# scrose/pylc

Measured on AMD Instinct MI355X. Metric: 512x512 tiles/sec fwd+bwd (DeepLabV3+/ResNet101, 9-class), higher is better.
Workload: dtype f32; 1 GPU; DeepLabV3+ ResNet101 OS16, 3-ch 512x512 tiles, 9 classes, CE+Dice+Focal, clip 0.5 + AdamW, bs=32/GPU (BASELINE.json configs[2]); global_batch=32, parallelism=dp1, conv_arithmetic=f16x3 split (fp32-grade), rccl_ranks=0, wgrad_queue=compute stream, sync_bn=True, activation_format=fp16 planes between BatchNorm and conv kernels (4 B/element)

## Files before the change

### include/pylc_hip.h

```cpp
#ifndef PYLC_HIP_H
#define PYLC_HIP_H

#include <stddef.h>
#include <stdint.h>

#ifdef __cplusplus
extern "C" {
#endif

#define PYLC_OK 0
#define PYLC_ERR_ARG 1
#define PYLC_ERR_HIP 2
#define PYLC_ERR_WORKSPACE 3
#define PYLC_ERR_UNSUPPORTED 4

const char* pylc_last_error(void);
int pylc_abi_version(void);
int pylc_experimental_build(void);
int pylc_init(void);

typedef struct PylcConvDesc {
    int B, H, W;
    int Cin, Cout;
    int R, S;
// ... 38 lines not shown
int pylc_to_planes(const float* x, int x_pitch, void* planes, int p_pitch, long long plane_stride, long long M, int C,
                   const unsigned int* amax, int nplanes, void* stream);
int pylc_from_planes(const void* planes, int p_pitch, long long plane_stride, float* x, int x_pitch, long long M, int C,
                     const unsigned int* amax, int nplanes, void* stream);
size_t pylc_planes_colsum_workspace_floats(int C);
int pylc_upsample2_crop_concat_planes(const float* z, int z_pitch, int B, int h, int w, int C1, const float* bridge, int bridge_pitch, int HH, int WW,
                                      int C2, void* planes, long long plane_stride, int nplanes, const unsigned int* bound, void* stream);
int pylc_planes_colsum(const void* planes, int p_pitch, long long plane_stride, int nplanes, const unsigned int* amax, long long M, int C,
                       float* sums, float* workspace, void* stream);

int pylc_conv2d_fwd(const PylcConvDesc* d, const float* x, const float* w_krsc, const float* bias,
                    float* y, void* stream);
int pylc_conv2d_fwd_bnact(const PylcConvDesc* d, const float* x, const float* w_krsc, const float* bias,
                          const float* scale, const float* shift, const float* residual, int relu, float* y,
                          unsigned int* amax_out, void* stream);

typedef struct PylcFwdEp {
    const float* scale;
    const float* shift;
    const unsigned int* scale_amax;
    const unsigned int* shift_amax;
    const void* residual;
    int res_fmt;
    const unsigned int* res_scale_bound;
    const unsigned int* res_amax;
    const unsigned int* x_true_amax;
    int relu;
    unsigned int* amax_out;
} PylcFwdEp;
int pylc_conv2d_fwd_bnact_ex(const PylcConvDesc* d, const void* x, const float* w, const float* bias, const PylcFwdEp* ep, void* y, void* stream);
size_t pylc_conv2d_fwd_stats_floats(const PylcConvDesc* d);
int pylc_conv2d_fwd_stats(const PylcConvDesc* d, const float* x, const float* w_krsc, const float* bias,
                          float* y, float* stats_partial, int* stats_rows, void* stream);
int pylc_conv2d_dgrad(const PylcConvDesc* d, const float* dy, const float* w_crsk, float* dx,
                      int accumulate, void* stream);
int pylc_conv2d_dgrad_add(const PylcConvDesc* d, const float* dy, const float* w_crsk, float* dx, int accumulate,
                          const float* add_src, const void* add_mask, void* stream);
#ifdef PYLC_EXPERIMENTAL
typedef struct PylcBnBack {
    const float* y;
    const float* mean;
    const float* invstd;
    const float* scale;
    const float* shift;
    const void* relu_mask;
    int relu;
    unsigned int* g_amax;
} PylcBnBack;
size_t pylc_conv2d_dgrad_bn_floats(const PylcConvDesc* d);
int pylc_conv2d_dgrad_bn(const PylcConvDesc* d, const float* dy, const float* w_crsk, float* dx, int accumulate,
                         const float* add_src, const void* add_mask, const PylcBnBack* bn, float* sums_partial, int* sums_rows,
                         void* stream);
#endif
int pylc_relu_bwd_bits(const float* dout, const void* mask, float* g_out, long long M, int C, void* stream);
int pylc_conv2d_dgrad_needs_f32_weights(const PylcConvDesc* d);
size_t pylc_conv2d_wgrad_workspace(const PylcConvDesc* d);
int pylc_conv2d_wgrad(const PylcConvDesc* d, const float* x, const float* dy, float* dw_krsc,
                      float* dbias ,
                      void* workspace, size_t workspace_bytes, void* stream);
typedef struct PylcSlabSum {
    const float* slabs;
    float* dw;
    long long n4;
    long long slab_stride;
    int splits;
    int reserved;
// ... 56 lines not shown
int pylc_bn_apply(const float* y, int y_pitch, const float* scale, const float* shift,
                  const float* residual, int res_pitch, float* out, int out_pitch,
                  long long M, int C, int relu, unsigned int* amax_out, void* stream);
int pylc_bn_bwd_reduce(const float* dout, int dout_pitch, const float* out, int out_pitch,
                       const float* y, int y_pitch, const float* mean, const float* invstd,
                       long long M, int C, int relu, float* sums , float* workspace,
                       const float* scale, const float* shift, void* stream);
int pylc_bn_bwd_apply(const float* dout, int dout_pitch, const float* out, int out_pitch,
                      const float* y, int y_pitch, const float* mean, const float* invstd,
                      const float* gamma, const float* sums, double n,
                      long long M, int C, int relu, float* dy, int dy_pitch, float* g_out, int g_pitch,
                      unsigned int* amax_dy, const float* scale, const float* shift, void* stream);
typedef struct PylcBnExtra {
    void* out_planes;        long long out_plane_stride;  const unsigned int* out_bound;
    const void* res_planes;  long long res_plane_stride;  const unsigned int* res_amax;
    void* dy_planes;         long long dy_plane_stride;   const unsigned int* dy_bound;
    int nplanes;
    float drop_p;
    uint64_t drop_seed;
    unsigned int* g_amax;
    void* relu_mask;
    const unsigned int* y_half_bound;
    const unsigned int* dout_half_bound;
} PylcBnExtra;
int pylc_bn_finalize_ex(const float* sums, double n, int C, const float* gamma, const float* beta, float eps, float momentum,
                        int clamp_eps, float* running_mean, float* running_var, float* mean, float* invstd, float* scale,
                        float* shift, const unsigned int* bound_extra, float bound_mul, unsigned int* bound_out,
                        const float* y, int y_pitch, long long M, const float* stat_shift, void* stream);
int pylc_bn_finalize_from_partial_ex(const float* partial, int n_rows, double n, int C, const float* gamma, const float* beta,
                                     float eps, float momentum, int clamp_eps, float* running_mean, float* running_var,
                                     float* mean, float* invstd, float* scale, float* shift, const unsigned int* bound_extra,
                                     float bound_mul, unsigned int* bound_out, const float* y, int y_pitch, long long M,
                                     const float* stat_shift, void* stream);
int pylc_bn_local_moments(const float* sums, double n, int C, const float* y, int y_pitch, long long M, const float* stat_shift,
                          double* moments, void* stream);
int pylc_bn_finalize_moments(const double* moments, double n, int C, const float* gamma, const float* beta, float eps, float momentum,
                             int clamp_eps, float* running_mean, float* running_var, float* mean, float* invstd, float* scale,
                             float* shift, const unsigned int* bound_extra, float bound_mul, unsigned int* bound_out,
                             const float* stat_shift, void* stream);
int pylc_bn_apply_ex(const float* y, int y_pitch, const float* scale, const float* shift, const float* residual, int res_pitch,
                     float* out, int out_pitch, long long M, int C, int relu, unsigned int* amax_out, const PylcBnExtra* ex,
                     void* stream);
int pylc_bn_bwd_reduce_ex(const float* dout, int dout_pitch, const float* out, int out_pitch, const float* y, int y_pitch,
                          const float* mean, const float* invstd, long long M, int C, int relu, float* sums, float* workspace,
                          const float* scale, const float* shift, const float* gamma, double n, const PylcBnExtra* ex,
                          unsigned int* dy_bound_out, void* stream);
int pylc_bn_bwd_bound(const float* sums, const float* gamma, const float* invstd, double n, int C, const unsigned int* g_amax,
                      unsigned int* bound_out, void* stream);
#ifdef PYLC_EXPERIMENTAL
int pylc_bn_bwd_sums_from_partial(const float* partial, int rows, int C, float* sums, const float* gamma, const float* invstd, double n,
                                  const unsigned int* g_amax, unsigned int* dy_bound_out, void* stream);
#endif
int pylc_bn_bwd_apply_ex(const float* dout, int dout_pitch, const float* out, int out_pitch, const float* y, int y_pitch,
                         const float* mean, const float* invstd, const float* gamma, const float* sums, double n, long long M,
                         int C, int relu, float* dy, int dy_pitch, float* g_out, int g_pitch, unsigned int* amax_dy,
                         const float* scale, const float* shift, const PylcBnExtra* ex, void* stream);
typedef struct PylcBnTwin {
    const float* y;          int y_pitch;
    const float* scale;      const float* shift;
    const float* mean;       const float* invstd;         const float* gamma;
    float* sums;             float* workspace;            unsigned int* dy_bound_out;
    float* dy;               int dy_pitch;
    void* dy_planes;         long long dy_plane_stride;   const unsigned int* dy_bound;
    unsigned int* amax_dy;
} PylcBnTwin;
int pylc_bn_affine_amax(const float* y, int y_pitch, const float* scale, const float* shift, long long M, int C, unsigned int* amax_out,
// ... 229 lines not shown
```

### pylc_amd/csrc/bn.hip

```cpp
#include "conv_common.h"
#include "slab.h"

namespace pylc {

struct PlanesRef {
    _Float16* base;
    long long plane_stride;
    int nplanes;
    float scale;
};

__device__ __forceinline__ void planes_store4(const PlanesRef& p, long long elem, f32x4 v) {
    uint2 p0, p1;
    split2(v, p.scale, p0, p1);
    if (p.nplanes == 2) {
        const bool odd = threadIdx.x & 1;
        const uint2 send = odd ? p0 : p1;
        uint2 recv;
        recv.x = (unsigned)__builtin_amdgcn_update_dpp(0, (int)send.x, 0xB1, 0xF, 0xF, true);
        recv.y = (unsigned)__builtin_amdgcn_update_dpp(0, (int)send.y, 0xB1, 0xF, 0xF, true);
        const uint4 val = odd ? make_uint4(recv.x, recv.y, p1.x, p1.y) : make_uint4(p0.x, p0.y, recv.x, recv.y);
        const bool il = planes_il(p.plane_stride);
        _Float16* dst = odd ? p.base + p.plane_stride + planes_phys(elem - 4, il) : p.base + planes_phys(elem, il);
        *reinterpret_cast<uint4*>(dst) = val;
// ... 304 lines not shown
    __shared__ double red[2][32][9];
    const int tx = threadIdx.x & 7, ty = threadIdx.x >> 3;
    const int c = blockIdx.x * 8 + tx;
    const bool mine = ty == 0 && c < C;
    bn_finalize_tail(mine ? (double)sums[c] : 0.0, mine ? (double)sums[C + c] : 0.0, red, tx, ty, c, n, C, gamma, beta, eps, momentum, clamp_eps,
                     running_mean, running_var, mean, invstd, scale, shift, bound_extra, bound_mul, bound_out, src);
}

__global__ __launch_bounds__(256) void bn_local_moments_kernel(const float* __restrict__ sums, double n, int C, RefineSrc src,
                                                               double* __restrict__ moments) {
    __shared__ double red[2][32][9];
    const int tx = threadIdx.x & 7, ty = threadIdx.x >> 3;
    const int c = blockIdx.x * 8 + tx;
    const bool mine = ty == 0 && c < C;
    double S1, S2;
    bn_local_moments(mine ? (double)sums[c] : 0.0, mine ? (double)sums[C + c] : 0.0, red, tx, ty, c, n, C, src, S1, S2);
    if (mine) {
        moments[c] = S1;
        moments[C + c] = S2;
        if (c == 0) moments[2 * C] = n;
    }
}

__global__ void bn_finalize_moments_kernel(const double* __restrict__ moments, double n, int C, const float* __restrict__ gamma,
                                           const float* __restrict__ beta, float eps, float momentum, int clamp_eps, float* running_mean,
                                           float* running_var, float* mean, float* invstd, float* scale, float* shift,
                                           const unsigned* bound_extra, float bound_mul, unsigned* bound_out, const float* stat_shift) {
    const int c = blockIdx.x * blockDim.x + threadIdx.x;
    if (c >= C) return;
    bn_coeffs_from_moments(moments[c], moments[C + c], stat_shift != nullptr ? (double)stat_shift[c] : 0.0, c, n, gamma, beta, eps, momentum,
                           clamp_eps, running_mean, running_var, mean, invstd, scale, shift, bound_extra, bound_mul, bound_out);
}

__global__ __launch_bounds__(256) void bn_finalize_partial_kernel(const float* __restrict__ partial, int nrows, double n, int C,
                                                                  const float* __restrict__ gamma, const float* __restrict__ beta, float eps,
                                                                  float momentum, int clamp_eps, float* running_mean, float* running_var,
                                                                  float* mean, float* invstd, float* scale, float* shift,
                                                                  const unsigned* bound_extra, float bound_mul, unsigned* bound_out,
                                                                  RefineSrc src) {
    __shared__ double red[2][32][9];
    const int tx = threadIdx.x & 7, ty = threadIdx.x >> 3;
    const int c = blockIdx.x * 8 + tx;
    double a0 = 0.0, a1 = 0.0;
    if (c < C) {
        for (int r = ty; r < nrows; r += 8 * 32) {
            float v0[8], v1[8];
#pragma unroll
            for (int u = 0; u < 8; ++u) {
                const int rr = r + u * 32;
                const size_t row = rr < nrows ? (size_t)rr : 0;
                v0[u] = partial[row * 2 * C + c];
                v1[u] = partial[row * 2 * C + C + c];
            }
#pragma unroll
            for (int u = 0; u < 8; ++u) {
                const bool ok = r + u * 32 < nrows;
                a0 += ok ? (double)v0[u] : 0.0;
                a1 += ok ? (double)v1[u] : 0.0;
            }
        }
    }
    red[0][ty][tx] = a0;
    red[1][ty][tx] = a1;
    __syncthreads();
    double s0 = 0.0, s1 = 0.0;
    if (ty == 0) {
#pragma unroll
        for (int k = 0; k < 32; ++k) { s0 += red[0][k][tx]; s1 += red[1][k][tx]; }
    }
    bn_finalize_tail((double)(float)s0, (double)(float)s1, red, tx, ty, c, n, C, gamma, beta, eps, momentum, clamp_eps, running_mean, running_var,
                     mean, invstd, scale, shift, bound_extra, bound_mul, bound_out, src);
}

__global__ void bn_eval_coeffs_kernel(const float* rm, const float* rv, const float* gamma, const float* beta, float eps,
                                      int C, float* scale, float* shift, float* mean, float* invstd) {
    const int c = blockIdx.x * blockDim.x + threadIdx.x;
    if (c >= C) return;
    const float sc = gamma[c] / sqrtf(rv[c] + eps);
    scale[c] = sc;
    shift[c] = beta[c] - rm[c] * sc;
    if (mean != nullptr) {
        mean[c] = rm[c];
        invstd[c] = 1.f / sqrtf(rv[c] + eps);
    }
}

template <bool EX = false, bool DROP = false, bool BITS = false, bool YH = false, bool TWIN = false>
__global__ __launch_bounds__(256) void bn_apply_kernel(const float* __restrict__ y, int y_pitch,
                                                       const float* __restrict__ scale, const float* __restrict__ shift,
                                                       const float* __restrict__ res, int res_pitch, float* __restrict__ out,
                                                       int out_pitch, int relu, Slab g, unsigned* __restrict__ amax_out, BnEx ex, BnTw tw) {
    const int tx = threadIdx.x % g.cols, ty = threadIdx.x / g.cols;
    const long long r_begin = (long long)blockIdx.x * g.rows_per_slab;
    long long r_end = r_begin + g.rows_per_slab;
    if (r_end > g.M) r_end = g.M;
    float amax = 0.f;
    PlanesRef po{}, pr{};
    DropRef dr{};
    float res_inv = 1.f;
    if constexpr (EX) {
        if (ex.out_pl != nullptr) po = PlanesRef{ex.out_pl, ex.out_ps, ex.nplanes, pow2_scale_for(*ex.out_bound)};
        if (ex.res_pl != nullptr) {
            pr = PlanesRef{const_cast<_Float16*>(ex.res_pl), ex.res_ps, ex.nplanes, 1.f};
            res_inv = 1.f / pow2_scale_for(*ex.res_amax);
// ... 419 lines not shown
}

extern "C" int pylc_bn_finalize_ex(const float* sums, double n, int C, const float* gamma, const float* beta, float eps, float momentum,
                                   int clamp_eps, float* running_mean, float* running_var, float* mean, float* invstd, float* scale,
                                   float* shift, const unsigned int* bound_extra, float bound_mul, unsigned int* bound_out,
                                   const float* y, int y_pitch, long long M, const float* stat_shift, void* stream) {
    PYLC_REQUIRE(sums && gamma && beta && mean && invstd && scale && shift && C > 0 && n > 0, "bn_finalize: bad arguments");
    PYLC_REQUIRE((running_mean == nullptr) == (running_var == nullptr), "bn_finalize: running stats must both be set or both NULL");
    PYLC_REQUIRE(y == nullptr || (y_pitch >= C && M > 0 && (double)M == n), "bn_finalize: the refinement source must be the n rows the sums cover");
    hipLaunchKernelGGL(bn_finalize_kernel, dim3(cdiv(C, 8)), dim3(256), 0, as_stream(stream), sums, n, C, gamma, beta, eps, momentum,
                       clamp_eps, running_mean, running_var, mean, invstd, scale, shift, bound_extra, bound_mul, bound_out,
                       RefineSrc{y, y_pitch, M, stat_shift});
    PYLC_LAUNCH_CHECK();
    return PYLC_OK;
}

extern "C" int pylc_bn_finalize(const float* sums, double n, int C, const float* gamma, const float* beta, float eps, float momentum,
                                int clamp_eps, float* running_mean, float* running_var, float* mean, float* invstd, float* scale,
                                float* shift, void* stream) {
    return pylc_bn_finalize_ex(sums, n, C, gamma, beta, eps, momentum, clamp_eps, running_mean, running_var, mean, invstd, scale, shift,
                               nullptr, 1.f, nullptr, nullptr, 0, 0, nullptr, stream);
}

extern "C" int pylc_bn_finalize_from_partial_ex(const float* partial, int n_rows, double n, int C, const float* gamma, const float* beta,
                                                float eps, float momentum, int clamp_eps, float* running_mean, float* running_var,
                                                float* mean, float* invstd, float* scale, float* shift, const unsigned int* bound_extra,
                                                float bound_mul, unsigned int* bound_out, const float* y, int y_pitch, long long M,
                                                const float* stat_shift, void* stream) {
    PYLC_REQUIRE(partial && n_rows > 0 && gamma && beta && mean && invstd && scale && shift && C > 0 && n > 0,
                 "bn_finalize_from_partial: bad arguments");
    PYLC_REQUIRE((running_mean == nullptr) == (running_var == nullptr), "bn_finalize_from_partial: running stats must both be set or both NULL");
    PYLC_REQUIRE(y == nullptr || (y_pitch >= C && M > 0 && (double)M == n),
                 "bn_finalize_from_partial: the refinement source must be the n rows the partials cover");
    hipLaunchKernelGGL(bn_finalize_partial_kernel, dim3(cdiv(C, 8)), dim3(256), 0, as_stream(stream), partial, n_rows, n, C, gamma, beta, eps,
                       momentum, clamp_eps, running_mean, running_var, mean, invstd, scale, shift, bound_extra, bound_mul, bound_out,
                       RefineSrc{y, y_pitch, M, stat_shift});
    PYLC_LAUNCH_CHECK();
    return PYLC_OK;
}

extern "C" int pylc_bn_finalize_from_partial(const float* partial, int n_rows, double n, int C, const float* gamma, const float* beta,
                                             float eps, float momentum, int clamp_eps, float* running_mean, float* running_var,
                                             float* mean, float* invstd, float* scale, float* shift, void* stream) {
    return pylc_bn_finalize_from_partial_ex(partial, n_rows, n, C, gamma, beta, eps, momentum, clamp_eps, running_mean, running_var, mean,
                                            invstd, scale, shift, nullptr, 1.f, nullptr, nullptr, 0, 0, nullptr, stream);
}

extern "C" int pylc_bn_local_moments(const float* sums, double n, int C, const float* y, int y_pitch, long long M, const float* stat_shift,
                                     double* moments, void* stream) {
    PYLC_REQUIRE(sums && moments && C > 0 && n > 0, "bn_local_moments: bad arguments");
    PYLC_REQUIRE(y == nullptr || (y_pitch >= C && M > 0 && (double)M == n), "bn_local_moments: the refinement source must be the n rows the sums cover");
    hipLaunchKernelGGL(bn_local_moments_kernel, dim3(cdiv(C, 8)), dim3(256), 0, as_stream(stream), sums, n, C, RefineSrc{y, y_pitch, M, stat_shift},
                       moments);
    PYLC_LAUNCH_CHECK();
    return PYLC_OK;
}

extern "C" int pylc_bn_finalize_moments(const double* moments, double n, int C, const float* gamma, const float* beta, float eps,
                                        float momentum, int clamp_eps, float* running_mean, float* running_var, float* mean, float* invstd,
                                        float* scale, float* shift, const unsigned int* bound_extra, float bound_mul,
                                        unsigned int* bound_out, const float* stat_shift, void* stream) {
    PYLC_REQUIRE(moments && gamma && beta && mean && invstd && scale && shift && C > 0 && n > 0, "bn_finalize_moments: bad arguments");
    PYLC_REQUIRE((running_mean == nullptr) == (running_var == nullptr), "bn_finalize_moments: running stats must both be set or both NULL");
    hipLaunchKernelGGL(bn_finalize_moments_kernel, dim3(cdiv(C, 256)), dim3(256), 0, as_stream(stream), moments, n, C, gamma, beta, eps, momentum,
                       clamp_eps, running_mean, running_var, mean, invstd, scale, shift, bound_extra, bound_mul, bound_out, stat_shift);
    PYLC_LAUNCH_CHECK();
    return PYLC_OK;
}

// ... 393 lines not shown
```

### pylc_amd/csrc/conv_common.h

```cpp
#pragma once
#include "common.h"
#include <type_traits>

namespace pylc {

typedef float f32x4 __attribute__((ext_vector_type(4)));
typedef float f32x16 __attribute__((ext_vector_type(16)));

typedef __bf16 bf16x8 __attribute__((ext_vector_type(8)));

typedef _Float16 f16x8 __attribute__((ext_vector_type(8)));
typedef _Float16 f16x2 __attribute__((ext_vector_type(2)));
typedef float f32x2 __attribute__((ext_vector_type(2)));

constexpr int LDB = 80;

__device__ __forceinline__ void split3(const float (&x)[4], uint2& p0, uint2& p1, uint2& p2) {
    unsigned u0[4], u1[4], u2[4];
#pragma unroll
    for (int e = 0; e < 4; ++e) {
        u0[e] = __float_as_uint(x[e]);
        const float r1 = x[e] - __uint_as_float(u0[e] & 0xFFFF0000u);
        u1[e] = __float_as_uint(r1);
        const float r2 = r1 - __uint_as_float(u1[e] & 0xFFFF0000u);
// ... 63 lines not shown
    const float* ep_scale;
    const float* ep_shift;
    const float* ep_res;
    unsigned* ep_amax;
    int ep_relu;
    int ep_vec_ok;
    const unsigned* bound_x;
    const unsigned* ep_scale_amax;
    const unsigned* ep_shift_amax;
    const unsigned* ep_res_amax;
    const unsigned* ep_res_scale;
    int ep_res_fmt;
    long long ep_res_plane_stride;
    int out_planes2;
    long long out_plane_stride;
    int tiles_n;
    int n_tiles;
    const unsigned* amax_x;
    const unsigned* amax_w;
    long long x_bytes, w_bytes;
    const void* w_planes;
    long long w_plane_stride;
    int w_il;
    const void* x_planes;
    long long x_plane_stride;
    int nterms;
    int tile_bm;
    int halo_tiles_m;
    int ident;
    int stagger, stagger_blocks;
    int dbg_flags;
    unsigned long long* dbg;
    float* stats;
};

typedef float f32x4v __attribute__((ext_vector_type(4)));

__device__ __forceinline__ float row_sum16(float v) {
#define PYLC_DPP_ADD(ctrl) v += __builtin_bit_cast(float, __builtin_amdgcn_update_dpp(0, __builtin_bit_cast(int, v), ctrl, 0xF, 0xF, true))
    PYLC_DPP_ADD(0xB1);
    PYLC_DPP_ADD(0x4E);
    PYLC_DPP_ADD(0x141);
    PYLC_DPP_ADD(0x140);
#undef PYLC_DPP_ADD
    return v;
}


struct WgradArgs {
    const float* x;
    const float* dy;
    float* out;
    int M, P, Q;
    int IH, IW, Cin, x_pitch, in_sh, in_sw;
    int TR, TS, dh0, dh_step, dw0, dw_step;
    int N, N_ld, dy_pitch;
    int out_row_stride;
    int tiles_n, tiles_c;
    int splits, m_per_split;
    long long slab_stride;
    const unsigned* amax_dy;
    const unsigned* amax_x;
    long long x_bytes, dy_bytes;
    const void* x_planes;
    const void* dy_planes;
    long long x_plane_stride, dy_plane_stride;
// ... 34 lines not shown
```

### pylc_amd/csrc/conv_igemm.hip

```cpp
#include "conv_common.h"

namespace pylc {

template <int BM, int BN, int WM, int WN, bool CIN4, int PREC>
__global__ __launch_bounds__((BM / WM) * (BN / WN) * 64, 2) void gather_gemm_kernel(const GatherGemmArgs a) {
    constexpr int WAVES_N = BN / WN;
    constexpr int MT = WM / 32, NT = WN / 32;
    constexpr int NTHR = (BM / WM) * (BN / WN) * 64;
    constexpr int RPI = NTHR / 8;
    constexpr int A_IT = BM / RPI, B_IT = BN / RPI;
    static_assert(NTHR == 256 || NTHR == 512, "4 or 8 waves per block");
    static_assert(BM % RPI == 0 && BN % RPI == 0, "tile rows must divide evenly over the loader");
    extern __shared__ __attribute__((aligned(16))) float smem[];
    float* sA = smem;
    float* sB = smem + 2 * BM * LDT;

    const int tile = xcd_remap(blockIdx.x, gridDim.x);
    const int m0 = (tile / a.tiles_n) * BM;
    const int n0 = (tile % a.tiles_n) * BN;
    const int tid = threadIdx.x, lane = tid & 63, wave = tid >> 6;
    const int wave_m = wave / WAVES_N, wave_n = wave % WAVES_N;
    const int v = tid & 7, r0 = tid >> 3;

    int rowh[A_IT], roww[A_IT], rowpix[A_IT];
// ... 1506 lines not shown
    const int ow = (d->W + 2 * d->pad - d->dil * (d->S - 1) - 1) / d->stride + 1;
    PYLC_REQUIRE(oh == d->OH && ow == d->OW && oh > 0 && ow > 0, "OH/OW (%d,%d) inconsistent with geometry (%d,%d)", d->OH, d->OW, oh, ow);
    PYLC_REQUIRE((long long)d->B * d->H * d->W * d->x_pitch < (1ll << 31) && (long long)d->B * d->OH * d->OW * d->y_pitch < (1ll << 31),
                 "tensor exceeds 2^31 elements");
    return PYLC_OK;
}

static inline int roundup4(int v) { return (v + 3) & ~3; }

}

using namespace pylc;

extern "C" int pylc_set_conv_precision(int mode) {
    PYLC_REQUIRE(mode >= 0 && mode <= 3, "conv precision mode must be 0 (fp32 MFMA), 1 (bf16x6), 2 (f16x3) or 3 (fp16 operands, fp32 accumulation)");
    g_conv_precision = mode;
    return PYLC_OK;
}

extern "C" int pylc_get_conv_precision(void) { return g_conv_precision; }

extern "C" int pylc_debug_pp_stamps(unsigned long long* buf) { g_pp_stamps = buf; return PYLC_OK; }
extern "C" int pylc_debug_pp_flags(int flags) { g_pp_flags = flags; g_wgrad_fast = !(flags & 8); return PYLC_OK; }

extern "C" int pylc_debug_set_big_tile(int on) { g_big_tile = on; return PYLC_OK; }

namespace {
struct FwdEpilogue {
    const float* scale; const float* shift; const float* res; unsigned* amax; int relu;
    const PylcFwdEp* ex = nullptr;
};
}
static int conv2d_fwd_impl(const PylcConvDesc* d, const float* x, const float* w, const float* bias, float* y, float* stats, int* stats_rows,
                           void* stream, const FwdEpilogue* ep = nullptr);

extern "C" int pylc_conv2d_fwd(const PylcConvDesc* d, const float* x, const float* w, const float* bias, float* y, void* stream) {
    return conv2d_fwd_impl(d, x, w, bias, y, nullptr, nullptr, stream);
}

extern "C" int pylc_conv2d_fwd_bnact(const PylcConvDesc* d, const float* x, const float* w, const float* bias, const float* scale,
                                     const float* shift, const float* residual, int relu, float* y, unsigned int* amax_out, void* stream) {
    PYLC_REQUIRE(scale && shift, "conv2d_fwd_bnact: null scale / shift");
    const FwdEpilogue ep{scale, shift, residual, amax_out, relu};
    return conv2d_fwd_impl(d, x, w, bias, y, nullptr, nullptr, stream, &ep);
}

extern "C" int pylc_conv2d_fwd_bnact_ex(const PylcConvDesc* d, const void* x, const float* w, const float* bias, const PylcFwdEp* ep, void* y,
                                        void* stream) {
    PYLC_REQUIRE(ep != nullptr && ep->scale && ep->shift, "conv2d_fwd_bnact_ex: null epilogue / scale / shift");
    PYLC_REQUIRE(d->x_fmt == 1, "conv2d_fwd_bnact_ex: x must be an fp16-plane tensor (pylc_conv2d_fwd_bnact takes fp32 tensors)");
    PYLC_REQUIRE(ep->res_fmt >= 0 && ep->res_fmt <= 2 && (ep->res_fmt == 0 || (ep->residual && ep->res_scale_bound)),
                 "conv2d_fwd_bnact_ex: res_fmt 1 / 2 needs the residual planes and the bound they were scaled with");
    PYLC_REQUIRE(d->out_fmt == 0 || (d->out_bound && ep->scale_amax && ep->shift_amax && (ep->residual == nullptr || ep->res_amax)),
                 "conv2d_fwd_bnact_ex: a plane output needs out_bound, max|scale|, max|shift| and (with a residual) max|residual|");
    const FwdEpilogue fe{ep->scale, ep->shift, ep->res_fmt == 0 ? static_cast<const float*>(ep->residual) : nullptr, ep->amax_out, ep->relu, ep};
    return conv2d_fwd_impl(d, static_cast<const float*>(x), w, bias, static_cast<float*>(y), nullptr, nullptr, stream, &fe);
}

extern "C" size_t pylc_conv2d_fwd_stats_floats(const PylcConvDesc* d) {
    if (check_desc(d)) return 0;
    const long long M = (long long)d->B * d->OH * d->OW;
    return (size_t)cdiv<long long>(M, 128) * 2 * (size_t)roundup4(d->Cout);
}

extern "C" int pylc_conv2d_fwd_stats(const PylcConvDesc* d, const float* x, const float* w, const float* bias, float* y, float* stats_partial,
                                     int* stats_rows, void* stream) {
    PYLC_REQUIRE(stats_partial && stats_rows, "conv2d_fwd_stats: null statistics buffer");
    return conv2d_fwd_impl(d, x, w, bias, y, stats_partial, stats_rows, stream);
}

static int conv2d_fwd_impl(const PylcConvDesc* d, const float* x, const float* w, const float* bias, float* y, float* stats, int* stats_rows,
                           void* stream, const FwdEpilogue* ep) {
    if (int rc = check_desc(d)) return rc;
    PYLC_REQUIRE(x && y && (w || (d->x_fmt == 1 && d->w_planes)), "null pointer");
    GatherGemmArgs a{};
    if (ep != nullptr) {
        a.ep_scale = ep->scale; a.ep_shift = ep->shift; a.ep_res = ep->res; a.ep_amax = ep->amax; a.ep_relu = ep->relu;
        a.ep_vec_ok = ((reinterpret_cast<uintptr_t>(ep->scale) | reinterpret_cast<uintptr_t>(ep->shift) | reinterpret_cast<uintptr_t>(bias)) & 15) == 0;
    }
    a.stats = stats;
    a.dbg = g_pp_stamps;
    a.dbg_flags = g_pp_flags;
    PYLC_REQUIRE(g_conv_precision < 2 || (d->x_amax && d->w_amax), "f16x3 / fp16 mode: conv2d_fwd needs x_amax and w_amax in the descriptor");
    a.amax_x = d->x_amax; a.amax_w = d->w_amax;
    a.x = x; a.w = w; a.bias = bias; a.y = y;
    a.x_bytes = (((long long)d->B * d->H * d->W - 1) * d->x_pitch + d->Cin) * 4;
    a.w_bytes = (long long)d->Cout * d->R * d->S * d->Cin * 4;
    a.w_planes = d->w_planes; a.w_plane_stride = (long long)d->Cout * d->R * d->S * d->Cin;
    a.w_il = (d->w_planes != nullptr && (d->w_planes_fmt & 1)) ? 1 : 0;
    if (d->x_fmt == 1) {
        a.x_planes = x; a.x = nullptr;
        a.x_plane_stride = planes_stride_rule((long long)d->B * d->H * d->W, d->Cin, d->x_pitch, (g_conv_precision == 3 ? 1 : 2));
        a.x_bytes /= 2;
    }
    a.P = d->OH; a.Q = d->OW; a.M = d->B * d->OH * d->OW;
    a.IH = d->H; a.IW = d->W; a.Cin = d->Cin; a.x_pitch = d->x_pitch;
    a.in_sh = a.in_sw = d->stride;
    a.TR = d->R; a.TS = d->S;
    a.dh0 = -d->pad; a.dh_step = d->dil; a.dw0 = -d->pad; a.dw_step = d->dil;
    a.w_off0 = 0; a.w_step_r = d->S * d->Cin; a.w_step_s = d->Cin; a.w_row_stride = d->R * d->S * d->Cin;
    a.N = d->Cout; a.N_store = roundup4(d->Cout) <= d->y_pitch ? roundup4(d->Cout) : d->Cout;
    a.OH = d->OH; a.OW = d->OW; a.out_sh = a.out_sw = 1; a.oh0 = a.ow0 = 0; a.y_pitch = d->y_pitch;
    a.accumulate = 0;
    if (ep != nullptr && ep->ex != nullptr) {
        const PylcFwdEp* ex = ep->ex;
        a.bound_x = ex->x_true_amax;
        a.ep_scale_amax = ex->scale_amax; a.ep_shift_amax = ex->shift_amax;
        if (ex->residual != nullptr) {
            a.ep_res = static_cast<const float*>(ex->residual);
            a.ep_res_fmt = ex->res_fmt; a.ep_res_scale = ex->res_scale_bound; a.ep_res_amax = ex->res_amax;
            a.ep_res_plane_stride = planes_stride_rule((long long)d->B * d->OH * d->OW, d->Cout, d->Cout, ex->res_fmt == 2 ? 2 : 1);
        }
        if (d->out_fmt != 0) {
            PYLC_REQUIRE((d->out_fmt == 1 || d->out_fmt == 2) && d->y_pitch == d->Cout && d->Cout % 4 == 0,
                         "conv2d_fwd_bnact_ex: a plane output (out_fmt 1 / 2) needs a dense y with Cout %% 4 == 0");
            a.out_half = d->out_fmt == 1; a.out_planes2 = d->out_fmt == 2;
            a.out_plane_stride = planes_stride_rule((long long)d->B * d->OH * d->OW, d->Cout, d->y_pitch, d->out_fmt == 2 ? 2 : 1);
            a.out_bound_k = (float)(d->Cin * d->R * d->S); a.out_bound = d->out_bound;
        }
    } else if (d->out_fmt == 1) {
        PYLC_REQUIRE(d->x_fmt == 1 && d->out_bound && bias == nullptr && ep == nullptr && d->y_pitch == d->Cout && d->Cout % 4 == 0,
                     "conv2d_fwd: a one-plane fp16 output needs fp16-plane input, out_bound, no bias / fused epilogue and a dense y");
        a.out_half = 1; a.out_bound_k = (float)(d->Cin * d->R * d->S); a.out_bound = d->out_bound;
    }
    const bool cin4 = d->Cin == 4 && d->R * d->S > 1;
    if (cin4 && ep == nullptr && takes_stem(a)) {
        if (int rc = launch_stem_fwd(a, as_stream(stream))) return rc;
    } else if (int rc = dispatch_gg(a, cin4, as_stream(stream))) return rc;
    if (stats_rows) *stats_rows = a.halo_tiles_m > 0 ? a.halo_tiles_m : cdiv(a.M, a.x_planes != nullptr ? a.tile_bm : (a.tiles_n > 0 ? g_last_bm : 128));
    return PYLC_OK;
}

extern "C" int pylc_conv2d_dgrad_needs_f32_weights(const PylcConvDesc* d) {
    if (check_desc(d)) return 1;
    if (g_conv_precision < 2 || d->w_planes_t == nullptr) return 1;
    if (d->dy_fmt == 1) return 0;
    if (d->stride != 1) return 1;
    const int Kp = roundup4(d->Cout);
    GatherGemmArgs a{};
    a.Cin = Kp;
    a.x_bytes = (((long long)d->B * d->OH * d->OW - 1) * d->y_pitch + Kp) * 4;
    a.w_bytes = (long long)d->Cin * d->R * d->S * Kp * 4;
    const long long M = (long long)d->B * d->H * d->W;
    const bool big = d->Cin > 64 && g_big_tile && cdiv<long long>(M, 256) * cdiv(d->Cin, 128) >= 192;
    return (big && takes_pp(a)) ? 0 : 1;
}

extern "C" int pylc_conv2d_dgrad_add(const PylcConvDesc* d, const float* dy, const float* w_crsk, float* dx, int accumulate,
                                     const float* add_src, const void* add_mask, void* stream);
extern "C" int pylc_conv2d_dgrad(const PylcConvDesc* d, const float* dy, const float* w_crsk, float* dx, int accumulate, void* stream) {
    return pylc_conv2d_dgrad_add(d, dy, w_crsk, dx, accumulate, nullptr, nullptr, stream);
}

struct BnBackArgs { const float* y; const float* mean; const float* invstd; const float* scale; const float* shift; const void* relu_mask; int relu; unsigned int* g_amax; };
static int conv2d_dgrad_impl(const PylcConvDesc* d, const float* dy, const float* w_crsk, float* dx, int accumulate,
                             const float* add_src, const void* add_mask, const BnBackArgs* bn, float* sums_partial, int* sums_rows, void* stream);

extern "C" int pylc_conv2d_dgrad_add(const PylcConvDesc* d, const float* dy, const float* w_crsk, float* dx, int accumulate,
                                     const float* add_src, const void* add_mask, void* stream) {
    return conv2d_dgrad_impl(d, dy, w_crsk, dx, accumulate, add_src, add_mask, nullptr, nullptr, nullptr, stream);
}
// ... 304 lines not shown
```

### pylc_amd/csrc/conv_pl.hip

```cpp
#include "conv_common.h"

namespace pylc {

typedef __attribute__((address_space(3))) void* lds_vptr;

constexpr int PL_BN = 128;
constexpr int PL_ROW = 64;
template <int NTERMS>
constexpr int pl_row_bytes() { return NTERMS == 1 ? 128 : PL_ROW; }
template <int NTERMS, int BM>
constexpr int pl_stage_bytes() { return (NTERMS == 3 ? 2 : 1) * (BM + PL_BN) * pl_row_bytes<NTERMS>(); }
template <int BM>
constexpr int pl_stages() { return BM == 256 ? 3 : 2; }
template <int NTERMS, int BM>
constexpr int pl_lds_bytes() { return pl_stages<BM>() * pl_stage_bytes<NTERMS, BM>() + BM * 4 + 64; }

#ifndef PYLC_EPI_FULL_LINES
#define PYLC_EPI_FULL_LINES 1
#endif
#ifndef PYLC_EPI_PK
#define PYLC_EPI_PK 0
#endif
__device__ __forceinline__ f32x4v epi_fma(f32x4v a, float b, f32x4v c) {
#if PYLC_EPI_PK
    const f32x4v bb = {b, b, b, b};
    return __builtin_elementwise_fma(a, bb, c);
#else
    return f32x4v{__builtin_fmaf(a[0], b, c[0]), __builtin_fmaf(a[1], b, c[1]), __builtin_fmaf(a[2], b, c[2]), __builtin_fmaf(a[3], b, c[3])};
#endif
}
__device__ __forceinline__ f32x4v epi_mul(f32x4v a, float b) {
#if PYLC_EPI_PK
    return a * b;
#else
    return f32x4v{a[0] * b, a[1] * b, a[2] * b, a[3] * b};
#endif
}
__device__ __forceinline__ f32x4v epi_sq(f32x4v a) {
#if PYLC_EPI_PK
    return a * a;
#else
    return f32x4v{a[0] * a[0], a[1] * a[1], a[2] * a[2], a[3] * a[3]};
#endif
}
__device__ __forceinline__ f32x4v epi_add(f32x4v a, f32x4v b) {
#if PYLC_EPI_PK
    return a + b;
#else
    return f32x4v{a[0] + b[0], a[1] + b[1], a[2] + b[2], a[3] + b[3]};
#endif
}

template <int AM, int NPL, int NTERMS>
__device__ __forceinline__ void pl_step_schedule() {
    constexpr int AT = 4;
    if constexpr (AM >= 3) {
        __builtin_amdgcn_sched_group_barrier(0x100, (AT + 2) * NPL, 0);
        __builtin_amdgcn_sched_group_barrier(0x008, AT * NTERMS, 0);
#pragma unroll
        for (int r = 2; r < AM; ++r) {
            __builtin_amdgcn_sched_group_barrier(0x100, NPL, 0);
            __builtin_amdgcn_sched_group_barrier(0x008, AT * NTERMS, 0);
        }
        __builtin_amdgcn_sched_group_barrier(0x008, AT * NTERMS, 0);
    } else {
        __builtin_amdgcn_sched_group_barrier(0x100, (AT + AM) * NPL, 0);
        __builtin_amdgcn_sched_group_barrier(0x008, AM * AT * NTERMS, 0);
    }
}

template <int AM, int STATS, int PREV, bool HALF>
__device__ __forceinline__ void pl_epilogue_lean(const GatherGemmArgs& a, f32x4v (&acc)[AM][4], const int* rowoff,
                                                 float* sdst, int nb, int wave_m, int lane, float c, float hscale,
                                                 const float* extra, const unsigned char* amask, const float* bias) {
    constexpr int AT = 4, WM = 16 * AM;
    typedef _Float16 f16x4_ __attribute__((ext_vector_type(4)));
    typedef unsigned u32x2_ __attribute__((ext_vector_type(2)));
    unsigned offs[AM];
#pragma unroll
    for (int i = 0; i < AM; ++i) offs[i] = (unsigned)(rowoff[wave_m * WM + i * 16 + (lane & 15)] + nb);
    constexpr bool FULL = !HALF && PYLC_EPI_FULL_LINES != 0;
    unsigned offsP[FULL ? AM : 1];
    if constexpr (FULL) {
#pragma unroll
        for (int i = 0; i < AM; ++i) offsP[i] = (unsigned)(rowoff[wave_m * WM + i * 16 + ((lane & 15) ^ 8)] + nb);
    }
    const bool upper = (lane & 8) != 0;
    uint2 hq[(HALF && PYLC_EPI_FULL_LINES != 0) ? AM : 1][4];
    f32x4v hold[FULL ? AM : 1];
    f32x4v prevn[(FULL && PREV != 0) ? AM : 1];
    const float k = HALF ? c * hscale : c;
    const float post = HALF ? pow2_inv(hscale) : c;
    const bool odd_row = (lane >> 4) & 1;
#pragma unroll
    for (int j = 0; j < AT; ++j) {
        f32x4v prev[PREV ? AM : 1];
        if constexpr (PREV != 0) {
            unsigned mb[AM];
#pragma unroll
            for (int i = 0; i < AM; ++i) {
                if constexpr (!FULL) prev[i] = *reinterpret_cast<const f32x4v*>(extra + (offs[i] + j * 16));
                if constexpr (PREV == 2) mb[i] = amask[(offs[i] + j * 16) >> 3];
            }
            if constexpr (FULL) {
                if ((j & 1) == 0) {
                    const unsigned col = (upper ? j + 1 : j) * 16;
                    f32x4v la[AM], lb[AM];
#pragma unroll
                    for (int i = 0; i < AM; ++i) {
                        la[i] = *reinterpret_cast<const f32x4v*>(extra + ((upper ? offsP[i] : offs[i]) + col));
                        lb[i] = *reinterpret_cast<const f32x4v*>(extra + ((upper ? offs[i] : offsP[i]) + col));
                    }
#pragma unroll
                    for (int i = 0; i < AM; ++i)
#pragma unroll
                        for (int r = 0; r < 4; ++r) {
                            const float send = upper ? la[i][r] : lb[i][r];
                            const float recv = __builtin_bit_cast(float, __builtin_amdgcn_update_dpp(0, __builtin_bit_cast(int, send), 0x128, 0xF, 0xF, true));
                            prev[i][r] = upper ? recv : la[i][r];
                            prevn[i][r] = upper ? lb[i][r] : recv;
                        }
                } else {
#pragma unroll
                    for (int i = 0; i < AM; ++i) prev[i] = prevn[i];
                }
            }
            if constexpr (PREV == 2) {
#pragma unroll
                for (int i = 0; i < AM; ++i) {
                    const int nib = (int)(mb[i] >> ((((offs[i] + j * 16) >> 2) & 1u) * 4u));
#pragma unroll
                    for (int r = 0; r < 4; ++r)
                        prev[i][r] = __uint_as_float(__float_as_uint(prev[i][r]) & (unsigned)__builtin_amdgcn_sbfe(nib, r, 1));
                }
            }
        }
        f32x4v bv = {0.f, 0.f, 0.f, 0.f};
        if (!HALF && bias != nullptr) bv = *reinterpret_cast<const f32x4v*>(bias + nb + j * 16);
        f32x4v cs = {0.f, 0.f, 0.f, 0.f}, css = cs;
#pragma unroll
        for (int i = 0; i < AM; ++i) {
            const f32x4v t = acc[i][j];
            if constexpr (HALF) {
                const f32x4v v = epi_mul(t, k);
                const f16x4_ h = {(_Float16)v[0], (_Float16)v[1], (_Float16)v[2], (_Float16)v[3]};
                if constexpr (STATS != 0) {
#pragma unroll
                    for (int r = 0; r < 4; ++r) {
                        cs[r] = i == 0 ? (float)h[r] : __builtin_fmaf((float)h[r], 1.f, cs[r]);
                        css[r] = i == 0 ? (float)h[r] * (float)h[r] : __builtin_fmaf((float)h[r], (float)h[r], css[r]);
                    }
                }
                if constexpr (PYLC_EPI_FULL_LINES != 0) {
                    hq[i][j] = __builtin_bit_cast(uint2, h);
                } else {
                    const uint2 hu = __builtin_bit_cast(uint2, h);
                    const u32x2_ sx = __builtin_amdgcn_permlane16_swap(hu.x, hu.x, false, false);
                    const u32x2_ sy = __builtin_amdgcn_permlane16_swap(hu.y, hu.y, false, false);
                    if (!odd_row) *reinterpret_cast<uint4*>(reinterpret_cast<_Float16*>(a.y) + (offs[i] + j * 16)) = uint4{hu.x, hu.y, sx.y, sy.y};
                }
            } else {
                if constexpr (STATS != 0) {
                    cs = i == 0 ? t : epi_add(cs, t);
                    css = i == 0 ? epi_sq(t) : epi_add(css, epi_sq(t));
                }
                f32x4v v = epi_fma(t, k, bv);
                if constexpr (PREV != 0) v = epi_add(v, prev[i]);
                if constexpr (!FULL) {
                    *reinterpret_cast<f32x4v*>(a.y + (offs[i] + j * 16)) = v;
                } else if ((j & 1) == 0) {
                    hold[i] = v;
                } else {
                    f32x4v recv;
#pragma unroll
                    for (int r = 0; r < 4; ++r) {
                        const float send = upper ? hold[i][r] : v[r];
                        recv[r] = __builtin_bit_cast(float, __builtin_amdgcn_update_dpp(0, __builtin_bit_cast(int, send), 0x128, 0xF, 0xF, true));
                    }
                    const unsigned col = (upper ? j : j - 1) * 16;
                    f32x4v da, db;
#pragma unroll
                    for (int r = 0; r < 4; ++r) { da[r] = upper ? recv[r] : hold[i][r]; db[r] = upper ? v[r] : recv[r]; }
                    *reinterpret_cast<f32x4v*>(a.y + ((upper ? offsP[i] : offs[i]) + col)) = da;
                    *reinterpret_cast<f32x4v*>(a.y + ((upper ? offs[i] : offsP[i]) + col)) = db;
                }
            }
        }
        if constexpr (STATS != 0) {
#pragma unroll
            for (int r = 0; r < 4; ++r) { cs[r] = row_sum16(cs[r]); css[r] = row_sum16(css[r]); }
            if ((lane & 15) == 0) {
#pragma unroll
                for (int r = 0; r < 4; ++r) { sdst[(j * 16 + r) * 2] = cs[r] * post; sdst[(j * 16 + r) * 2 + 1] = css[r] * post * post; }
            }
        }
    }
    if constexpr (HALF && PYLC_EPI_FULL_LINES != 0) {
        unsigned offsP[AM];
#pragma unroll
        for (int i = 0; i < AM; ++i) offsP[i] = (unsigned)(rowoff[wave_m * WM + i * 16 + ((lane & 15) ^ 8)] + nb - 4 * (lane >> 4));
        const unsigned q4 = (unsigned)(lane >> 4);
        const unsigned colq = odd_row ? 16u + 4u * (q4 - 1u) : 4u * q4;
#pragma unroll
        for (int i = 0; i < AM; ++i) {
            const u32x2_ ax = __builtin_amdgcn_permlane16_swap(hq[i][0].x, hq[i][1].x, false, false);
            const u32x2_ ay = __builtin_amdgcn_permlane16_swap(hq[i][0].y, hq[i][1].y, false, false);
            const u32x2_ bx = __builtin_amdgcn_permlane16_swap(hq[i][2].x, hq[i][3].x, false, false);
            const u32x2_ by = __builtin_amdgcn_permlane16_swap(hq[i][2].y, hq[i][3].y, false, false);
            const unsigned s0 = upper ? ax.x : bx.x, s1 = upper ? ay.x : by.x, s2 = upper ? ax.y : bx.y, s3 = upper ? ay.y : by.y;
            const unsigned r0 = (unsigned)__builtin_amdgcn_update_dpp(0, (int)s0, 0x128, 0xF, 0xF, true);
            const unsigned r1 = (unsigned)__builtin_amdgcn_update_dpp(0, (int)s1, 0x128, 0xF, 0xF, true);
            const unsigned r2 = (unsigned)__builtin_amdgcn_update_dpp(0, (int)s2, 0x128, 0xF, 0xF, true);
            const unsigned r3 = (unsigned)__builtin_amdgcn_update_dpp(0, (int)s3, 0x128, 0xF, 0xF, true);
            const unsigned base_own = offs[i] - 4u * q4, base_par = offsP[i];
            const unsigned col = (upper ? 32u : 0u) + colq;
            const uint4 da = {upper ? r0 : ax.x, upper ? r1 : ay.x, upper ? r2 : ax.y, upper ? r3 : ay.y};
            const uint4 db = {upper ? bx.x : r0, upper ? by.x : r1, upper ? bx.y : r2, upper ? by.y : r3};
            *reinterpret_cast<uint4*>(reinterpret_cast<_Float16*>(a.y) + ((upper ? base_par : base_own) + col)) = da;
            *reinterpret_cast<uint4*>(reinterpret_cast<_Float16*>(a.y) + ((upper ? base_own : base_par) + col)) = db;
        }
    }
}

template <int AM, int PREV, bool EDGE>
__device__ __forceinline__ float pl_epilogue_bn(const GatherGemmArgs& a, f32x4v (&acc)[AM][4], const int* rowoff, float* sdst, int nb, int wave_m,
                                                int lane, float c, const float* extra, const unsigned char* amask) {
// ... 229 lines not shown
                    val[r] = t * esc[j][r] + esh[j][r];
                }
                if constexpr (RES != 0) {
                    const f32x4v rv = __builtin_convertvector(__builtin_bit_cast(f16x4_, rq[j]), f32x4v) * res_unscale;
#pragma unroll
                    for (int r = 0; r < 4; ++r) val[r] += rv[r];
                }
#pragma unroll
                for (int r = 0; r < 4; ++r) {
                    if (relu) val[r] = fmaxf(val[r], 0.f);
                    ep_max = fmaxf(ep_max, fabsf(val[r]));
                }
                const f32x4v v = val * hscale;
                const f16x4_ h = {(_Float16)v[0], (_Float16)v[1], (_Float16)v[2], (_Float16)v[3]};
                hq[j] = __builtin_bit_cast(uint2, h);
            }
            const u32x2_ ax = __builtin_amdgcn_permlane16_swap(hq[0].x, hq[1].x, false, false), ay = __builtin_amdgcn_permlane16_swap(hq[0].y, hq[1].y, false, false);
            const u32x2_ bx = __builtin_amdgcn_permlane16_swap(hq[2].x, hq[3].x, false, false), by = __builtin_amdgcn_permlane16_swap(hq[2].y, hq[3].y, false, false);
            const unsigned s0 = upper ? ax.x : bx.x, s1 = upper ? ay.x : by.x, s2 = upper ? ax.y : bx.y, s3 = upper ? ay.y : by.y;
            const unsigned r0 = (unsigned)__builtin_amdgcn_update_dpp(0, (int)s0, 0x128, 0xF, 0xF, true);
            const unsigned r1 = (unsigned)__builtin_amdgcn_update_dpp(0, (int)s1, 0x128, 0xF, 0xF, true);
            const unsigned r2 = (unsigned)__builtin_amdgcn_update_dpp(0, (int)s2, 0x128, 0xF, 0xF, true);
            const unsigned r3 = (unsigned)__builtin_amdgcn_update_dpp(0, (int)s3, 0x128, 0xF, 0xF, true);
            const uint4 da = {upper ? r0 : ax.x, upper ? r1 : ay.x, upper ? r2 : ax.y, upper ? r3 : ay.y};
            const uint4 db = {upper ? bx.x : r0, upper ? by.x : r1, upper ? bx.y : r2, upper ? by.y : r3};
            *reinterpret_cast<uint4*>(yp + ((upper ? baseP[i] : base[i]) + col)) = da;
            *reinterpret_cast<uint4*>(yp + ((upper ? base[i] : baseP[i]) + col)) = db;
        }
        __builtin_amdgcn_sched_barrier(0);
    }
    return ep_max;
}

template <int NTERMS, int BM, bool BNB = false, int AM = 4, bool EP = false, bool LEAN_RES = true>
__device__ __forceinline__ int pl_epilogue(const GatherGemmArgs& a, f32x4v (&acc)[AM][4], f32x4v (&acc_lo)[NTERMS == 3 ? AM : 1][NTERMS == 3 ? 4 : 1],
                                            const int* rowoff, float* smem, int tile_m, int n0, int wave_m, int wave_n, int lane, int tid, bool rows_full,
                                            const unsigned* ranges = nullptr, int stat_cols = PL_BN) {
    constexpr int BN = PL_BN, WM = 16 * AM, WN = 64, AT = 4;
    typedef f32x4v f32x4v_;
    float* sred = smem;
    const bool do_stats = a.stats != nullptr;
    const unsigned ax_bits = ranges != nullptr ? ranges[0] : (a.amax_x ? *a.amax_x : 0u);
    const unsigned aw_bits = ranges != nullptr ? ranges[1] : (a.amax_w ? *a.amax_w : 0u);
    const float scale_a = a.amax_x ? pow2_scale_for(ax_bits) : 1.f;
    const float scale_b = a.amax_w ? pow2_scale_for(aw_bits) : 1.f;
    const float unscale_a = pow2_inv(scale_a), unscale_b = pow2_inv(scale_b);
    float hscale = 1.f;
    if (a.out_half || (EP && a.out_planes2)) {
        float b;
        if constexpr (EP) {
            b = a.out_bound_k * __uint_as_float(*(a.bound_x != nullptr ? a.bound_x : a.amax_x)) * __uint_as_float(*a.amax_w);
            if (a.ep_scale_amax != nullptr) b = b * __uint_as_float(*a.ep_scale_amax) + __uint_as_float(*a.ep_shift_amax);
            if (a.ep_res_amax != nullptr) b += __uint_as_float(*a.ep_res_amax);
        } else {
            b = a.out_bound_k * __uint_as_float(ax_bits) * __uint_as_float(aw_bits);
        }
        hscale = pow2_scale_for(__float_as_uint(b));
        if (blockIdx.x == 0 && tid == 0) *a.out_bound = __float_as_uint(b);
    }
    const float* extra = a.add_src != nullptr ? a.add_src : (a.accumulate ? a.y : ((EP && a.ep_res_fmt == 0) ? a.ep_res : nullptr));
    const bool res_planes = EP && a.ep_res != nullptr && a.ep_res_fmt != 0;
    const float res_unscale = res_planes ? pow2_inv(pow2_scale_for(*a.ep_res_scale)) : 1.f;
    const unsigned char* amask = a.add_mask;
    if constexpr (NTERMS == 3) {
#pragma unroll
        for (int i = 0; i < AM; ++i)
#pragma unroll
            for (int j = 0; j < AT; ++j) acc[i][j] = epi_fma(acc_lo[i][j], 1.f / 2048.f, acc[i][j]);
    }
    bool done = false;
    int tail_stores = 0;
    if constexpr (!EP && !BNB) {
        const bool cols_full = n0 + wave_n * WN + WN <= (a.bias != nullptr ? a.N : a.N_store);
        if ((a.bias == nullptr || ((reinterpret_cast<uintptr_t>(a.bias) & 15) == 0 && !a.out_half)) && rows_full && cols_full && !(do_stats && extra != nullptr) && (NTERMS == 1 || !a.out_half) &&
            !(a.out_half && extra != nullptr) && !(a.dbg_flags & 8)) {
            done = true;
            tail_stores = (PYLC_EPI_FULL_LINES != 0) ? (a.out_half ? 2 * AM : 4 * AM) : 0;
            float* const sd = smem + ((wave_m * BN) + wave_n * WN + 4 * (lane >> 4)) * 2;
            const int nb = n0 + wave_n * WN + 4 * (lane >> 4);
            const float c = unscale_a * unscale_b;
#define PYLC_LEAN(ST, PV, HF) pl_epilogue_lean<AM, ST, PV, HF>(a, acc, rowoff, sd, nb, wave_m, lane, c, hscale, extra, amask, a.bias)
            if constexpr (NTERMS == 1) {
                if (a.out_half) {
                    if (do_stats) PYLC_LEAN(1, 0, true); else PYLC_LEAN(0, 0, true);
                } else if (extra != nullptr) {
                    if (amask != nullptr) PYLC_LEAN(0, 2, false); else PYLC_LEAN(0, 1, false);
                } else if (do_stats) PYLC_LEAN(1, 0, false);
                else PYLC_LEAN(0, 0, false);
            } else {
                if (extra != nullptr) {
                    if (amask != nullptr) PYLC_LEAN(0, 2, false); else PYLC_LEAN(0, 1, false);
                } else if (do_stats) PYLC_LEAN(1, 0, false);
                else PYLC_LEAN(0, 0, false);
            }
#undef PYLC_LEAN
        }
    }
    if constexpr (EP) {
        const int nchunk = n0 + wave_n * WN;
        const bool res_ok = a.ep_res == nullptr || (LEAN_RES && a.ep_res_fmt == 2 && planes_il(a.ep_res_plane_stride));
        if (rows_full && nchunk + WN <= a.N && a.out_planes2 && !a.out_half && planes_il(a.out_plane_stride) && a.y_pitch == a.N_store && (a.bias == nullptr || a.ep_res == nullptr) &&
            a.ep_scale != nullptr && a.ep_vec_ok && extra == nullptr && res_ok &&
            !do_stats && !(a.dbg_flags & 8)) {
            done = true;
            const float c = unscale_a * unscale_b;
            float m;
            if (LEAN_RES && a.ep_res != nullptr) m = pl_epilogue_lean_ep<AM, LEAN_RES ? 2 : 0, false>(a, acc, rowoff, nchunk, wave_m, lane, c, hscale, res_unscale);
            else if (a.bias != nullptr) m = pl_epilogue_lean_ep<AM, 0, true>(a, acc, rowoff, nchunk, wave_m, lane, c, hscale, res_unscale);
            else m = pl_epilogue_lean_ep<AM, 0, false>(a, acc, rowoff, nchunk, wave_m, lane, c, hscale, res_unscale);
            if (a.ep_amax != nullptr) amax_commit(m, a.ep_amax);
        }
        if constexpr (NTERMS == 1) {
            const bool res1_ok = a.ep_res == nullptr || (LEAN_RES && a.ep_res_fmt == 1);
            if (!done && rows_full && nchunk + WN <= a.N && a.out_half && a.y_pitch == a.N_store && (a.N_store & 7) == 0 && a.ep_scale != nullptr &&
                a.ep_vec_ok && extra == nullptr && res1_ok && !do_stats && !(a.dbg_flags & 8)) {
                done = true;
                const float c = unscale_a * unscale_b;
                float m;
                if (LEAN_RES && a.ep_res != nullptr) {
                    m = a.bias != nullptr ? pl_epilogue_lean_ep_half<AM, LEAN_RES ? 1 : 0, true>(a, acc, rowoff, nchunk, wave_m, lane, c, hscale, res_unscale)
                                          : pl_epilogue_lean_ep_half<AM, LEAN_RES ? 1 : 0, false>(a, acc, rowoff, nchunk, wave_m, lane, c, hscale, res_unscale);
                } else {
                    m = a.bias != nullptr ? pl_epilogue_lean_ep_half<AM, 0, true>(a, acc, rowoff, nchunk, wave_m, lane, c, hscale, res_unscale)
                                          : pl_epilogue_lean_ep_half<AM, 0, false>(a, acc, rowoff, nchunk, wave_m, lane, c, hscale, res_unscale);
                }
// ... 38 lines not shown
            for (int i = 0; i < AM; ++i) eoff[i][j] = (nok && offs[i] >= 0) ? offs[i] + n4 : -1;
#pragma unroll
            for (int r = 0; r < 4; ++r) bv[j][r] = (a.bias != nullptr && n4 + r < a.N) ? a.bias[n4 + r] : 0.f;
            if constexpr (EP) {
#pragma unroll
                for (int r = 0; r < 4; ++r) {
                    esc[j][r] = (a.ep_scale != nullptr && n4 + r < a.N) ? a.ep_scale[n4 + r] : 1.f;
                    esh[j][r] = (a.ep_scale != nullptr && n4 + r < a.N) ? a.ep_shift[n4 + r] : 0.f;
                }
            }
        }
    }
    constexpr int PJ = 2;
    __builtin_amdgcn_sched_barrier(0);
#pragma unroll
    for (int i = 0; i < AM; ++i)
#pragma unroll
        for (int j = 0; j < AT; ++j)
#pragma unroll
            for (int r = 0; r < 4; ++r) {
                acc[i][j][r] = acc[i][j][r] * unscale_a * unscale_b;
            }
    if (!EP && a.out_half) {
        const float inv_h = pow2_inv(hscale);
#pragma unroll
        for (int i = 0; i < AM; ++i)
#pragma unroll
            for (int j = 0; j < AT; ++j)
#pragma unroll
                for (int r = 0; r < 4; ++r) acc[i][j][r] = (float)(_Float16)(acc[i][j][r] * hscale) * inv_h;
    }
    __builtin_amdgcn_sched_barrier(0);
    float* sdst = sred + ((wave_m * BN) + wave_n * WN + 4 * (lane >> 4)) * 2;
    auto finish = [&](auto has_prev, auto j0c, const f32x4v_ (&prev)[AM][PJ]) {
        constexpr int j0 = decltype(j0c)::value;
        constexpr bool phased = decltype(has_prev)::value;
        constexpr int NJ = phased ? PJ : AT;
#pragma unroll
        for (int jj = 0; jj < NJ; ++jj) {
            const int j = j0 + jj;
            float cs[4] = {0.f, 0.f, 0.f, 0.f}, css[4] = {0.f, 0.f, 0.f, 0.f};
#pragma unroll
            for (int i = 0; i < AM; ++i) {
                const bool stored = eoff[i][j] >= 0;
#pragma unroll
                for (int r = 0; r < 4; ++r) {
                    float val = acc[i][j][r] + bv[j][r];
                    if constexpr (EP) val = val * esc[j][r] + esh[j][r];
                    if constexpr (decltype(has_prev)::value) val += prev[i][jj][r];
                    if constexpr (EP) {
                        if (a.ep_relu) val = fmaxf(val, 0.f);
                        ep_max = fmaxf(ep_max, stored ? fabsf(val) : 0.f);
                    }
                    acc[i][j][r] = val;
                    const float cv = stored ? val - bv[j][r] : 0.f;
                    cs[r] += cv;
                    css[r] += cv * cv;
                }
            }
            if (do_stats) {
#pragma unroll
                for (int r = 0; r < 4; ++r) { cs[r] = row_sum16(cs[r]); css[r] = row_sum16(css[r]); }
                if ((lane & 15) == 0) {
#pragma unroll
                    for (int r = 0; r < 4; ++r) { sdst[(j * 16 + r) * 2] = cs[r]; sdst[(j * 16 + r) * 2 + 1] = css[r]; }
                }
            }
        }
        __builtin_amdgcn_sched_barrier(0);
        if (a.out_half || (EP && a.out_planes2)) {
            typedef _Float16 f16x4_ __attribute__((ext_vector_type(4)));
            typedef unsigned u32x2_ __attribute__((ext_vector_type(2)));
            const bool odd_row = (lane >> 4) & 1;
#pragma unroll
            for (int jj = 0; jj < NJ; ++jj)
#pragma unroll
                for (int i = 0; i < AM; ++i) {
                    const int e = eoff[i][j0 + jj];
                    uint4 q;
                    const bool ilo = !a.out_half && planes_il(a.out_plane_stride);
                    _Float16* dst = reinterpret_cast<_Float16*>(a.y) + planes_phys(odd_row ? e - 4 : e, ilo);
                    if (a.out_half) {
                        const f32x4v_ v = acc[i][j0 + jj] * hscale;
                        const f16x4_ h = {(_Float16)v[0], (_Float16)v[1], (_Float16)v[2], (_Float16)v[3]};
                        const uint2 hu = __builtin_bit_cast(uint2, h);
                        const u32x2_ sx = __builtin_amdgcn_permlane16_swap(hu.x, hu.x, false, false);
                        const u32x2_ sy = __builtin_amdgcn_permlane16_swap(hu.y, hu.y, false, false);
                        q = uint4{hu.x, hu.y, sx.y, sy.y};
                        if (e >= 0 && !odd_row) *reinterpret_cast<uint4*>(dst) = q;
                    } else {
// ... 74 lines not shown
        fetch_res(0);
        __builtin_amdgcn_sched_barrier(0);
        finish(std::true_type{}, std::integral_constant<int, 0>{}, prev);
        __builtin_amdgcn_sched_barrier(0);
        fetch_res(2);
        __builtin_amdgcn_sched_barrier(0);
        finish(std::true_type{}, std::integral_constant<int, 2>{}, prev);
    } else if (extra == nullptr) {
        finish(std::false_type{}, std::integral_constant<int, 0>{}, none);
    } else {
        fetch(0);
        __builtin_amdgcn_sched_barrier(0);
        finish(std::true_type{}, std::integral_constant<int, 0>{}, prev);
        __builtin_amdgcn_sched_barrier(0);
        fetch(2);
        __builtin_amdgcn_sched_barrier(0);
        finish(std::true_type{}, std::integral_constant<int, 2>{}, prev);
    }
    if (EP && a.ep_amax != nullptr) amax_commit(ep_max, a.ep_amax);
    }
    }
    if (bn && a.bn_gmax != nullptr) amax_commit(gmax, a.bn_gmax);
    if (do_stats) {
        asm volatile("s_waitcnt lgkmcnt(0)\n\ts_barrier" ::: "memory");
        if (tid < stat_cols) {
            const int n = n0 + tid;
            if (n < a.N_store) {
                float sm = 0.f, sq = 0.f;
#pragma unroll
                for (int wm = 0; wm < BM / WM; ++wm) { sm += sred[(wm * BN + tid) * 2]; sq += sred[(wm * BN + tid) * 2 + 1]; }
                float* dst = a.stats + (size_t)tile_m * 2 * a.N_store;
                dst[n] = sm;
                dst[a.N_store + n] = sq;
            }
        }
    }
    return tail_stores;
}

template <int NTERMS, int BM, bool STAMPS = false, bool BNB = false, bool NARROW = false, bool EP = false>
__global__ __launch_bounds__(BM * 2, 2) void gg_pl_kernel(const GatherGemmArgs a) {
    constexpr int BN = PL_BN, AM = NARROW ? 2 : 4, WM = 16 * AM, WN = 64, AT = 4, ROW = pl_row_bytes<NTERMS>();
    constexpr int KS = ROW / 2;
    constexpr int RPI = 1024 / ROW;
    constexpr int NW = BM / 32;
    constexpr int NST = pl_stages<BM>();
    constexpr int AI = 32 / RPI;
    constexpr int BI = BN / (RPI * NW);
    constexpr int NPL = NTERMS == 3 ? 2 : 1;
    constexpr int NDMA = (AI + BI) * NPL;
    constexpr int STAGE = pl_stage_bytes<NTERMS, BM>();
    constexpr int OFF_B = NPL * BM * ROW;
    constexpr unsigned OOB = 0x80000000u;
    extern __shared__ __attribute__((aligned(16))) float smem[];
    char* lds = reinterpret_cast<char*>(smem);
    int* rowoff = reinterpret_cast<int*>(lds + NST * STAGE);
    unsigned long long* s_wave_taps = reinterpret_cast<unsigned long long*>(lds + NST * STAGE + BM * 4);
    unsigned long long* stamp_base = reinterpret_cast<unsigned long long*>(lds + NST * STAGE + BM * 4 + 64);
    int n_stamp = 0;
#define PL_STAMP()                                                                                                    \
    if constexpr (STAMPS) {                                                                                           \
        if (stamper && n_stamp < 250) stamp_base[(wave != 0) * 256 + n_stamp++] = __builtin_amdgcn_s_memtime();       \
    }

    const int tile = xcd_remap(blockIdx.x, gridDim.x);
    const int m0 = (tile / a.tiles_n) * BM;
    const int n0 = (tile % a.tiles_n) * BN;
    const int tid = threadIdx.x, lane = tid & 63;
    const int wave = __builtin_amdgcn_readfirstlane(tid >> 6);
    const int wave_m = NARROW ? wave : wave >> 1, wave_n = NARROW ? 0 : wave & 1;
    if constexpr (BM == 128) {
        if (a.stagger > 0 && (int)blockIdx.x < a.stagger_blocks) {
            if (a.dbg_flags & 32768) {
// ... 198 lines not shown
    } else {
        if (S > 0) {
            PL_STAMP();
            issue(0);
            if (S > 1) issue(1);
            int sc = 0, sn = 2;
            const bool late = wave >= NW / 2 && !(a.dbg_flags & 32768);
            for (int s = 0; s < S; ++s) {
                PL_STAMP();
                if (s + 1 < S) {
                    static_assert(NDMA == 6, "256-row tiles: 6 DMA instructions per wave and K-step (f16x3: (2 + 1) x 2 planes; one plane, 128-byte rows: 4 + 2)");
                    asm volatile("s_waitcnt vmcnt(6)" ::: "memory");
                } else {
                    asm volatile("s_waitcnt vmcnt(0)" ::: "memory");
                }
                __builtin_amdgcn_s_barrier();
                __builtin_amdgcn_sched_barrier(0);
                PL_STAMP();
                if (!late && s + 2 < S && !(STAMPS && (a.dbg_flags & 64))) issue(sn);
                __builtin_amdgcn_sched_barrier(0);
                PL_STAMP();
                if (!(STAMPS && (a.dbg_flags & 128))) compute(sc);
                __builtin_amdgcn_sched_barrier(0);
                if (late && s + 2 < S && !(STAMPS && (a.dbg_flags & 64))) issue(sn);
                __builtin_amdgcn_sched_barrier(0);
                sc = sc == 2 ? 0 : sc + 1;
                sn = sn == 2 ? 0 : sn + 1;
            }
        }
    }
    PL_STAMP();
    __syncthreads();

    pl_epilogue<NTERMS, BM, BNB, AM, EP>(a, acc, acc_lo, rowoff, reinterpret_cast<float*>(smem), tile / a.tiles_n, n0, wave_m, wave_n, lane, tid, m0 + BM <= a.M);
    if constexpr (STAMPS) {
        __builtin_amdgcn_sched_barrier(0);
        PL_STAMP();
        if (stamper && a.dbg != nullptr)
            for (int k = 0; k < 256; ++k) a.dbg[(wave != 0) * 256 + k] = k < n_stamp ? stamp_base[(wave != 0) * 256 + k] : 0ull;
    }
#undef PL_STAMP
}

template <int PREV, typename Between, typename Stamp>
__device__ __forceinline__ void plp_epilogue_lean(const GatherGemmArgs& a, f32x4v (&acc)[4][4], const int* rowoff, int n0, int wave_m, int wave_n, int lane, float c,
                                                  const float* extra, const unsigned char* amask, Between&& between, Stamp&& stamp) {
    constexpr int AM = 4, AT = 4, WM = 64, WN = 64;
    const int nb = n0 + wave_n * WN + 4 * (lane >> 4);
    unsigned offs[AM], offsP[AM];
#pragma unroll
    for (int i = 0; i < AM; ++i) {
        offs[i] = (unsigned)(rowoff[wave_m * WM + i * 16 + (lane & 15)] + nb);
        offsP[i] = (unsigned)(rowoff[wave_m * WM + i * 16 + ((lane & 15) ^ 8)] + nb);
    }
    const bool upper = (lane & 8) != 0;
    f32x4v la[PREV ? 2 : 1][PREV ? AM : 1], lb[PREV ? 2 : 1][PREV ? AM : 1];
    uint2 mw[PREV == 2 ? AM : 1];
    if constexpr (PREV != 0) {
#pragma unroll
        for (int jp = 0; jp < 2; ++jp) {
            const unsigned col = (upper ? 2 * jp + 1 : 2 * jp) * 16;
#pragma unroll
            for (int i = 0; i < AM; ++i) {
                la[jp][i] = *reinterpret_cast<const f32x4v*>(extra + ((upper ? offsP[i] : offs[i]) + col));
                lb[jp][i] = *reinterpret_cast<const f32x4v*>(extra + ((upper ? offs[i] : offsP[i]) + col));
            }
        }
// ... 23 lines not shown
                        prev[r] = upper ? recv : la[j >> 1][i][r];
                        la[j >> 1][i][r] = upper ? lb[j >> 1][i][r] : recv;
                    }
                } else {
                    prev = la[j >> 1][i];
                }
                if constexpr (PREV == 2) {
                    const int nib = (int)(((j < 2) ? mw[i].x : mw[i].y) >> (16u * (unsigned)(j & 1) + 4u * (unsigned)(lane >> 4)));
#pragma unroll
                    for (int r = 0; r < 4; ++r) prev[r] = __uint_as_float(__float_as_uint(prev[r]) & (unsigned)__builtin_amdgcn_sbfe(nib, r, 1));
                }
                v = epi_add(v, prev);
            }
            if ((j & 1) == 0) {
                hold[i] = v;
            } else {
                f32x4v recv;
#pragma unroll
                for (int r = 0; r < 4; ++r) {
                    const float send = upper ? hold[i][r] : v[r];
                    recv[r] = __builtin_bit_cast(float, __builtin_amdgcn_update_dpp(0, __builtin_bit_cast(int, send), 0x128, 0xF, 0xF, true));
                }
                const unsigned col = (upper ? j : j - 1) * 16;
                f32x4v da, db;
#pragma unroll
                for (int r = 0; r < 4; ++r) { da[r] = upper ? recv[r] : hold[i][r]; db[r] = upper ? v[r] : recv[r]; }
                *reinterpret_cast<f32x4v*>(a.y + ((upper ? offsP[i] : offs[i]) + col)) = da;
                *reinterpret_cast<f32x4v*>(a.y + ((upper ? offs[i] : offsP[i]) + col)) = db;
            }
        }
    }
}

template <typename Between, typename Stamp>
__device__ __forceinline__ void plp_epilogue_stats(const GatherGemmArgs& a, f32x4v (&acc)[4][4], const int* rowoff, float* sred, int tile_m, int n0,
                                                   int wave_m, int wave_n, int lane, int tid, float c, Between&& between, Stamp&& stamp) {
    constexpr int AM = 4, AT = 4, WM = 64, WN = 64, BN = PL_BN, BM = 128;
    const int nb = n0 + wave_n * WN + 4 * (lane >> 4);
    unsigned offs[AM], offsP[AM];
#pragma unroll
    for (int i = 0; i < AM; ++i) {
        offs[i] = (unsigned)(rowoff[wave_m * WM + i * 16 + (lane & 15)] + nb);
        offsP[i] = (unsigned)(rowoff[wave_m * WM + i * 16 + ((lane & 15) ^ 8)] + nb);
    }
    const bool upper = (lane & 8) != 0;
    const unsigned sdst_at = (unsigned)(uintptr_t)(lds_vptr)(sred + ((wave_m * BN) + wave_n * WN + 4 * (lane >> 4)) * 2);
    const unsigned comb_at = (unsigned)(uintptr_t)(lds_vptr)(sred + (tid & (BN - 1)) * 2);
    __builtin_amdgcn_sched_barrier(0);
    stamp();
    between();
    __builtin_amdgcn_sched_barrier(0);
    stamp();
    f32x4v hold[AM];
#pragma unroll
    for (int j = 0; j < AT; ++j) {
        f32x4v cs = {0.f, 0.f, 0.f, 0.f}, css = cs;
#pragma unroll
        for (int i = 0; i < AM; ++i) {
            const f32x4v t = acc[i][j];
            cs = i == 0 ? t : epi_add(cs, t);
            css = i == 0 ? epi_sq(t) : epi_add(css, epi_sq(t));
            const f32x4v v = epi_mul(t, c);
            if ((j & 1) == 0) {
                hold[i] = v;
            } else {
                f32x4v recv;
#pragma unroll
                for (int r = 0; r < 4; ++r) {
                    const float send = upper ? hold[i][r] : v[r];
                    recv[r] = __builtin_bit_cast(float, __builtin_amdgcn_update_dpp(0, __builtin_bit_cast(int, send), 0x128, 0xF, 0xF, true));
                }
                const unsigned col = (upper ? j : j - 1) * 16;
                f32x4v da, db;
#pragma unroll
                for (int r = 0; r < 4; ++r) { da[r] = upper ? recv[r] : hold[i][r]; db[r] = upper ? v[r] : recv[r]; }
                *reinterpret_cast<f32x4v*>(a.y + ((upper ? offsP[i] : offs[i]) + col)) = da;
                *reinterpret_cast<f32x4v*>(a.y + ((upper ? offs[i] : offsP[i]) + col)) = db;
            }
        }
#pragma unroll
        for (int r = 0; r < 4; ++r) { cs[r] = row_sum16(cs[r]); css[r] = row_sum16(css[r]); }
        if ((lane & 15) == 0) {
#pragma unroll
            for (int r = 0; r < 4; ++r) {
                const float s0 = cs[r] * c, s1 = css[r] * c * c;
                asm volatile("ds_write_b32 %0, %1" :: "v"(sdst_at + (unsigned)((j * 16 + r) * 8)), "v"(s0) : "memory");
                asm volatile("ds_write_b32 %0, %1" :: "v"(sdst_at + (unsigned)((j * 16 + r) * 8 + 4)), "v"(s1) : "memory");
            }
        }
    }
    asm volatile("s_waitcnt lgkmcnt(0)\n\ts_barrier" ::: "memory");
    if (tid < BN) {
        const int n = n0 + tid;
        if (n < a.N_store) {
            float p00, p01, p10, p11;
            asm volatile("ds_read_b32 %0, %1" : "=v"(p00) : "v"(comb_at) : "memory");
            asm volatile("ds_read_b32 %0, %1" : "=v"(p01) : "v"(comb_at + 4u) : "memory");
            asm volatile("ds_read_b32 %0, %1" : "=v"(p10) : "v"(comb_at + (unsigned)(BN * 8)) : "memory");
            asm volatile("ds_read_b32 %0, %1" : "=v"(p11) : "v"(comb_at + (unsigned)(BN * 8 + 4)) : "memory");
            asm volatile("s_waitcnt lgkmcnt(0)" ::: "memory");
            asm volatile("" : "+v"(p00), "+v"(p01), "+v"(p10), "+v"(p11));
            float sm = 0.f, sq = 0.f;
            sm += p00; sq += p01;
            sm += p10; sq += p11;
            float* dst = a.stats + (size_t)tile_m * 2 * a.N_store;
            dst[n] = sm;
            dst[a.N_store + n] = sq;
        }
    }
    static_assert(BM / WM == 2, "two row halves per statistics column");
}

template <int NTERMS>
constexpr int plp_lds_bytes() { return 2 * pl_stage_bytes<NTERMS, 128>() + 4 * 128 * 4 + 2 * PL_BN * 2 * 4 + 64; }

#define PLP_VMCNT(n) __builtin_amdgcn_s_waitcnt(((n) & 15) | (((n) >> 4) << 14) | (7 << 4) | (15 << 8))
__device__ __forceinline__ void plp_wait_vm(int n) {
    if (n >= 16) PLP_VMCNT(16);
    else if (n >= 8) PLP_VMCNT(8);
    else PLP_VMCNT(0);
}

template <int NTERMS, int EPK, bool STAMPS = false>
__global__ __launch_bounds__(256, 2) void gg_plp_kernel(const GatherGemmArgs a) {
    constexpr int BM = 128, BN = PL_BN, AM = 4, WM = 64, WN = 64, AT = 4, ROW = pl_row_bytes<NTERMS>();
    constexpr int KS = ROW / 2, RPI = 1024 / ROW, NW = 4, AI = 32 / RPI, BI = BN / (RPI * NW), NPL = NTERMS == 3 ? 2 : 1;
    constexpr int STAGE = pl_stage_bytes<NTERMS, BM>();
    constexpr int OFF_B = NPL * BM * ROW;
    constexpr unsigned OOB = 0x80000000u;
    extern __shared__ __attribute__((aligned(16))) float smem[];
    char* lds = reinterpret_cast<char*>(smem);
    int* const rowoff4 = reinterpret_cast<int*>(lds + 2 * STAGE);
    float* const sred = reinterpret_cast<float*>(lds + 2 * STAGE + 4 * BM * 4);

    const int tid = threadIdx.x, lane = tid & 63;
    const int wave = __builtin_amdgcn_readfirstlane(tid >> 6);
    const int wave_m = wave >> 1, wave_n = wave & 1;
    const bool stamper = STAMPS && (int)blockIdx.x == (a.dbg_flags >> 16) && lane == 0 && (wave == 0 || wave == 3);
    unsigned stamp_at = (unsigned)(uintptr_t)(lds_vptr)(lds + plp_lds_bytes<NTERMS>() + (wave != 0) * 2048);
    int n_stamp = 0;
    auto stamp = [&]() {
        if constexpr (STAMPS) {
            if (stamper && n_stamp < 250) {
                const unsigned long long t = __builtin_amdgcn_s_memtime();
                asm volatile("ds_write_b64 %0, %1" :: "v"(stamp_at), "v"(t) : "memory");
                stamp_at += 8;
                ++n_stamp;
// ... 128 lines not shown
    zero_acc();
#pragma clang loop unroll(disable)
    for (int g = 0; g < total; ++g) {
        stamp();
        if (soft_waits > 0) { plp_wait_vm(stores_in_flight); --soft_waits; }
        else PLP_VMCNT(0);
        if constexpr (STAMPS) { __builtin_amdgcn_sched_barrier(0); stamp(); }
        __builtin_amdgcn_s_barrier();
        __builtin_amdgcn_sched_barrier(0);
        stamp();
        if (skip_issue > 0) --skip_issue;
        else issue((g + 1) & 1);
        __builtin_amdgcn_sched_barrier(0);
        stamp();
        compute(g & 1);
        __builtin_amdgcn_sched_barrier(0);
        if (++s == S) {
            s = 0;
            stamp();
            asm volatile("s_waitcnt lgkmcnt(0)" ::: "memory");
            __builtin_amdgcn_s_barrier();
            __builtin_amdgcn_sched_barrier(0);
            stamp();
            const int tile = xcd_remap(v, n_tiles);
            const int n0 = (tile % a.tiles_n) * BN;
            bool pre2 = false;
            if constexpr (NTERMS == 3) {
#pragma unroll
                for (int i = 0; i < AM; ++i)
#pragma unroll
                    for (int j = 0; j < AT; ++j) acc[i][j] = epi_fma(acc_lo[i][j], 1.f / 2048.f, acc[i][j]);
            }
            auto between = [&]() { pre2 = issue(g & 1); };
            if constexpr (EPK == 1)
                plp_epilogue_stats(a, acc, rowoff4 + (k & 3) * BM, sred, tile / a.tiles_n, n0, wave_m, wave_n, lane, tid, c_unscale, between, stamp);
            else
                plp_epilogue_lean<EPK >= 2 ? EPK - 1 : 0>(a, acc, rowoff4 + (k & 3) * BM, n0, wave_m, wave_n, lane, c_unscale, a.add_src != nullptr ? a.add_src : a.y,
                                                          a.add_mask, between, stamp);
            stamp();
            PLP_VMCNT(16);
            stores_in_flight = 16;
            __builtin_amdgcn_sched_barrier(0);
            zero_acc();
            v += G;
            ++k;
            soft_waits = (pre2 && !(a.dbg_flags & 2097152)) ? 2 : 0;
            skip_issue = pre2 ? 1 : 0;
        }
    }
    if constexpr (STAMPS) {
        stamp();
        PLP_VMCNT(0);
        asm volatile("s_waitcnt lgkmcnt(0)" ::: "memory");
        if (stamper && a.dbg != nullptr) {
            const unsigned long long* sb = reinterpret_cast<const unsigned long long*>(lds + plp_lds_bytes<NTERMS>() + (wave != 0) * 2048);
            for (int q = 0; q < 256; ++q) a.dbg[(wave != 0) * 256 + q] = q < n_stamp ? sb[q] : 0ull;
        }
    }
}

template __global__ void gg_plp_kernel<3, 0>(const GatherGemmArgs);
template __global__ void gg_plp_kernel<3, 0, true>(const GatherGemmArgs);
template __global__ void gg_plp_kernel<3, 1, true>(const GatherGemmArgs);
template __global__ void gg_plp_kernel<3, 1>(const GatherGemmArgs);
template __global__ void gg_plp_kernel<3, 2>(const GatherGemmArgs);
template __global__ void gg_plp_kernel<3, 3>(const GatherGemmArgs);
template __global__ void gg_plp_kernel<1, 0>(const GatherGemmArgs);
template __global__ void gg_plp_kernel<1, 1>(const GatherGemmArgs);
template __global__ void gg_plp_kernel<1, 2>(const GatherGemmArgs);
template __global__ void gg_plp_kernel<1, 3>(const GatherGemmArgs);

constexpr int PLH_HW = 18;
constexpr int PLH_PIECES = 24;
constexpr int PLH_HROWS = PLH_PIECES * 16;
template <int NTERMS>
constexpr int plh_halo_bytes() { return (NTERMS == 3 ? 2 : 1) * PLH_HROWS * PL_ROW; }
template <int NTERMS>
constexpr int plh_bstage_bytes() { return (NTERMS == 3 ? 2 : 1) * PL_BN * PL_ROW; }
template <int NTERMS>
constexpr int plh_lds_bytes() { return 2 * plh_halo_bytes<NTERMS>() + 3 * plh_bstage_bytes<NTERMS>() + 256 * 4 + 64; }

template <int NTERMS, bool BNB = false, bool EP = false>
__global__ __launch_bounds__(512, 2) void gg_plh_kernel(const GatherGemmArgs a) {
    constexpr int BM = 256, BN = PL_BN, WN = 64, AT = 4, ROW = PL_ROW;
    constexpr int NPL = NTERMS == 3 ? 2 : 1;
    constexpr int HALO = plh_halo_bytes<NTERMS>(), HPL = PLH_HROWS * ROW;
    constexpr int BST = plh_bstage_bytes<NTERMS>();
    constexpr int NB = NPL, NH = 3 * NPL;
    constexpr unsigned OOB = 0x80000000u;
    extern __shared__ __attribute__((aligned(16))) float smem[];
    char* lds = reinterpret_cast<char*>(smem);
    char* const ldsB = lds + 2 * HALO;
    int* rowoff = reinterpret_cast<int*>(lds + 2 * HALO + 3 * BST);

    const int tile = xcd_remap(blockIdx.x, gridDim.x);
    const int tm = tile / a.tiles_n;
    const int n0 = (tile % a.tiles_n) * BN;
    const int tid = threadIdx.x, lane = tid & 63;
    const int wave = __builtin_amdgcn_readfirstlane(tid >> 6);
// ... 112 lines not shown
    for (int s = 0; s < S; ++s) {
        const bool more = c + 1 < nchunks;
        const int young = (s + 1 < S ? NB : 0) + ((more && (t == 1 || t == 2)) ? NH : 0);
        if (young == NB + NH) {
            if constexpr (NPL == 2) asm volatile("s_waitcnt vmcnt(8)" ::: "memory"); else asm volatile("s_waitcnt vmcnt(4)" ::: "memory");
        } else if (young == NB) {
            if constexpr (NPL == 2) asm volatile("s_waitcnt vmcnt(2)" ::: "memory"); else asm volatile("s_waitcnt vmcnt(1)" ::: "memory");
        } else {
            asm volatile("s_waitcnt vmcnt(0)" ::: "memory");
        }
        __builtin_amdgcn_s_barrier();
        __builtin_amdgcn_sched_barrier(0);
        if (s + 2 < S) issue_b(s + 2, nslot);
        if (t == 0 && more) issue_halo(c + 1);
        __builtin_amdgcn_sched_barrier(0);
        compute(c, t, slot);
        __builtin_amdgcn_sched_barrier(0);
        slot = slot == 2 ? 0 : slot + 1;
        nslot = nslot == 2 ? 0 : nslot + 1;
        if (++t == 9) { t = 0; ++c; }
    }
    asm volatile("s_waitcnt vmcnt(0)" ::: "memory");
    __syncthreads();
    pl_epilogue<NTERMS, BM, BNB, 4, EP, false>(a, acc, acc_lo, rowoff, reinterpret_cast<float*>(smem), tm, n0, wave_m, wave_n, lane, tid, y0 + 16 <= a.P && x0 + 16 <= a.Q);
}

template __global__ void gg_plh_kernel<3>(const GatherGemmArgs);
template __global__ void gg_plh_kernel<1>(const GatherGemmArgs);

template __global__ void gg_pl_kernel<3, 128>(const GatherGemmArgs);
template __global__ void gg_pl_kernel<3, 256>(const GatherGemmArgs);
template __global__ void gg_pl_kernel<1, 128>(const GatherGemmArgs);
template __global__ void gg_pl_kernel<1, 256>(const GatherGemmArgs);
template __global__ void gg_pl_kernel<3, 128, true>(const GatherGemmArgs);
template __global__ void gg_pl_kernel<3, 256, true>(const GatherGemmArgs);
#ifdef PYLC_EXPERIMENTAL
template __global__ void gg_pl_kernel<3, 128, false, true>(const GatherGemmArgs);
template __global__ void gg_pl_kernel<3, 256, false, true>(const GatherGemmArgs);
template __global__ void gg_pl_kernel<1, 128, false, true>(const GatherGemmArgs);
template __global__ void gg_pl_kernel<1, 256, false, true>(const GatherGemmArgs);
#endif
template __global__ void gg_pl_kernel<3, 128, false, false, true>(const GatherGemmArgs);
template __global__ void gg_pl_kernel<3, 256, false, false, true>(const GatherGemmArgs);
template __global__ void gg_pl_kernel<1, 128, false, false, true>(const GatherGemmArgs);
template __global__ void gg_pl_kernel<1, 256, false, false, true>(const GatherGemmArgs);
#ifdef PYLC_EXPERIMENTAL
template __global__ void gg_plh_kernel<3, true>(const GatherGemmArgs);
template __global__ void gg_plh_kernel<1, true>(const GatherGemmArgs);
#endif
template __global__ void gg_pl_kernel<3, 128, false, false, false, true>(const GatherGemmArgs);
template __global__ void gg_pl_kernel<3, 256, false, false, false, true>(const GatherGemmArgs);
template __global__ void gg_pl_kernel<1, 128, false, false, false, true>(const GatherGemmArgs);
template __global__ void gg_pl_kernel<1, 256, false, false, false, true>(const GatherGemmArgs);
template __global__ void gg_pl_kernel<3, 128, false, false, true, true>(const GatherGemmArgs);
template __global__ void gg_pl_kernel<3, 256, false, false, true, true>(const GatherGemmArgs);
template __global__ void gg_pl_kernel<1, 128, false, false, true, true>(const GatherGemmArgs);
template __global__ void gg_pl_kernel<1, 256, false, false, true, true>(const GatherGemmArgs);
template __global__ void gg_plh_kernel<3, false, true>(const GatherGemmArgs);
template __global__ void gg_plh_kernel<1, false, true>(const GatherGemmArgs);


template <int NTERMS>
constexpr int plhn_bstage_bytes() { return (NTERMS == 3 ? 2 : 1) * 64 * PL_ROW; }
template <int NTERMS>
constexpr int plhn_lds_bytes() { return plh_halo_bytes<NTERMS>() + 3 * plhn_bstage_bytes<NTERMS>() + 256 * 4 + 64; }

// ... 154 lines not shown
            if (s + 2 < S) issue_b(s + 2, nslot);
        }
        __builtin_amdgcn_sched_barrier(0);
        compute(t, slot);
        __builtin_amdgcn_sched_barrier(0);
        slot = slot == 2 ? 0 : slot + 1;
        nslot = nslot == 2 ? 0 : nslot + 1;
        if (++t == 9) { t = 0; ++c; }
    }
    static_assert(NB == NPL, "counted waits above: one filter DMA instruction per plane, wave and step");
    asm volatile("s_waitcnt vmcnt(0)" ::: "memory");
    __syncthreads();
    pl_epilogue<NTERMS, BM, false, 4, EP, false>(a, acc, acc_lo, rowoff, reinterpret_cast<float*>(smem), tm, n0, wave, 0, lane, tid, y0 + 16 <= a.P && x0 + 16 <= a.Q, nullptr, BNN);
}

template __global__ void gg_plhn_kernel<3>(const GatherGemmArgs);
template __global__ void gg_plhn_kernel<1>(const GatherGemmArgs);
template __global__ void gg_plhn_kernel<3, true>(const GatherGemmArgs);
template __global__ void gg_plhn_kernel<1, true>(const GatherGemmArgs);


int g_stagger = -1;
extern "C" int pylc_debug_stagger(int units) { g_stagger = units; return PYLC_OK; }

bool takes_pl(const GatherGemmArgs& a) {
    const bool aligned = a.y_pitch % 4 == 0 && a.N_store % 4 == 0 && (reinterpret_cast<uintptr_t>(a.y) & 15) == 0 &&
                         (reinterpret_cast<uintptr_t>(a.x_planes) & 15) == 0 && (a.x_plane_stride % 8) == 0 && a.x_pitch % 8 == 0;
    const bool ila = a.nterms == 3 && planes_il(a.x_plane_stride);
    if (ila && (a.Cin % 32 != 0 || a.x_pitch != a.Cin || a.x_bytes >= (1ll << 30))) return false;
    return a.x_planes != nullptr && a.w_planes != nullptr && aligned && a.Cin % 8 == 0 && a.x_bytes > 0 && a.x_bytes < (1ll << 31) &&
           a.w_plane_stride * 4 < (1ll << 31);
}

template <int NTERMS, int BM>
static void launch_pl(const GatherGemmArgs& a, unsigned grid, hipStream_t st) {
    constexpr int lds_bytes = pl_lds_bytes<NTERMS, BM>();
    if (NTERMS == 3 && (a.dbg != nullptr || (a.dbg_flags & (64 | 128)))) {
        hipLaunchKernelGGL((gg_pl_kernel<3, BM, true>), dim3(grid), dim3(BM * 2), lds_bytes + 4096, st, a);
        return;
    }
    const bool ep = a.ep_scale != nullptr || a.ep_amax != nullptr || a.out_planes2 || a.ep_res != nullptr;
    if (ep && a.N_store <= 64 && !(g_pp_flags & 65536)) hipLaunchKernelGGL((gg_pl_kernel<NTERMS, BM, false, false, true, true>), dim3(grid), dim3(BM * 2), lds_bytes, st, a);
    else if (ep) hipLaunchKernelGGL((gg_pl_kernel<NTERMS, BM, false, false, false, true>), dim3(grid), dim3(BM * 2), lds_bytes, st, a);
#ifdef PYLC_EXPERIMENTAL
    else if (a.bn_y != nullptr) hipLaunchKernelGGL((gg_pl_kernel<NTERMS, BM, false, true>), dim3(grid), dim3(BM * 2), lds_bytes, st, a);
#endif
    else if (a.N_store <= 64 && !(g_pp_flags & 65536)) hipLaunchKernelGGL((gg_pl_kernel<NTERMS, BM, false, false, true>), dim3(grid), dim3(BM * 2), lds_bytes, st, a);
    else hipLaunchKernelGGL((gg_pl_kernel<NTERMS, BM>), dim3(grid), dim3(BM * 2), lds_bytes, st, a);
}

int launch_gg_pl(GatherGemmArgs& a, hipStream_t st) {
    PYLC_REQUIRE(takes_pl(a), "conv (fp16-plane operands): needs prepared filter planes, Cin %% 8 == 0, pitches %% 8 == 0, 16-byte aligned "
                              "buffers below 2 GiB per plane");
    if (a.dh_step > 2 || a.dh_step < -2 || a.dw_step > 2 || a.dw_step < -2) a.dbg_flags |= 4096;
    a.ident = a.TR == 1 && a.TS == 1 && a.in_sh == 1 && a.in_sw == 1 && a.dh0 == 0 && a.dw0 == 0 && a.IH == a.P && a.IW == a.Q &&
              a.out_sh == 1 && a.out_sw == 1 && a.oh0 == 0 && a.ow0 == 0 && a.OH == a.P && a.OW == a.Q;
    PYLC_REQUIRE(!(a.out_half || a.out_planes2) ||
                     (a.out_bound != nullptr && a.amax_x && a.amax_w && !a.accumulate && a.add_src == nullptr && a.bn_y == nullptr &&
                      (a.bias == nullptr || a.ep_scale != nullptr) && a.y_pitch == a.N_store && a.N_store % 8 == 0),
                 "conv with an fp16-plane output: needs out_bound, the operand ranges and a dense y of a multiple of 8 channels; no accumulation, residual-gradient source or BatchNorm sums "
                 "(a bias only with the fused inference epilogue)");
    PYLC_REQUIRE(a.ep_res == nullptr || a.ep_res_fmt == 0 || (a.ep_res_scale != nullptr && a.y_pitch == a.N_store && a.N_store % 8 == 0),
                 "conv with a fused fp16-plane residual: needs the residual's scale bound and a dense y of a multiple of 8 channels");
    PYLC_REQUIRE(!(a.ep_scale != nullptr || a.out_planes2 || a.ep_res != nullptr) || (a.stats == nullptr && !a.accumulate && a.add_src == nullptr && a.bn_y == nullptr),
                 "conv with the fused inference epilogue: no statistics, accumulation or backward fusions");
    PYLC_REQUIRE(a.add_src == nullptr || (a.y_pitch == a.N_store && a.N_store % 8 == 0 && !a.accumulate),
                 "conv dgrad with a masked residual source needs a dense output (pitch == channels, channels %% 8 == 0) and no accumulation");
    PYLC_REQUIRE(a.bn_y == nullptr || (a.y_pitch == a.N_store && a.stats != nullptr && a.bn_mean && a.bn_invstd && (!a.bn_relu || a.bn_mask || (a.bn_scale && a.bn_shift))),
                 "conv dgrad with BatchNorm-backward sums needs a dense output, a partials buffer, mean / invstd and a mask source");
// ... 40 lines not shown
        } else if (a.nterms == 1) hipLaunchKernelGGL((gg_plh_kernel<1>), dim3((unsigned)n_tiles), dim3(512), plh_lds_bytes<1>(), st, a);
        else hipLaunchKernelGGL((gg_plh_kernel<3>), dim3((unsigned)n_tiles), dim3(512), plh_lds_bytes<3>(), st, a);
        PYLC_LAUNCH_CHECK();
        return PYLC_OK;
    }
    const long long ksteps = (long long)a.TR * a.TS * cdiv(a.Cin, BK);
    const long long tiles256 = (long long)cdiv(a.M, 256) * cdiv(a.N_store, PL_BN);
    bool big = ksteps >= 24 && tiles256 >= kNumCU;
    if (g_pp_flags & 2048) big = false;
    if (a.TR * a.TS > 1 && !(g_pp_flags & 8388608)) big = false;
    if (g_pp_flags & 8192) big = true;
    const int bm = big ? 256 : 128;
    a.tile_bm = bm;
    a.tiles_n = cdiv(a.N_store, PL_BN);
    const long long n_tiles = (long long)cdiv(a.M, bm) * a.tiles_n;
    PYLC_REQUIRE(n_tiles > 0 && n_tiles < (1ll << 31), "conv grid out of range");
    a.n_tiles = (int)n_tiles;
    a.stagger = 0;
    a.stagger_blocks = 2 * kNumCU;
    if (!big && n_tiles >= 3 * kNumCU) {
        const long long cycles = (ksteps * 1200 + 8000) / 2;
        a.stagger = (int)(cycles / 2048);
        if (g_stagger >= 0) a.stagger = g_stagger;
    }
    const bool ep_any = a.ep_scale != nullptr || a.ep_amax != nullptr || a.out_planes2 || a.ep_res != nullptr;
    const int ks_tile = a.nterms == 1 ? 64 : 32;
    const float* extra_src = a.add_src != nullptr ? a.add_src : (a.accumulate ? a.y : nullptr);
    if (!big && !(g_pp_flags & 524288) && a.ident && n_tiles > 2 * kNumCU && !ep_any && a.bn_y == nullptr && (a.dbg == nullptr || a.nterms == 3) &&
        !(a.dbg_flags & (8 | 64 | 128)) && cdiv(a.Cin, ks_tile) >= 2 &&
        a.M % 128 == 0 && a.N_store % PL_BN == 0 && a.bias == nullptr && !a.out_half && !(a.stats != nullptr && extra_src != nullptr) && PYLC_EPI_FULL_LINES != 0 &&
        (long long)a.M * a.y_pitch < (1ll << 31) && (a.add_mask == nullptr || (a.y_pitch == a.N_store && (reinterpret_cast<uintptr_t>(a.add_mask) & 7) == 0))) {
        const unsigned grid = (g_pp_flags & 1048576) ? (unsigned)n_tiles : ((g_pp_flags & 4194304) ? 3 * kNumCU : 2 * kNumCU);
        const int epk = extra_src != nullptr ? (a.add_mask != nullptr ? 3 : 2) : (a.stats != nullptr ? 1 : 0);
#define PYLC_PLP(NT, E) hipLaunchKernelGGL((gg_plp_kernel<NT, E>), dim3(grid), dim3(256), plp_lds_bytes<NT>(), st, a)
        if (a.dbg != nullptr && epk <= 1) {
            if (epk == 0) hipLaunchKernelGGL((gg_plp_kernel<3, 0, true>), dim3(grid), dim3(256), plp_lds_bytes<3>() + 4096, st, a);
            else hipLaunchKernelGGL((gg_plp_kernel<3, 1, true>), dim3(grid), dim3(256), plp_lds_bytes<3>() + 4096, st, a);
            PYLC_LAUNCH_CHECK();
            return PYLC_OK;
        }
        if (a.nterms == 1) { if (epk == 0) PYLC_PLP(1, 0); else if (epk == 1) PYLC_PLP(1, 1); else if (epk == 2) PYLC_PLP(1, 2); else PYLC_PLP(1, 3); }
        else { if (epk == 0) PYLC_PLP(3, 0); else if (epk == 1) PYLC_PLP(3, 1); else if (epk == 2) PYLC_PLP(3, 2); else PYLC_PLP(3, 3); }
#undef PYLC_PLP
        PYLC_LAUNCH_CHECK();
        return PYLC_OK;
    }
    if (a.nterms == 1) {
        if (big) launch_pl<1, 256>(a, (unsigned)n_tiles, st); else launch_pl<1, 128>(a, (unsigned)n_tiles, st);
    } else {
        if (big) launch_pl<3, 256>(a, (unsigned)n_tiles, st); else launch_pl<3, 128>(a, (unsigned)n_tiles, st);
    }
    PYLC_LAUNCH_CHECK();
    return PYLC_OK;
}

template <typename K>
static hipError_t opt_in(K kernel, int bytes) {
    return hipFuncSetAttribute(reinterpret_cast<const void*>(kernel), hipFuncAttributeMaxDynamicSharedMemorySize, bytes);
}

int conv_pl_init() {
    PYLC_HIP(opt_in(gg_pl_kernel<3, 128>, pl_lds_bytes<3, 128>()));
    PYLC_HIP(opt_in(gg_pl_kernel<3, 256>, pl_lds_bytes<3, 256>()));
    PYLC_HIP(opt_in(gg_pl_kernel<1, 128>, pl_lds_bytes<1, 128>()));
    PYLC_HIP(opt_in(gg_pl_kernel<1, 256>, pl_lds_bytes<1, 256>()));
    PYLC_HIP(opt_in(gg_plh_kernel<3>, plh_lds_bytes<3>()));
    PYLC_HIP(opt_in(gg_plh_kernel<1>, plh_lds_bytes<1>()));
    PYLC_HIP(opt_in(gg_plhn_kernel<3>, plhn_lds_bytes<3>()));
    PYLC_HIP(opt_in(gg_plhn_kernel<1>, plhn_lds_bytes<1>()));
    PYLC_HIP(opt_in((gg_plhn_kernel<3, true>), plhn_lds_bytes<3>()));
    PYLC_HIP(opt_in((gg_plhn_kernel<1, true>), plhn_lds_bytes<1>()));
    PYLC_HIP(opt_in((gg_plp_kernel<3, 0>), plp_lds_bytes<3>()));
    PYLC_HIP(opt_in((gg_plp_kernel<3, 0, true>), plp_lds_bytes<3>() + 4096));
    PYLC_HIP(opt_in((gg_plp_kernel<3, 1, true>), plp_lds_bytes<3>() + 4096));
    PYLC_HIP(opt_in((gg_plp_kernel<3, 1>), plp_lds_bytes<3>()));
    PYLC_HIP(opt_in((gg_plp_kernel<3, 2>), plp_lds_bytes<3>()));
    PYLC_HIP(opt_in((gg_plp_kernel<3, 3>), plp_lds_bytes<3>()));
    PYLC_HIP(opt_in((gg_plp_kernel<1, 0>), plp_lds_bytes<1>()));
    PYLC_HIP(opt_in((gg_plp_kernel<1, 1>), plp_lds_bytes<1>()));
    PYLC_HIP(opt_in((gg_plp_kernel<1, 2>), plp_lds_bytes<1>()));
    PYLC_HIP(opt_in((gg_plp_kernel<1, 3>), plp_lds_bytes<1>()));
#ifdef PYLC_EXPERIMENTAL
    PYLC_HIP(opt_in((gg_pl_kernel<3, 128, false, true>), pl_lds_bytes<3, 128>()));
    PYLC_HIP(opt_in((gg_pl_kernel<3, 256, false, true>), pl_lds_bytes<3, 256>()));
    PYLC_HIP(opt_in((gg_pl_kernel<1, 128, false, true>), pl_lds_bytes<1, 128>()));
    PYLC_HIP(opt_in((gg_pl_kernel<1, 256, false, true>), pl_lds_bytes<1, 256>()));
#endif
    PYLC_HIP(opt_in((gg_pl_kernel<3, 128, false, false, true>), pl_lds_bytes<3, 128>()));
    PYLC_HIP(opt_in((gg_pl_kernel<3, 256, false, false, true>), pl_lds_bytes<3, 256>()));
    PYLC_HIP(opt_in((gg_pl_kernel<1, 128, false, false, true>), pl_lds_bytes<1, 128>()));
    PYLC_HIP(opt_in((gg_pl_kernel<1, 256, false, false, true>), pl_lds_bytes<1, 256>()));
#ifdef PYLC_EXPERIMENTAL
    PYLC_HIP(opt_in((gg_plh_kernel<3, true>), plh_lds_bytes<3>()));
    PYLC_HIP(opt_in((gg_plh_kernel<1, true>), plh_lds_bytes<1>()));
#endif
    PYLC_HIP(opt_in((gg_pl_kernel<3, 128, false, false, false, true>), pl_lds_bytes<3, 128>()));
    PYLC_HIP(opt_in((gg_pl_kernel<3, 256, false, false, false, true>), pl_lds_bytes<3, 256>()));
    PYLC_HIP(opt_in((gg_pl_kernel<1, 128, false, false, false, true>), pl_lds_bytes<1, 128>()));
    PYLC_HIP(opt_in((gg_pl_kernel<1, 256, false, false, false, true>), pl_lds_bytes<1, 256>()));
    PYLC_HIP(opt_in((gg_pl_kernel<3, 128, false, false, true, true>), pl_lds_bytes<3, 128>()));
    PYLC_HIP(opt_in((gg_pl_kernel<3, 256, false, false, true, true>), pl_lds_bytes<3, 256>()));
    PYLC_HIP(opt_in((gg_pl_kernel<1, 128, false, false, true, true>), pl_lds_bytes<1, 128>()));
    PYLC_HIP(opt_in((gg_pl_kernel<1, 256, false, false, true, true>), pl_lds_bytes<1, 256>()));
    PYLC_HIP(opt_in((gg_plh_kernel<3, false, true>), plh_lds_bytes<3>()));
    PYLC_HIP(opt_in((gg_plh_kernel<1, false, true>), plh_lds_bytes<1>()));
    PYLC_HIP(opt_in(gg_pl_kernel<3, 128, true>, pl_lds_bytes<3, 128>() + 4096));
    PYLC_HIP(opt_in(gg_pl_kernel<3, 256, true>, pl_lds_bytes<3, 256>() + 4096));

    return PYLC_OK;
}

}
```

### pylc_amd/layers.py

```python
import math

import torch
from torch import nn

from . import ops
from .runtime import runtime


class Conv2d(nn.Module):

    def __init__(self, cin, cout, k, stride=1, padding=0, dilation=1, bias=False, init='resnet', bn=False):
        super().__init__()
        self.cin, self.cout, self.k = cin, cout, k
        self.feeds_bn = bn and cout % 4 == 0
        self.bn_frozen = False
        self.stride, self.padding, self.dilation = stride, padding, dilation
        w = torch.empty(cout, k, k, cin)
        fan_in = cin * k * k
        if init == 'resnet':
            w.normal_(0, math.sqrt(2.0 / (k * k * cout)))
        elif init == 'kaiming':
            w.normal_(0, math.sqrt(2.0 / fan_in))
        else:
            w.uniform_(-1.0 / math.sqrt(fan_in), 1.0 / math.sqrt(fan_in))
        self.weight = nn.Parameter(w.permute(0, 3, 1, 2))
        if bias:
            self.bias = nn.Parameter(torch.empty(cout).uniform_(-1.0 / math.sqrt(fan_in), 1.0 / math.sqrt(fan_in)))
        else:
            self.register_parameter('bias', None)

    def forward(self, x, res_link=None, out=None):
        return ops.conv2d(x, self.weight, self.bias, self.stride, self.padding, self.dilation, self.feeds_bn and self.training and not self.bn_frozen, res_link, out)

    def takes_planes(self):
        return self.cout % 4 == 0 and self.cin % 8 == 0

    def extra_repr(self):
        return '%d, %d, k=%d, s=%d, p=%d, d=%d%s' % (self.cin, self.cout, self.k, self.stride, self.padding, self.dilation,
                                                      '' if self.bias is None else ', bias')


class DepthwiseConv3x3(nn.Module):

    def __init__(self, c, stride=1, dilation=1):
        super().__init__()
        self.c, self.stride, self.dilation = c, stride, dilation
        self.bn_frozen = False
        self.weight = nn.Parameter(torch.empty(c, 1, 3, 3).normal_(0, math.sqrt(2.0 / (9 * c))))

    def forward(self, x, res_link=None):
        return ops.dwconv3x3(x, self.weight, self.stride, self.dilation, res_link, want_stats=self.training and not self.bn_frozen)


class BatchNorm2d(nn.Module):

    frozen = False

    def __init__(self, c, eps=1e-5, momentum=0.1):
        super().__init__()
        self.num_features, self.eps, self.momentum = c, eps, momentum
        self.weight = nn.Parameter(torch.ones(c))
        self.bias = nn.Parameter(torch.zeros(c))
        self.register_buffer('running_mean', torch.zeros(c))
        self.register_buffer('running_var', torch.ones(c))
        self.register_buffer('num_batches_tracked', torch.zeros((), dtype=torch.long))
# ... 114 lines not shown
```

### pylc_amd/lib.py

```python
import ctypes as C
import os

import torch

_HERE = os.path.dirname(os.path.abspath(__file__))
LIB_PATH = os.environ.get('PYLC_LIB') or os.path.join(_HERE, 'libpylc_hip.so')

ABI_VERSION = 15


class PylcError(RuntimeError):
    pass


class ConvDesc(C.Structure):
    _fields_ = [(n, C.c_int) for n in ('B', 'H', 'W', 'Cin', 'Cout', 'R', 'S', 'stride', 'pad', 'dil',
                                       'OH', 'OW', 'x_pitch', 'y_pitch')] + \
               [(n, C.c_void_p) for n in ('x_amax', 'w_amax', 'dy_amax',
                                          'w_planes', 'w_planes_t')] + \
               [(n, C.c_int) for n in ('x_fmt', 'dy_fmt', 'out_fmt')] + [('out_bound', C.c_void_p)] + \
               [('w_planes_fmt', C.c_int)]


class WPrepEntry(C.Structure):
# ... 53 lines not shown
    'pylc_debug_pp_flags': (_I, [_I]),
    'pylc_debug_stagger': (_I, [_I]),
    'pylc_debug_wgrad_flags': (_I, [_I]),
    'pylc_debug_wgrad_max_steps': (_I, [_I]),
    'pylc_comm_available': (_I, []),
    'pylc_comm_unique_id': (_I, [_P]),
    'pylc_comm_init': (_I, [_P, _I, _I, C.POINTER(C.c_void_p)]),
    'pylc_comm_allreduce': (_I, [_P, _P, _LL, _I, _P]),
    'pylc_comm_syncbn_reduce': (_I, [_P, _P, _I, _P]),
    'pylc_comm_destroy': (_I, [_P]),
    'pylc_debug_dw_tiles': (_I, [_I]),
    'pylc_range_product': (_I, [_P, _P, _F, _P, _P, _P]),
    'pylc_maxpool_fwd_planes': (_I, [_P, _P, _LL, _I, _P, _P, _I, _I, _I, _I, _I, _I, _I, _I, _I, _P]),
    'pylc_upsample2_crop_concat_planes': (_I, [_P, _I, _I, _I, _I, _I, _P, _I, _I, _I, _I, _P, _LL, _I, _P, _P]),
    'pylc_conv1x1_fold_input_affine': (_I, [_P, _P, _P, _P, _I, _I, _P, _P, _P, _P]),
    'pylc_debug_wgrad_acc1': (_I, [_I]),
    'pylc_debug_wgrad_sets': (_I, [_I]),
    'pylc_debug_wgrad_m16': (_I, [_I]),
    'pylc_debug_wgrad_dma': (_I, [_I]),
    'pylc_debug_pp_stamps': (_I, [_P]),
    'pylc_amax': (_I, [_P, _LL, _I, _I, _P, _P]),
    'pylc_amax_segments': (_I, [_P, _P, _I, _P, _P]),
    'pylc_to_planes': (_I, [_P, _I, _P, _I, _LL, _LL, _I, _P, _I, _P]),
    'pylc_from_planes': (_I, [_P, _I, _LL, _P, _I, _LL, _I, _P, _I, _P]),
    'pylc_planes_colsum_workspace_floats': (C.c_size_t, [_I]),
    'pylc_planes_colsum': (_I, [_P, _I, _LL, _I, _P, _LL, _I, _P, _P, _P]),
    'pylc_weight_prepare': (_I, [_P, _P, _I, _LL, _P, _P, _I, _P]),
    'pylc_conv2d_dgrad_needs_f32_weights': (_I, [C.POINTER(ConvDesc)]),
    'pylc_conv2d_fwd': (_I, [C.POINTER(ConvDesc), _P, _P, _P, _P, _P]),
    'pylc_conv2d_fwd_bnact': (_I, [C.POINTER(ConvDesc), _P, _P, _P, _P, _P, _P, _I, _P, _P, _P]),
    'pylc_conv2d_fwd_bnact_ex': (_I, [C.POINTER(ConvDesc), _P, _P, _P, C.POINTER(FwdEp), _P, _P]),
    'pylc_conv2d_fwd_stats_floats': (_SZ, [C.POINTER(ConvDesc)]),
    'pylc_conv2d_fwd_stats': (_I, [C.POINTER(ConvDesc), _P, _P, _P, _P, _P, C.POINTER(_I), _P]),
    'pylc_conv2d_dgrad': (_I, [C.POINTER(ConvDesc), _P, _P, _P, _I, _P]),
    'pylc_conv2d_dgrad_add': (_I, [C.POINTER(ConvDesc), _P, _P, _P, _I, _P, _P, _P]),
    'pylc_relu_bwd_bits': (_I, [_P, _P, _P, _LL, _I, _P]),
    'pylc_conv2d_dgrad_bn_floats': (_SZ, [C.POINTER(ConvDesc)]),
    'pylc_conv2d_dgrad_bn': (_I, [C.POINTER(ConvDesc), _P, _P, _P, _I, _P, _P, C.POINTER(BnBack), _P, C.POINTER(_I), _P]),
    'pylc_bn_bwd_sums_from_partial': (_I, [_P, _I, _I, _P, _P, _P, _D, _P, _P, _P]),
    'pylc_conv2d_wgrad_workspace': (_SZ, [C.POINTER(ConvDesc)]),
    'pylc_conv2d_wgrad': (_I, [C.POINTER(ConvDesc), _P, _P, _P, _P, _P, _SZ, _P]),
    'pylc_conv2d_wgrad_slabs': (_I, [C.POINTER(ConvDesc), _P, _P, _P, _P, _SZ, C.POINTER(SlabSum), _P]),
    'pylc_splitk_reduce_batch': (_I, [_P, _P, _I, C.c_longlong, _P]),
    'pylc_weight_transpose': (_I, [_P, _P, _I, _I, _I, _P]),
    'pylc_dwconv3x3_fwd': (_I, [C.POINTER(DwDesc), _P, _P, _P, _P]),
    'pylc_dwconv3x3_fwd_stats_rows': (_I, [C.POINTER(DwDesc)]),
    'pylc_dwconv3x3_fwd_stats': (_I, [C.POINTER(DwDesc), _P, _P, _P, _P, _P]),
    'pylc_dwconv3x3_dgrad': (_I, [C.POINTER(DwDesc), _P, _P, _P, _P]),
    'pylc_dwconv3x3_dgrad_acc': (_I, [C.POINTER(DwDesc), _P, _P, _P, _I, _P]),
    'pylc_dwconv3x3_wgrad_workspace': (_SZ, [C.POINTER(DwDesc)]),
    'pylc_dwconv3x3_wgrad': (_I, [C.POINTER(DwDesc), _P, _P, _P, _P, _SZ, _P]),
    'pylc_dwconv3x3_half_ok': (_I, [C.POINTER(DwDesc)]),
    'pylc_dwconv3x3_fwd_h_stats_rows': (_I, [C.POINTER(DwDesc)]),
    'pylc_dwconv3x3_bn_ok': (_I, [C.POINTER(DwDesc)]),
    'pylc_dwconv3x3_fwd_h_bn': (_I, [C.POINTER(DwDesc), _P, _P, _P, _P, _I, _P, _P, _P, _P, _P, _P, _P]),
    'pylc_dwconv3x3_wgrad_h_bn': (_I, [C.POINTER(DwDesc), _P, _P, _P, _P, _I, _P, _P, _P, _P, _P, _SZ, _P]),
    'pylc_dwconv3x3_dgrad_h_add_ok': (_I, [C.POINTER(DwDesc)]),
    'pylc_dwconv3x3_dgrad_h_add': (_I, [C.POINTER(DwDesc), _P, _P, _P, _P, _P, _P, _P, _P]),
    'pylc_dwconv3x3_fwd_h': (_I, [C.POINTER(DwDesc), _P, _P, _P, _P, _P, _P, _P, _P]),
    'pylc_dwconv3x3_fwd_h_eval': (_I, [C.POINTER(DwDesc), _P, _P, _P, _P, _P, _P, _P, _P]),
    'pylc_dwconv3x3_dgrad_h': (_I, [C.POINTER(DwDesc), _P, _P, _P, _P, _P, _P, _I, _P, _P]),
    'pylc_dwconv3x3_wgrad_h': (_I, [C.POINTER(DwDesc), _P, _P, _P, _P, _P, _P, _SZ, _P]),
    'pylc_bn_workspace_floats': (_SZ, [_LL, _I]),
    'pylc_bn_stats': (_I, [_P, _LL, _I, _I, _P, _P, _P]),
    'pylc_bn_stats_from_partial': (_I, [_P, _I, _I, _P, _P]),
    'pylc_bn_finalize': (_I, [_P, _D, _I, _P, _P, _F, _F, _I, _P, _P, _P, _P, _P, _P, _P]),
    'pylc_bn_eval_coeffs': (_I, [_P, _P, _P, _P, _F, _I, _P, _P, _P]),
    'pylc_bn_eval_coeffs_full': (_I, [_P, _P, _P, _P, _F, _I, _P, _P, _P, _P, _P]),
    'pylc_bn_finalize_from_partial': (_I, [_P, _I, _D, _I, _P, _P, _F, _F, _I, _P, _P, _P, _P, _P, _P, _P]),
    'pylc_bn_finalize_ex': (_I, [_P, _D, _I, _P, _P, _F, _F, _I, _P, _P, _P, _P, _P, _P, _P, _F, _P, _P, _I, _LL, _P, _P]),
    'pylc_bn_local_moments': (_I, [_P, _D, _I, _P, _I, _LL, _P, _P, _P]),
    'pylc_bn_finalize_moments': (_I, [_P, _D, _I, _P, _P, _F, _F, _I, _P, _P, _P, _P, _P, _P, _P, _F, _P, _P, _P]),
    'pylc_bn_finalize_from_partial_ex': (_I, [_P, _I, _D, _I, _P, _P, _F, _F, _I, _P, _P, _P, _P, _P, _P, _P, _F, _P, _P, _I, _LL, _P, _P]),
    'pylc_bn_apply_ex': (_I, [_P, _I, _P, _P, _P, _I, _P, _I, _LL, _I, _I, _P, C.POINTER(BnExtra), _P]),
    'pylc_bn_bwd_reduce_ex': (_I, [_P, _I, _P, _I, _P, _I, _P, _P, _LL, _I, _I, _P, _P, _P, _P, _P, _D, C.POINTER(BnExtra), _P, _P]),
    'pylc_bn_bwd_bound': (_I, [_P, _P, _P, _D, _I, _P, _P, _P]),
    'pylc_bn_bwd_apply_ex': (_I, [_P, _I, _P, _I, _P, _I, _P, _P, _P, _P, _D, _LL, _I, _I, _P, _I, _P, _I, _P, _P, _P,
                                  C.POINTER(BnExtra), _P]),
    'pylc_bn_affine_amax': (_I, [_P, _I, _P, _P, _LL, _I, _P, _P]),
    'pylc_bn_apply_pair': (_I, [_P, _I, _P, _P, _P, _I, _LL, _I, _P, C.POINTER(BnExtra), C.POINTER(BnTwin), _P]),
    'pylc_bn_bwd_reduce_pair': (_I, [_P, _I, _P, _I, _P, _P, _LL, _I, _P, _P, _P, _D, C.POINTER(BnExtra), _P, C.POINTER(BnTwin), _P]),
    'pylc_bn_bwd_apply_pair': (_I, [_P, _I, _P, _I, _P, _P, _P, _P, _D, _LL, _I, _P, _I, _P, C.POINTER(BnExtra), C.POINTER(BnTwin), _P]),
    'pylc_bn_apply': (_I, [_P, _I, _P, _P, _P, _I, _P, _I, _LL, _I, _I, _P, _P]),
    'pylc_bn_bwd_reduce': (_I, [_P, _I, _P, _I, _P, _I, _P, _P, _LL, _I, _I, _P, _P, _P, _P, _P]),
    'pylc_bn_bwd_apply': (_I, [_P, _I, _P, _I, _P, _I, _P, _P, _P, _P, _D, _LL, _I, _I, _P, _I, _P, _I, _P, _P, _P, _P]),
    'pylc_bn_frozen_bwd': (_I, [_P, _I, _P, _I, _P, _I, _P, _P, _P, _LL, _I, _I, _P, _I, _P, _I, _P, _P, _P, _P, _P, C.POINTER(BnExtra), _P]),
    'pylc_relu_fwd': (_I, [_P, _I, _P, _I, _LL, _I, _P]),
    'pylc_relu_bwd': (_I, [_P, _I, _P, _I, _P, _I, _LL, _I, _P]),
    'pylc_maxpool_fwd': (_I, [_P, _P, _P, _I, _I, _I, _I, _I, _I, _I, _I, _I, _P]),
    'pylc_maxpool_bwd': (_I, [_P, _P, _P, _I, _I, _I, _I, _I, _I, _I, _I, _I, _P]),
    'pylc_maxpool_bwd_add': (_I, [_P, _P, _P, _I, _I, _I, _I, _I, _I, _I, _I, _I, _P, _I, _I, _I, _I, _I, _P]),
    'pylc_crop_copy': (_I, [_P, _I, _I, _I, _I, _I, _P, _I, _I, _I, _I, _I, _P]),
    'pylc_bilinear_fwd': (_I, [_P, _I, _P, _I, _I, _I, _I, _I, _I, _I, _P]),
    'pylc_bilinear_bwd': (_I, [_P, _I, _P, _I, _I, _I, _I, _I, _I, _I, _P]),
    'pylc_bilinear_bwd_workspace': (C.c_size_t, [_I, _I, _I, _I]),
    'pylc_bilinear_bwd_separable': (_I, [_P, _I, _P, _I, _I, _I, _I, _I, _I, _I, _P, _P, _P]),
    'pylc_gap_fwd': (_I, [_P, _P, _I, _I, _I, _P]),
    'pylc_gap_fwd_planes': (_I, [_P, _LL, _I, _P, _P, _I, _I, _I, _P]),
    'pylc_gap_bwd': (_I, [_P, _P, _I, _I, _I, _P]),
    'pylc_gap_bwd_acc': (_I, [_P, _P, _I, _I, _I, _I, _P]),
    'pylc_image_pack': (_I, [_P, _I, _I, _I, _I, C.POINTER(_F), C.POINTER(_F), _P, _P]),
    'pylc_image_pack_tiles': (_I, [_P, _I, _I, _I, _I, _I, _I, _I, C.POINTER(_F), C.POINTER(_F), _P, _P]),
    'pylc_stitch_argmax': (_I, [_P, _I, _I, _I, _I, _I, _I, _P, _P]),
    'pylc_colourize_resize': (_I, [_P, _I, _I, _P, _P, _I, _I, _P]),
    'pylc_image_pack_tiles_reflect': (_I, [_P, _I, _I, _I, _I, _I, _I, _I, _I, _I, C.POINTER(_F), C.POINTER(_F), _P, _P]),
    'pylc_stitch_overlap_argmax': (_I, [_P, _I, _I, _I, _I, _I, _I, _I, _P, _P, _P]),
# ... 137 lines not shown
```

### pylc_amd/nets/encoder_resnet.py

```python
import torch
from torch import nn

from .. import ops
from ..layers import Conv2d, BatchNorm2d, Named, conv_bn
from ..runtime import runtime


class Bottleneck(nn.Module):
    def __init__(self, inplanes, planes, stride, dilation, project):
        super().__init__()
        self.conv1 = Conv2d(inplanes, planes, 1, bn=True)
        self.bn1 = BatchNorm2d(planes)
        self.conv2 = Conv2d(planes, planes, 3, stride, dilation, dilation, bn=True)
        self.bn2 = BatchNorm2d(planes)
        self.conv3 = Conv2d(planes, planes * 4, 1, bn=True)
        self.bn3 = BatchNorm2d(planes * 4)
        if project:
            self.downsample = Named(_0=Conv2d(inplanes, planes * 4, 1, stride, bn=True), _1=BatchNorm2d(planes * 4))
        else:
            self.downsample = None
        self.pl1, self.pl2 = self.conv2.takes_planes(), self.conv3.takes_planes()
        self.out_planes = False

    def forward(self, x):
        link = ops.grad_link(x)
        out = conv_bn(self.conv1, self.bn1, x, relu=True, conv_link=link, out_planes=self.pl1, sole=True)
        out = conv_bn(self.conv2, self.bn2, out, relu=True, out_planes=self.pl2, sole=True)
        if self.downsample is not None:
            if self.pair_eligible(torch.is_grad_enabled() and (x.requires_grad or self.bn3.weight.requires_grad)):
                return self._tail_pair(out, x, link)
            res = conv_bn(self.downsample.child(0), self.downsample.child(1), x, conv_link=link)
            return self._tail(out, res, None)
        return self._tail(out, x, link)

    def pair_eligible(self, needs_grad=True):
        bn3, dbn = self.bn3, self.downsample.child(1)
        return ops.proj_pair_eligible(runtime.fuse_proj_bn, bn3.training and dbn.training, bn3.frozen or dbn.frozen,
                                      runtime.sync_group if runtime.sync_bn else None, runtime.bn_clamp_eps, None, bn3.num_features,
                                      not ops.half_acts(), not runtime.no_relu_bits, needs_grad)

    def _tail_pair(self, out, x, link):
        dconv, dbn, bn3 = self.downsample.child(0), self.downsample.child(1), self.bn3
        y_ds = dconv(x, res_link=link)
        y3 = self.conv3(out)
        bn3._nbt_pending += 1
        dbn._nbt_pending += 1
        return ops.bn_act_pair(y3, bn3.weight, bn3.bias, bn3.running_mean, bn3.running_var, bn3.eps, bn3.momentum,
                               y_ds, dbn.weight, dbn.bias, dbn.running_mean, dbn.running_var, dbn.eps, dbn.momentum,
                               out_planes=self.out_planes)

    def _tail(self, out, res, link):
        if link is None:
            return conv_bn(self.conv3, self.bn3, out, residual=res, relu=True, out_planes=self.out_planes)
        return self.bn3(self.conv3(out), residual=res, relu=True, res_link=link, out_planes=self.out_planes)


class ResNet101(nn.Module):
    LAYERS = ((64, 3), (128, 4), (256, 23))
    MULTI_GRID = (1, 2, 4)

    def __init__(self, output_stride=16):
        super().__init__()
        if output_stride == 16:
            strides, dils = (1, 2, 2, 1), (1, 1, 1, 2)
        elif output_stride == 8:
            strides, dils = (1, 2, 1, 1), (1, 1, 2, 4)
        else:
            raise NotImplementedError(output_stride)
        self.conv1 = Conv2d(3, 64, 7, 2, 3, bn=True)
        self.bn1 = BatchNorm2d(64)
        inpl = 64
        for li, (planes, n) in enumerate(self.LAYERS):
            blocks = []
            for b in range(n):
                s = strides[li] if b == 0 else 1
                blocks.append(Bottleneck(inpl, planes, s, dils[li], b == 0 and (s != 1 or inpl != planes * 4)))
# ... 24 lines not shown
```

### pylc_amd/ops/bn.py

```python
from . import _core
from ._core import *


def _bn_extra(**kw):
    ex = L.BnExtra()
    ex.nplanes = nplanes()
    for k, v in kw.items():
        setattr(ex, k, v)
    return ex


class BnState:
    __slots__ = ('cfg', 'g_param', 'b_param', 'y_shape', 'clamp', 'bn_emit_ok', 'sole', 'pre_sums', 'want_amax', 'out_pl', 'drop', 'dy_pl', 'res_link')

    def __init__(self, cfg, g_param, b_param, y_shape=None, clamp=(False, 1e-5), bn_emit_ok=False, sole=False, want_amax=False, out_pl=False,
                 drop=(0.0, 0), dy_pl=False, res_link=None):
        self.cfg, self.g_param, self.b_param, self.y_shape = cfg, g_param, b_param, y_shape
        self.clamp, self.want_amax, self.out_pl, self.drop, self.dy_pl, self.res_link = clamp, want_amax, out_pl, drop, dy_pl, res_link
        self.bn_emit_ok, self.sole, self.pre_sums = bn_emit_ok, sole, None


def bn_node_of(x):
    src = x.grad_fn if (torch.is_grad_enabled() and x.requires_grad) else None
    return src if isinstance(getattr(src, 'st', None), BnState) else None
# ... 353 lines not shown
        tm.__exit__()
        if amax_dy is not None:
            tag_amax(dy, amax_dy)
        dgamma = dbeta = None
        if direct:
            _deliver_grad(gamma, tg)
            _deliver_grad(beta, tb)
        else:
            if ctx.needs_input_grad[1]:
                if tg is not None:
                    tg.copy_(sums[:c])
                    dgamma = _deliver_grad(gamma, tg)
                else:
                    dgamma = sums[:c].clone()
            if ctx.needs_input_grad[2]:
                if tb is not None:
                    tb.copy_(sums[c:])
                    dbeta = _deliver_grad(beta, tb)
                else:
                    dbeta = sums[c:].clone()
        if res_is_dout:
            g_out = dout
        if g_out is not None and armed and lk.buf is None and lk.masked is None:
            lk.buf = g_out
            g_out = None
        return (dy if ctx.needs_input_grad[0] else None, dgamma, dbeta, None, None, g_out) + (None,) * 6


def proj_pair_eligible(fuse, training, frozen, group, clamp_eps, drop, channels, fp32_y, relu_bits, needs_grad=True):
    return bool(fuse and training and not frozen and group is None and not clamp_eps and drop is None and channels % 8 == 0 and fp32_y
                and relu_bits and needs_grad)


def _pair_finalize(y, yp, pre_sums, gamma, beta, running_mean, running_var, eps, momentum, coef, res_amax, bound, m, c, st):
    mean, invstd, scale, shift = coef[:c], coef[c:2 * c], coef[2 * c:3 * c], coef[3 * c:]
    refine_y = y if _runtime.bn_refine else None
    partial = pre_sums if (pre_sums is not None and pre_sums.dim() == 2 and pre_sums.shape[1] == 2 * c) else None
    kshift = getattr(partial, '_pylc_shift', None) if partial is not None else None
    if partial is not None:
        check(lib.pylc_bn_finalize_from_partial_ex(ptr(partial), partial.shape[0], float(m), c, ptr(gamma), ptr(beta), eps, momentum, 0,
                                                   ptr(running_mean), ptr(running_var), ptr(mean), ptr(invstd), ptr(scale), ptr(shift),
                                                   ptr(res_amax), 1.0, ptr(bound), ptr(refine_y), yp, m, ptr(kshift), st))
    else:
        sums = torch.empty(2 * c, device=y.device)
        ws = torch.empty(lib.pylc_bn_workspace_floats(m, c), device=y.device)
        check(lib.pylc_bn_stats(ptr(y), m, c, yp, ptr(sums), ptr(ws), st))
        check(lib.pylc_bn_finalize_ex(ptr(sums), float(m), c, ptr(gamma), ptr(beta), eps, momentum, 0, ptr(running_mean), ptr(running_var),
                                      ptr(mean), ptr(invstd), ptr(scale), ptr(shift), ptr(res_amax), 1.0, ptr(bound), ptr(refine_y), yp, m,
                                      None, st))


def _pair_param_grads(ctx, gi, bi, gamma, beta, tg, tb, direct, sums, c):
    dgamma = dbeta = None
    if direct:
        _deliver_grad(gamma, tg)
        _deliver_grad(beta, tb)
        return None, None
    if ctx.needs_input_grad[gi]:
        if tg is not None:
            tg.copy_(sums[:c])
            dgamma = _deliver_grad(gamma, tg)
        else:
            dgamma = sums[:c].clone()
    if ctx.needs_input_grad[bi]:
        if tb is not None:
            tb.copy_(sums[c:])
            dbeta = _deliver_grad(beta, tb)
        else:
            dbeta = sums[c:].clone()
    return dgamma, dbeta


class BnPairFn(torch.autograd.Function):

    @staticmethod
    def forward(ctx, y, y2, gamma, beta, running_mean, running_var, gamma2, beta2, running_mean2, running_var2, eps, momentum, eps2, momentum2,
                pre_sums, pre_sums2, want_amax, out_planes, dy_planes, dy_planes2):
        L.init()
        ctx.set_materialize_grads(False)
        y, y2 = as_nhwc(y), as_nhwc(y2)
        b, c, h, w = y.shape
        if tuple(y2.shape) != (b, c, h, w) or c % 8:
            raise L.PylcError('bn_act_pair: shapes %s / %s (need equal shapes, C %% 8 == 0)' % (tuple(y.shape), tuple(y2.shape)))
        m = b * h * w
        dev = y.device
        st = stream()
        yp, yp2 = pitch_of(y), pitch_of(y2)
        if m == 1:
            raise ValueError('Expected more than 1 value per channel when training, got input size %s' % (tuple(y.shape),))
        out_planes = bool(out_planes and planes_ok(c, m) and m >= _core.PLANES_MIN_PIXELS)
        coef, coef2 = torch.empty(4 * c, device=dev), torch.empty(4 * c, device=dev)
        bound = amax_slot(dev) if out_planes else None
        _pair_finalize(y2, yp2, pre_sums2, gamma2, beta2, running_mean2, running_var2, eps2, momentum2, coef2, None, None, m, c, st)
        res_amax = None
        if out_planes:
            res_amax = amax_slot(dev)
            tm = _bn_time('apply_range+proj', m, c, m * c * 4)
            tm.__enter__()
            check(lib.pylc_bn_affine_amax(ptr(y2), yp2, ptr(coef2[2 * c:3 * c]), ptr(coef2[3 * c:]), m, c, ptr(res_amax), st))
            tm.__exit__()
        _pair_finalize(y, yp, pre_sums, gamma, beta, running_mean, running_var, eps, momentum, coef, res_amax, bound, m, c, st)
        out = empty_nhwc(b, c, h, w, dev)
        amax = amax_slot(dev) if (want_amax and not out_planes) else None
        mask = torch.empty(m * c // 8, dtype=torch.uint8, device=dev)
        tm = _bn_time('apply+res+bits+proj', m, c, m * c * (4 + (2 * nplanes() if out_planes else 4) + 4 + 0.125))
        tm.__enter__()
        ex = _bn_extra()
        ex.relu_mask = ptr(mask)
        if out_planes:
            ex.out_planes, ex.out_plane_stride, ex.out_bound = ptr(out), pstride(m, c), ptr(bound)
        tw = L.BnTwin()
        tw.y, tw.y_pitch, tw.scale, tw.shift = ptr(y2), yp2, ptr(coef2[2 * c:3 * c]), ptr(coef2[3 * c:])
        check(lib.pylc_bn_apply_pair(ptr(y), yp, ptr(coef[2 * c:3 * c]), ptr(coef[3 * c:]), None if out_planes else ptr(out), c, m, c, ptr(amax),
                                     C.byref(ex), C.byref(tw), st))
        tm.__exit__()
        ctx.save_for_backward(y, y2, coef, coef2, mask)
        ctx.params = (gamma, beta, gamma2, beta2)
        ctx.want_amax = want_amax
        ctx.dy_pl = bool(dy_planes and planes_ok(c, m) and yp == c)
        ctx.dy_pl2 = bool(dy_planes2 and planes_ok(c, m) and yp2 == c)
        if out_planes:
            ctx.mark_non_differentiable(bound)
            return out, bound
        if want_amax:
            ctx.mark_non_differentiable(amax)
            return out, amax
        return out

    @staticmethod
    def backward(ctx, dout, *_unused):
        if dout is None:
            return (None,) * 20
        y, y2, coef, coef2, mask = ctx.saved_tensors
        gamma, beta, gamma2, beta2 = ctx.params
        dout = as_nhwc(dout)
        b, c, h, w = y.shape
        m = b * h * w
        dev = y.device
        st = stream()
        yp, yp2 = pitch_of(y), pitch_of(y2)
        n = float(m)
        tg, tb, tg2, tb2 = _grad_target(gamma), _grad_target(beta), _grad_target(gamma2), _grad_target(beta2)
        direct = (tg is not None and tb is not None and tb.data_ptr() == tg.data_ptr() + 4 * c
                  and ctx.needs_input_grad[2] and ctx.needs_input_grad[3])
        direct2 = (tg2 is not None and tb2 is not None and tb2.data_ptr() == tg2.data_ptr() + 4 * c
                   and ctx.needs_input_grad[6] and ctx.needs_input_grad[7])
        sums = torch.as_strided(tg, (2 * c,), (1,)) if direct else torch.empty(2 * c, device=dev)
        sums2 = torch.as_strided(tg2, (2 * c,), (1,)) if direct2 else torch.empty(2 * c, device=dev)
        ws = torch.empty(lib.pylc_bn_workspace_floats(m, c), device=dev)
        ws2 = torch.empty(lib.pylc_bn_workspace_floats(m, c), device=dev)
        dy_pl, dy_pl2 = ctx.dy_pl, ctx.dy_pl2
        g_amax = amax_slot(dev) if (dy_pl or dy_pl2) else None
        dy_bound = amax_slot(dev) if dy_pl else None
        dy_bound2 = amax_slot(dev) if dy_pl2 else None
        ex = _bn_extra()
        ex.relu_mask, ex.g_amax = ptr(mask), ptr(g_amax)
        tw = L.BnTwin()
        tw.y, tw.y_pitch, tw.mean, tw.invstd, tw.gamma = ptr(y2), yp2, ptr(coef2[:c]), ptr(coef2[c:2 * c]), ptr(gamma2)
        tw.sums, tw.workspace, tw.dy_bound_out = ptr(sums2), ptr(ws2), ptr(dy_bound2)
        tm = _bn_time('bwd_reduce(+sums)+proj', m, c, m * c * (12 + 0.125))
        tm.__enter__()
        check(lib.pylc_bn_bwd_reduce_pair(ptr(dout), pitch_of(dout), ptr(y), yp, ptr(coef[:c]), ptr(coef[c:2 * c]), m, c, ptr(sums), ptr(ws),
                                          ptr(gamma), n, C.byref(ex), ptr(dy_bound), C.byref(tw), st))
        tm.__exit__()
        dy, dy2 = empty_nhwc(b, c, h, w, dev), empty_nhwc(b, c, h, w, dev)
        amax_dy = amax_slot(dev) if (ctx.want_amax and not dy_pl) else None
        amax_dy2 = amax_slot(dev) if (ctx.want_amax and not dy_pl2) else None
        tm = _bn_time('bwd_apply+proj', m, c, m * c * (12 + 0.125 + (2 * nplanes() if dy_pl else 4) + (2 * nplanes() if dy_pl2 else 4)))
        tm.__enter__()
        if dy_pl:
            ex.dy_planes, ex.dy_plane_stride, ex.dy_bound = ptr(dy), pstride(m, c), ptr(dy_bound)
        if dy_pl2:
            tw.dy_planes, tw.dy_plane_stride, tw.dy_bound = ptr(dy2), pstride(m, c), ptr(dy_bound2)
        else:
            tw.dy = ptr(dy2)
        tw.dy_pitch, tw.amax_dy = c, ptr(amax_dy2)
        check(lib.pylc_bn_bwd_apply_pair(ptr(dout), pitch_of(dout), ptr(y), yp, ptr(coef[:c]), ptr(coef[c:2 * c]), ptr(gamma), ptr(sums), n, m, c,
                                         None if dy_pl else ptr(dy), c, ptr(amax_dy), C.byref(ex), C.byref(tw), st))
        tm.__exit__()
        for t, pl, bnd, amx in ((dy, dy_pl, dy_bound, amax_dy), (dy2, dy_pl2, dy_bound2, amax_dy2)):
            if pl:
                mark_planes(t, bnd)
            elif amx is not None:
                tag_amax(t, amx)
            t._pylc_zero_colsum = True
        dgamma, dbeta = _pair_param_grads(ctx, 2, 3, gamma, beta, tg, tb, direct, sums, c)
        dgamma2, dbeta2 = _pair_param_grads(ctx, 6, 7, gamma2, beta2, tg2, tb2, direct2, sums2, c)
        return (dy, dy2, dgamma, dbeta, None, None, dgamma2, dbeta2) + (None,) * 12


def bn_act_pair(y, gamma, beta, running_mean, running_var, eps, momentum, y2, gamma2, beta2, running_mean2, running_var2, eps2, momentum2,
                out_planes=False):
    pre, pre2 = getattr(y, '_pylc_sums', None), getattr(y2, '_pylc_sums', None)
    dy_ok = not _runtime.no_planes and _runtime.planes_dy
    dy_pl, dy_pl2 = bool(getattr(y, '_pylc_dy_pl', False)) and dy_ok, bool(getattr(y2, '_pylc_dy_pl', False)) and dy_ok
    ranged = ranges_needed()
    out_planes = bool(out_planes) and ranged and not _runtime.no_planes
    args = (y, y2, gamma, beta, running_mean, running_var, gamma2, beta2, running_mean2, running_var2, eps, momentum, eps2, momentum2, pre, pre2)
    if not ranged:
        return BnPairFn.apply(*args, False, False, False, False)
    out, tagv = BnPairFn.apply(*args, True, out_planes, dy_pl, dy_pl2)
    if is_planes_candidate(out_planes, True, y):
        mark_planes(out, tagv)
    else:
        tag_amax(out, tagv)
    return out


def _drive_collectives(gens, group):
    results = [None] * len(gens)
    live = list(range(len(gens)))
    while live:
        msgs = []
        for i in list(live):
            try:
                msgs.append(next(gens[i]))
            except StopIteration as e:
                results[i] = e.value
                live.remove(i)
        if len(msgs) == 1:
            _runtime.sync_all_reduce(msgs[0], group)
        elif msgs:
            flat = torch.cat([t.reshape(-1) for t in msgs])
            _runtime.sync_all_reduce(flat, group)
            o = 0
            for t in msgs:
                t.copy_(flat[o:o + t.numel()].view_as(t))
                o += t.numel()
    return results


class GroupBnActFn(torch.autograd.Function):

    @staticmethod
# ... 105 lines not shown
```

### pylc_amd/ops/conv.py

```python
from . import _core
from ._core import *
from .bn import bn_node_of


def pad_stem_filter(w, cin):
    cout, cin_w, r, s = w.shape
    w_k = torch.zeros((cout, r, s, cin), device=w.device, dtype=torch.float32)
    w_k[..., :cin_w] = w.detach().permute(0, 2, 3, 1)
    return w_k


def _padded_stem_filter(w, cin):
    arena = getattr(w, '_pylc_arena', None)
    arena = arena() if arena is not None else None
    key = (w._version, arena.generation if arena is not None else -1, cin)
    cache = getattr(w, '_pylc_w4', None)
    if cache is not None and cache[0] == key:
        return cache[1]
    w_k = pad_stem_filter(w, cin)
    w._pylc_w4 = (key, w_k)
    return w_k


class ConvState:
    __slots__ = ('geom', 'w_param', 'b_param', 'ranges', 'x_pl', 'dy_pl_ok', 'res_link', 'bn_src')

    def __init__(self, geom, w_param, b_param, ranges=(None, None), x_pl=False, dy_pl_ok=False, res_link=None, bn_src=None):
        self.geom, self.w_param, self.b_param, self.ranges = geom, w_param, b_param, ranges
        self.x_pl, self.dy_pl_ok = x_pl, dy_pl_ok
        self.res_link, self.bn_src = res_link, bn_src


def conv2d_forward(needs, x, w, bias, stride, pad, dil, want_stats=False, x_amax=None, w_amax=None, res_link=None, out=None, convert=False,
                   bn_src=None):
    L.init()
    res_link = res_link.arm() if (res_link is not None and needs[0]) else None
    bn_src = bn_src if needs[0] else None
    cout, cin_w, r, s = w.shape
    b_, _, h_, w_ = x.shape
    takes = conv_takes_planes(w, b_ * h_ * w_, 0) and w_amax is not None and out is None
    if takes and not is_planes(x) and convert:
        cache = getattr(x, '_pylc_plcache', None)
        if cache is not None and cache[1] == x._version:
            x = cache[0]
        else:
            src = x
            x = to_planes(x, x_amax)
            src._pylc_plcache = (x, src._version)
    x_pl = takes and is_planes(x)
    if not x_pl:
        x = as_nhwc(x)
        if _runtime.debug_planes:
            print('[pylc] conv fwd on fp32 operands: x %s w %s takes=%s grad=%s' % (tuple(x.shape), tuple(w.shape), takes, torch.is_grad_enabled()), flush=True)
    cin = x.shape[1]
    xp = pitch_of(x)
    w_k = w
    if cin_w % 4 != 0:
        if cin != _r4(cin_w):
            raise L.PylcError('conv expects the %d-channel packed input for a %d-channel filter' % (_r4(cin_w), cin_w))
        w_k = _padded_stem_filter(w, cin)
    elif cin != cin_w:
        raise L.PylcError('conv: input has %d channels, filter expects %d' % (cin, cin_w))
    elif not (w.permute(0, 2, 3, 1).is_contiguous()):
        raise L.PylcError('conv weight must have KRSC (channels_last) memory')
    b, _, h, wd = x.shape
    oh, ow = conv_out_size(h, r, stride, pad, dil), conv_out_size(wd, s, stride, pad, dil)
    if out is not None:
        buf = out[0]
        yp = pitch_of(buf)
        if tuple(buf.shape[2:]) != (oh, ow) or buf.shape[0] != b or buf.shape[1] < cout or cout % 4:
            raise L.PylcError('conv out= buffer %s does not fit a [%d,%d,%d,%d] result' % (tuple(buf.shape), b, cout, oh, ow))
        y = buf[:, :cout]
    else:
        yp = _r4(cout)
        y = empty_nhwc(b, cout, oh, ow, x.device, yp)
    d = _conv_desc(x, cin, cout, r, s, stride, pad, dil, xp, yp)
    if x_pl:
        d.x_fmt = 1
        x_amax = planes_amax(x)
    d.x_amax, d.w_amax = ptr(x_amax), ptr(w_amax)
    y_bound = None
    if want_stats and x_pl and convert and half_acts() and bias is None and out is None and cout % 8 == 0 and yp == cout and planes_ok(cout, b * oh * ow):
        y_bound = amax_slot(x.device)
        d.out_fmt, d.out_bound = 1, ptr(y_bound)
    planes = getattr(w, '_pylc_planes', None) if (w_amax is not None and w_k is w) else None
    if planes is not None:
        d.w_planes, d.w_planes_fmt = ptr(planes[0]), filter_planes_fmt(planes)
    ev = None
    if _core._timer is not None and (x_pl if _core._timer.planes else _is_dominant_tile(b * oh * ow, yp, cin, r * s)):
        ev = _core._timer.bracket(2.0 * b * oh * ow * cout * r * s * cin, 1, 'fwd%dx%d' % (r, s),
                            4.0 * (b * h * wd * cin + cout * r * s * cin + b * oh * ow * cout))
        ev[0].record()
    sums = None
    if want_stats:
        if cout % 4:
            raise L.PylcError('fused BatchNorm statistics need Cout % 4 == 0')
        part = torch.empty(lib.pylc_conv2d_fwd_stats_floats(C.byref(d)), device=x.device)
        rows = C.c_int(0)
        check(lib.pylc_conv2d_fwd_stats(C.byref(d), ptr(x), ptr(w_k), ptr(bias), ptr(y), ptr(part), C.byref(rows), stream()))
        sums = part[:rows.value * 2 * cout].view(rows.value, 2 * cout)
    else:
        check(lib.pylc_conv2d_fwd(C.byref(d), ptr(x), ptr(w_k), ptr(bias), ptr(y), stream()))
    if ev is not None:
        ev[1].record()
    st = ConvState((stride, pad, dil, cin_w, bias is not None), w, bias, (x_amax, w_amax), x_pl,
                   x_pl and cout % 8 == 0 and ow >= 16 and planes_ok(cout, b * oh * ow) and yp == cout, res_link, bn_src)
    aux = tuple(t for t in (sums, y_bound) if t is not None)
    return ((y,) + aux if aux else y), (x, w_k), st, aux


def conv2d_backward(state, saved, needs, dy):
    x, w_k = saved
    flush_deferred_wgrad(x.device)
    stride, pad, dil, cin_w, has_bias = state.geom
    w, bias = state.w_param, state.b_param
    x_pl = state.x_pl
    if x_pl:
        mark_planes(x, state.ranges[0])
    dy_pl = is_planes(dy)
    if x_pl and _runtime.planes_fwd_only:
        x, x_pl = from_planes(x), False
    if dy_pl and not x_pl:
        dy, dy_pl = from_planes(dy), False
    elif x_pl and not dy_pl:
        dy = as_nhwc(dy)
        if dy.shape[1] % 8 == 0 and pitch_of(dy) == dy.shape[1] and planes_ok(dy.shape[1], dy.shape[0] * dy.shape[2] * dy.shape[3]) \
                and dy.shape[3] >= 16:
            dy, dy_pl = to_planes(dy), True
        else:
            x, x_pl = from_planes(x), False
    if not dy_pl:
        dy = as_nhwc(dy)
        if _runtime.debug_planes:
            print('[pylc] conv bwd on fp32 operands: x %s w %s x_pl=%s dy_pl_ok=%s' % (tuple(x.shape), tuple(w.shape), state.x_pl, state.dy_pl_ok), flush=True)
    cout, _, r, s = w.shape
    cin = x.shape[1]
    yp = pitch_of(dy)
    if yp < _r4(cout):
        t = zeros_nhwc(dy.shape[0], cout, dy.shape[2], dy.shape[3], dy.device, _r4(cout))
        t.copy_(dy)
# ... 114 lines not shown
        hold = getattr(w, '_pylc_wgrad_hold', 0) if _runtime.wgrad_hold else 0
        if hold and side is not None and tgt is not None:
            _defer_wgrad(x.device, launch_wgrad, hold)
            dw = None
        elif _runtime.defer_wgrad_1x1 and r * s == 1 and side is not None and tgt is not None:
            _defer_wgrad(x.device, launch_wgrad)
            dw = None
        else:
            dw = launch_wgrad()
    if has_bias and needs[2] and getattr(dy, '_pylc_zero_colsum', False) and _runtime.skip_zero_bias_grad:
        tgt = _grad_target(bias)
        if tgt is not None:
            tgt.zero_()
            db = _deliver_grad(bias, tgt)
        else:
            db = torch.zeros_like(bias)
    elif has_bias and needs[2]:
        db = bias_grad(bias, dy, cout, dy_pl)
    return dx, dw, db


class Conv2dFn(torch.autograd.Function):

    @staticmethod
    def forward(ctx, *args):
        ctx.set_materialize_grads(False)
        return _adapt(ctx, conv2d_forward(ctx.needs_input_grad, *args))

    @staticmethod
    def backward(ctx, dy, *_unused):
        return _adapt_back(ctx, conv2d_backward, dy)


def conv2d(x, w, bias=None, stride=1, pad=0, dil=1, want_stats=False, res_link=None, out=None):
    xa = wa = None
    if ranges_needed():
        L.init()
        xa, wa = amax_of(x), weight_amax(w)
    bn_src = bn_node_of(x)
    if want_stats:
        res = Conv2dFn.apply(x, w, bias, stride, pad, dil, True, xa, wa, res_link, out, torch.is_grad_enabled(), bn_src)
        y, sums = res[0], res[1]
        if len(res) == 3:
            mark_planes(y, res[2])
        y._pylc_sums = sums
        if bias is not None:
            sums._pylc_shift = bias.detach()
    else:
        y = Conv2dFn.apply(x, w, bias, stride, pad, dil, False, xa, wa, res_link, out, torch.is_grad_enabled(), bn_src)
    fn = y.grad_fn
    if fn is not None and fn.st.dy_pl_ok:
        y._pylc_dy_pl = True
    return y


class ConvTranspose2x2Fn(torch.autograd.Function):

    @staticmethod
    def forward(ctx, x, w, bias):
        L.init()
        x = as_nhwc(x)
        b, cin, h, wd = x.shape
        if tuple(w.shape[:1] + w.shape[2:]) != (cin, 2, 2) or not w.permute(0, 2, 3, 1).is_contiguous() or cin % 4 or w.shape[1] % 4:
            raise L.PylcError('conv_transpose2x2: weight must be [Cin, Cout, 2, 2] with KRSC memory, channels multiples of 4')
        cout = w.shape[1]
        y = empty_nhwc(b, cout, 2 * h, 2 * wd, x.device)
        d = _conv_desc(y, cout, cin, 2, 2, 2, 0, 1, cout, pitch_of(x))
        xa = wa = None
        if ranges_needed():
            xa, wa = amax_of(x), weight_amax(w)
            d.dy_amax, d.w_amax = ptr(xa), ptr(wa)
        wt = torch.empty((cout, 4, cin), device=x.device, dtype=torch.float32)
        st = stream()
        check(lib.pylc_weight_transpose(ptr(w), ptr(wt), cin, 4, cout, st))
        check(lib.pylc_conv2d_dgrad(C.byref(d), ptr(x), ptr(wt), ptr(y), 0, st))
        if bias is not None:
# ... 166 lines not shown
```

### pylc_amd/runtime.py

```python
import itertools
import os


class _Runtime:
    def side_stream_on(self):
        if self.wgrad_side_stream is None:
            from .lib import lib
            return lib.pylc_get_conv_precision() == 3
        return bool(self.wgrad_side_stream)

    def __init__(self):
        self.sync_group = None
        self.sync_bn = os.environ.get('PYLC_SYNC_BN', '1') != '0'
        self.coalesce_sync_bn = True
        self.bn_refine = True
        self.defer_wgrad_1x1 = False
        self.wgrad_hold = True
        self.grad_group = None
        self.grad_ready = None
        self.wgrad_side_stream = False if os.environ.get('PYLC_NO_SIDE_STREAM') else (True if os.environ.get('PYLC_SIDE_STREAM') else None)
        self.wgrad_cus = 0
        self.no_relu_bits = False
        self.fuse_res_grad = True
        self.fuse_proj_bn = True
        self.skip_zero_bias_grad = True
        self.defer_bn_apply = True
        self.upcat_planes = True
        self.fused_grad_ranges = True
        self.gap_planes = True
        self.batch_slab_sums = True
        self.fuse_bn_sums = False
        self.half_acts = True
        self.half_dw = True
        self.eval_planes = True
        self.fuse_eval_bn = True
        self.bn_clamp_eps = False
        self.dropout_enabled = True
        self.no_planes = False
        self.planes_dy = True
        self.pool_planes = True
        self.fold_planes = True
        self.dw_wgrad_side = True
        self.adamw_ranges = True
        self.grad_overlap = True
        self.decoder_hold = (0, 0)
        self.debug_planes = False
        self.debug_streams = False
        self.planes_only = ''
        self.planes_fwd_only = False
        self.comm = None
        self.grad_comm = None
        self.shard_check = None
        self.collectives = 0
        self.seed = 0x5EED
        self._counter = itertools.count(1)
        self._apply_overrides(os.environ.get('PYLC_RUNTIME', ''))

# ... 50 lines not shown
```

Before: 445.4 tiles/s.

## Derive projection BN output range from conv epilogue column min/max

The projection-shortcut conv's fused stats epilogue now also records per-column min and max partials using DPP row reductions. The BN finalize kernel reduces them and computes the post-affine amax directly. This replaces the separate apply_range pass over the projection activation that was needed to bound the fp16 planes. It adds epilogue work and a second partial buffer, and the new path is only taken for plain f16x3 fp32-output launches.

```diff
diff --git a/include/pylc_hip.h b/include/pylc_hip.h
--- a/include/pylc_hip.h
+++ b/include/pylc_hip.h
@@ -94,6 +94,8 @@
 size_t pylc_conv2d_fwd_stats_floats(const PylcConvDesc* d);
 int pylc_conv2d_fwd_stats(const PylcConvDesc* d, const float* x, const float* w_krsc, const float* bias,
                           float* y, float* stats_partial, int* stats_rows, void* stream);
+int pylc_conv2d_fwd_stats_mm(const PylcConvDesc* d, const float* x, const float* w_krsc, const float* bias, float* y, float* stats_partial,
+                             int* stats_rows, float* minmax_partial, int* minmax_done, void* stream);
 int pylc_conv2d_dgrad(const PylcConvDesc* d, const float* dy, const float* w_crsk, float* dx,
                       int accumulate, void* stream);
 int pylc_conv2d_dgrad_add(const PylcConvDesc* d, const float* dy, const float* w_crsk, float* dx, int accumulate,
@@ -216,6 +218,10 @@
                                      float* mean, float* invstd, float* scale, float* shift, const unsigned int* bound_extra,
                                      float bound_mul, unsigned int* bound_out, const float* y, int y_pitch, long long M,
                                      const float* stat_shift, void* stream);
+int pylc_bn_finalize_from_partial_mm(const float* partial, const float* minmax_partial, int n_rows, double n, int C, const float* gamma,
+                                     const float* beta, float eps, float momentum, float* running_mean, float* running_var, float* mean,
+                                     float* invstd, float* scale, float* shift, unsigned int* affine_amax_out, const float* y, int y_pitch,
+                                     long long M, const float* stat_shift, void* stream);
 int pylc_bn_local_moments(const float* sums, double n, int C, const float* y, int y_pitch, long long M, const float* stat_shift,
                           double* moments, void* stream);
 int pylc_bn_finalize_moments(const double* moments, double n, int C, const float* gamma, const float* beta, float eps, float momentum,
diff --git a/pylc_amd/csrc/bn.hip b/pylc_amd/csrc/bn.hip
--- a/pylc_amd/csrc/bn.hip
+++ b/pylc_amd/csrc/bn.hip
@@ -360,44 +360,80 @@
                            clamp_eps, running_mean, running_var, mean, invstd, scale, shift, bound_extra, bound_mul, bound_out);
 }
 
+struct BnMm { const float* partial; unsigned* amax_out; };
+__device__ __forceinline__ float (*bn_mm_red())[32][9] {
+    __shared__ float r[2][32][9];
+    return r;
+}
+template <bool MM = false>
 __global__ __launch_bounds__(256) void bn_finalize_partial_kernel(const float* __restrict__ partial, int nrows, double n, int C,
                                                                   const float* __restrict__ gamma, const float* __restrict__ beta, float eps,
                                                                   float momentum, int clamp_eps, float* running_mean, float* running_var,
                                                                   float* mean, float* invstd, float* scale, float* shift,
                                                                   const unsigned* bound_extra, float bound_mul, unsigned* bound_out,
-                                                                  RefineSrc src) {
+                                                                  RefineSrc src, BnMm mm) {
     __shared__ double red[2][32][9];
     const int tx = threadIdx.x & 7, ty = threadIdx.x >> 3;
     const int c = blockIdx.x * 8 + tx;
+    [[maybe_unused]] float mn = INFINITY, mx = -INFINITY;
     double a0 = 0.0, a1 = 0.0;
     if (c < C) {
         for (int r = ty; r < nrows; r += 8 * 32) {
             float v0[8], v1[8];
+            [[maybe_unused]] float w0[MM ? 8 : 1], w1[MM ? 8 : 1];
 #pragma unroll
             for (int u = 0; u < 8; ++u) {
                 const int rr = r + u * 32;
                 const size_t row = rr < nrows ? (size_t)rr : 0;
                 v0[u] = partial[row * 2 * C + c];
                 v1[u] = partial[row * 2 * C + C + c];
+                if constexpr (MM) {
+                    w0[u] = mm.partial[row * 2 * C + c];
+                    w1[u] = mm.partial[row * 2 * C + C + c];
+                }
             }
 #pragma unroll
             for (int u = 0; u < 8; ++u) {
                 const bool ok = r + u * 32 < nrows;
                 a0 += ok ? (double)v0[u] : 0.0;
                 a1 += ok ? (double)v1[u] : 0.0;
+                if constexpr (MM) { mn = fminf(mn, w0[u]); mx = fmaxf(mx, w1[u]); }
             }
         }
     }
     red[0][ty][tx] = a0;
     red[1][ty][tx] = a1;
+    if constexpr (MM) {
+        float (*redm)[32][9] = bn_mm_red();
+        redm[0][ty][tx] = mn;
+        redm[1][ty][tx] = mx;
+    }
     __syncthreads();
     double s0 = 0.0, s1 = 0.0;
     if (ty == 0) {
 #pragma unroll
         for (int k = 0; k < 32; ++k) { s0 += red[0][k][tx]; s1 += red[1][k][tx]; }
+        if constexpr (MM) {
+            float (*redm)[32][9] = bn_mm_red();
+#pragma unroll
+            for (int k = 1; k < 32; ++k) { mn = fminf(mn, redm[0][k][tx]); mx = fmaxf(mx, redm[1][k][tx]); }
+        }
     }
     bn_finalize_tail((double)(float)s0, (double)(float)s1, red, tx, ty, c, n, C, gamma, beta, eps, momentum, clamp_eps, running_mean, running_var,
                      mean, invstd, scale, shift, bound_extra, bound_mul, bound_out, src);
+    if constexpr (MM) {
+        if (threadIdx.x < 64) {
+            float m = 0.f;
+            if (ty == 0 && c < C) {
+                const float sc = scale[c], sh = shift[c];
+                const float k = src.shift != nullptr ? src.shift[c] : 0.f;
+                const float lo = src.shift != nullptr ? mn + k : mn, hi = src.shift != nullptr ? mx + k : mx;
+                const float v0 = lo * sc + sh, v1 = hi * sc + sh;
+                m = fmaxf(fmaxf(m, fabsf(v0)), fabsf(v1));
+            }
+            amax_commit(m, mm.amax_out);
+        }
+    }
 }
 
 __global__ void bn_eval_coeffs_kernel(const float* rm, const float* rv, const float* gamma, const float* beta, float eps,
@@ -883,9 +919,25 @@
     PYLC_REQUIRE((running_mean == nullptr) == (running_var == nullptr), "bn_finalize_from_partial: running stats must both be set or both NULL");
     PYLC_REQUIRE(y == nullptr || (y_pitch >= C && M > 0 && (double)M == n),
                  "bn_finalize_from_partial: the refinement source must be the n rows the partials cover");
-    hipLaunchKernelGGL(bn_finalize_partial_kernel, dim3(cdiv(C, 8)), dim3(256), 0, as_stream(stream), partial, n_rows, n, C, gamma, beta, eps,
+    hipLaunchKernelGGL(bn_finalize_partial_kernel<false>, dim3(cdiv(C, 8)), dim3(256), 0, as_stream(stream), partial, n_rows, n, C, gamma, beta, eps,
                        momentum, clamp_eps, running_mean, running_var, mean, invstd, scale, shift, bound_extra, bound_mul, bound_out,
-                       RefineSrc{y, y_pitch, M, stat_shift});
+                       RefineSrc{y, y_pitch, M, stat_shift}, BnMm{nullptr, nullptr});
+    PYLC_LAUNCH_CHECK();
+    return PYLC_OK;
+}
+
+extern "C" int pylc_bn_finalize_from_partial_mm(const float* partial, const float* minmax_partial, int n_rows, double n, int C, const float* gamma,
+                                                const float* beta, float eps, float momentum, float* running_mean, float* running_var, float* mean,
+                                                float* invstd, float* scale, float* shift, unsigned int* affine_amax_out, const float* y, int y_pitch,
+                                                long long M, const float* stat_shift, void* stream) {
+    PYLC_REQUIRE(partial && minmax_partial && affine_amax_out && n_rows > 0 && gamma && beta && mean && invstd && scale && shift && C > 0 && n > 0,
+                 "bn_finalize_from_partial_mm: bad arguments");
+    PYLC_REQUIRE((running_mean == nullptr) == (running_var == nullptr), "bn_finalize_from_partial_mm: running stats must both be set or both NULL");
+    PYLC_REQUIRE(y == nullptr || (y_pitch >= C && M > 0 && (double)M == n),
+                 "bn_finalize_from_partial_mm: the refinement source must be the n rows the partials cover");
+    hipLaunchKernelGGL(bn_finalize_partial_kernel<true>, dim3(cdiv(C, 8)), dim3(256), 0, as_stream(stream), partial, n_rows, n, C, gamma, beta, eps,
+                       momentum, 0, running_mean, running_var, mean, invstd, scale, shift, nullptr, 1.f, nullptr,
+                       RefineSrc{y, y_pitch, M, stat_shift}, BnMm{minmax_partial, affine_amax_out});
     PYLC_LAUNCH_CHECK();
     return PYLC_OK;
 }
diff --git a/pylc_amd/csrc/conv_common.h b/pylc_amd/csrc/conv_common.h
--- a/pylc_amd/csrc/conv_common.h
+++ b/pylc_amd/csrc/conv_common.h
@@ -119,6 +119,8 @@
     int dbg_flags;
     unsigned long long* dbg;
     float* stats;
+    float* stats_mm;
+    int mm_done;
 };
 
 typedef float f32x4v __attribute__((ext_vector_type(4)));
diff --git a/pylc_amd/csrc/conv_igemm.hip b/pylc_amd/csrc/conv_igemm.hip
--- a/pylc_amd/csrc/conv_igemm.hip
+++ b/pylc_amd/csrc/conv_igemm.hip
@@ -1562,7 +1562,7 @@
 };
 }
 static int conv2d_fwd_impl(const PylcConvDesc* d, const float* x, const float* w, const float* bias, float* y, float* stats, int* stats_rows,
-                           void* stream, const FwdEpilogue* ep = nullptr);
+                           void* stream, const FwdEpilogue* ep = nullptr, float* stats_mm = nullptr, int* mm_done = nullptr);
 
 extern "C" int pylc_conv2d_fwd(const PylcConvDesc* d, const float* x, const float* w, const float* bias, float* y, void* stream) {
     return conv2d_fwd_impl(d, x, w, bias, y, nullptr, nullptr, stream);
@@ -1599,8 +1599,14 @@
     return conv2d_fwd_impl(d, x, w, bias, y, stats_partial, stats_rows, stream);
 }
 
+extern "C" int pylc_conv2d_fwd_stats_mm(const PylcConvDesc* d, const float* x, const float* w, const float* bias, float* y, float* stats_partial,
+                                        int* stats_rows, float* minmax_partial, int* minmax_done, void* stream) {
+    PYLC_REQUIRE(stats_partial && stats_rows && minmax_partial && minmax_done, "conv2d_fwd_stats_mm: null statistics buffer");
+    return conv2d_fwd_impl(d, x, w, bias, y, stats_partial, stats_rows, stream, nullptr, minmax_partial, minmax_done);
+}
+
 static int conv2d_fwd_impl(const PylcConvDesc* d, const float* x, const float* w, const float* bias, float* y, float* stats, int* stats_rows,
-                           void* stream, const FwdEpilogue* ep) {
+                           void* stream, const FwdEpilogue* ep, float* stats_mm, int* mm_done) {
     if (int rc = check_desc(d)) return rc;
     PYLC_REQUIRE(x && y && (w || (d->x_fmt == 1 && d->w_planes)), "null pointer");
     GatherGemmArgs a{};
@@ -1609,6 +1615,7 @@
         a.ep_vec_ok = ((reinterpret_cast<uintptr_t>(ep->scale) | reinterpret_cast<uintptr_t>(ep->shift) | reinterpret_cast<uintptr_t>(bias)) & 15) == 0;
     }
     a.stats = stats;
+    a.stats_mm = stats_mm;
     a.dbg = g_pp_stamps;
     a.dbg_flags = g_pp_flags;
     PYLC_REQUIRE(g_conv_precision < 2 || (d->x_amax && d->w_amax), "f16x3 / fp16 mode: conv2d_fwd needs x_amax and w_amax in the descriptor");
@@ -1657,6 +1664,7 @@
     if (cin4 && ep == nullptr && takes_stem(a)) {
         if (int rc = launch_stem_fwd(a, as_stream(stream))) return rc;
     } else if (int rc = dispatch_gg(a, cin4, as_stream(stream))) return rc;
+    if (mm_done) *mm_done = a.mm_done;
     if (stats_rows) *stats_rows = a.halo_tiles_m > 0 ? a.halo_tiles_m : cdiv(a.M, a.x_planes != nullptr ? a.tile_bm : (a.tiles_n > 0 ? g_last_bm : 128));
     return PYLC_OK;
 }
diff --git a/pylc_amd/csrc/conv_pl.hip b/pylc_amd/csrc/conv_pl.hip
--- a/pylc_amd/csrc/conv_pl.hip
+++ b/pylc_amd/csrc/conv_pl.hip
@@ -51,6 +51,23 @@
 #endif
 }
 
+__device__ __forceinline__ f32x4v epi_min(f32x4v a, f32x4v b) { return f32x4v{fminf(a[0], b[0]), fminf(a[1], b[1]), fminf(a[2], b[2]), fminf(a[3], b[3])}; }
+__device__ __forceinline__ f32x4v epi_max(f32x4v a, f32x4v b) { return f32x4v{fmaxf(a[0], b[0]), fmaxf(a[1], b[1]), fmaxf(a[2], b[2]), fmaxf(a[3], b[3])}; }
+template <bool MAX>
+__device__ __forceinline__ float row_minmax16(float v) {
+#define PYLC_DPP_MM(ctrl)                                                                                                                  \
+    {                                                                                                                                      \
+        const float o = __builtin_bit_cast(float, __builtin_amdgcn_update_dpp(0, __builtin_bit_cast(int, v), ctrl, 0xF, 0xF, true));       \
+        v = MAX ? fmaxf(v, o) : fminf(v, o);                                                                                               \
+    }
+    PYLC_DPP_MM(0xB1);
+    PYLC_DPP_MM(0x4E);
+    PYLC_DPP_MM(0x141);
+    PYLC_DPP_MM(0x140);
+#undef PYLC_DPP_MM
+    return v;
+}
+
 template <int AM, int NPL, int NTERMS>
 __device__ __forceinline__ void pl_step_schedule() {
     constexpr int AT = 4;
@@ -72,8 +89,9 @@
 template <int AM, int STATS, int PREV, bool HALF>
 __device__ __forceinline__ void pl_epilogue_lean(const GatherGemmArgs& a, f32x4v (&acc)[AM][4], const int* rowoff,
                                                  float* sdst, int nb, int wave_m, int lane, float c, float hscale,
-                                                 const float* extra, const unsigned char* amask, const float* bias) {
+                                                 const float* extra, const unsigned char* amask, const float* bias, float* sdst_mm = nullptr) {
     constexpr int AT = 4, WM = 16 * AM;
+    static_assert(STATS != 2 || !HALF, "column min / max: fp32 outputs only");
     typedef _Float16 f16x4_ __attribute__((ext_vector_type(4)));
     typedef unsigned u32x2_ __attribute__((ext_vector_type(2)));
     unsigned offs[AM];
@@ -138,9 +156,14 @@
         f32x4v bv = {0.f, 0.f, 0.f, 0.f};
         if (!HALF && bias != nullptr) bv = *reinterpret_cast<const f32x4v*>(bias + nb + j * 16);
         f32x4v cs = {0.f, 0.f, 0.f, 0.f}, css = cs;
+        [[maybe_unused]] f32x4v cmn = cs, cmx = cs;
 #pragma unroll
         for (int i = 0; i < AM; ++i) {
             const f32x4v t = acc[i][j];
+            if constexpr (STATS == 2) {
+                cmn = i == 0 ? t : epi_min(cmn, t);
+                cmx = i == 0 ? t : epi_max(cmx, t);
+            }
             if constexpr (HALF) {
                 const f32x4v v = epi_mul(t, k);
                 const f16x4_ h = {(_Float16)v[0], (_Float16)v[1], (_Float16)v[2], (_Float16)v[3]};
@@ -192,6 +215,14 @@
             if ((lane & 15) == 0) {
 #pragma unroll
                 for (int r = 0; r < 4; ++r) { sdst[(j * 16 + r) * 2] = cs[r] * post; sdst[(j * 16 + r) * 2 + 1] = css[r] * post * post; }
+            }
+        }
+        if constexpr (STATS == 2) {
+#pragma unroll
+            for (int r = 0; r < 4; ++r) { cmn[r] = row_minmax16<false>(cmn[r]); cmx[r] = row_minmax16<true>(cmx[r]); }
+            if ((lane & 15) == 0) {
+#pragma unroll
+                for (int r = 0; r < 4; ++r) { sdst_mm[(j * 16 + r) * 2] = cmn[r] * post; sdst_mm[(j * 16 + r) * 2 + 1] = cmx[r] * post; }
             }
         }
     }
@@ -487,13 +518,15 @@
     return ep_max;
 }
 
-template <int NTERMS, int BM, bool BNB = false, int AM = 4, bool EP = false, bool LEAN_RES = true>
+template <int NTERMS, int BM, bool BNB = false, int AM = 4, bool EP = false, bool LEAN_RES = true, bool MM = false>
 __device__ __forceinline__ int pl_epilogue(const GatherGemmArgs& a, f32x4v (&acc)[AM][4], f32x4v (&acc_lo)[NTERMS == 3 ? AM : 1][NTERMS == 3 ? 4 : 1],
                                             const int* rowoff, float* smem, int tile_m, int n0, int wave_m, int wave_n, int lane, int tid, bool rows_full,
                                             const unsigned* ranges = nullptr, int stat_cols = PL_BN) {
     constexpr int BN = PL_BN, WM = 16 * AM, WN = 64, AT = 4;
     typedef f32x4v f32x4v_;
+    static_assert(!MM || (NTERMS == 3 && !BNB && !EP && AM == 4), "column min / max: the plain f16x3 launches");
     float* sred = smem;
+    [[maybe_unused]] float* const sred_mm = smem + (BM / WM) * BN * 2;
     const bool do_stats = a.stats != nullptr;
     const unsigned ax_bits = ranges != nullptr ? ranges[0] : (a.amax_x ? *a.amax_x : 0u);
     const unsigned aw_bits = ranges != nullptr ? ranges[1] : (a.amax_w ? *a.amax_w : 0u);
@@ -534,7 +567,8 @@
             float* const sd = smem + ((wave_m * BN) + wave_n * WN + 4 * (lane >> 4)) * 2;
             const int nb = n0 + wave_n * WN + 4 * (lane >> 4);
             const float c = unscale_a * unscale_b;
-#define PYLC_LEAN(ST, PV, HF) pl_epilogue_lean<AM, ST, PV, HF>(a, acc, rowoff, sd, nb, wave_m, lane, c, hscale, extra, amask, a.bias)
+            [[maybe_unused]] float* const sd_mm = sd + (BM / WM) * BN * 2;
+#define PYLC_LEAN(ST, PV, HF) pl_epilogue_lean<AM, ST, PV, HF>(a, acc, rowoff, sd, nb, wave_m, lane, c, hscale, extra, amask, a.bias, sd_mm)
             if constexpr (NTERMS == 1) {
                 if (a.out_half) {
                     if (do_stats) PYLC_LEAN(1, 0, true); else PYLC_LEAN(0, 0, true);
@@ -545,7 +579,7 @@
             } else {
                 if (extra != nullptr) {
                     if (amask != nullptr) PYLC_LEAN(0, 2, false); else PYLC_LEAN(0, 1, false);
-                } else if (do_stats) PYLC_LEAN(1, 0, false);
+                } else if (do_stats) PYLC_LEAN(MM ? 2 : 1, 0, false);
                 else PYLC_LEAN(0, 0, false);
             }
 #undef PYLC_LEAN
@@ -650,6 +684,7 @@
     }
     __builtin_amdgcn_sched_barrier(0);
     float* sdst = sred + ((wave_m * BN) + wave_n * WN + 4 * (lane >> 4)) * 2;
+    [[maybe_unused]] float* const sdst_mm = sdst + (BM / WM) * BN * 2;
     auto finish = [&](auto has_prev, auto j0c, const f32x4v_ (&prev)[AM][PJ]) {
         constexpr int j0 = decltype(j0c)::value;
         constexpr bool phased = decltype(has_prev)::value;
@@ -658,6 +693,7 @@
         for (int jj = 0; jj < NJ; ++jj) {
             const int j = j0 + jj;
             float cs[4] = {0.f, 0.f, 0.f, 0.f}, css[4] = {0.f, 0.f, 0.f, 0.f};
+            [[maybe_unused]] float cmn[4] = {INFINITY, INFINITY, INFINITY, INFINITY}, cmx[4] = {-INFINITY, -INFINITY, -INFINITY, -INFINITY};
 #pragma unroll
             for (int i = 0; i < AM; ++i) {
                 const bool stored = eoff[i][j] >= 0;
@@ -674,6 +710,18 @@
                     const float cv = stored ? val - bv[j][r] : 0.f;
                     cs[r] += cv;
                     css[r] += cv * cv;
+                    if constexpr (MM) {
+                        cmn[r] = fminf(cmn[r], stored ? val - bv[j][r] : INFINITY);
+                        cmx[r] = fmaxf(cmx[r], stored ? val - bv[j][r] : -INFINITY);
+                    }
+                }
+            }
+            if constexpr (MM) {
+#pragma unroll
+                for (int r = 0; r < 4; ++r) { cmn[r] = row_minmax16<false>(cmn[r]); cmx[r] = row_minmax16<true>(cmx[r]); }
+                if ((lane & 15) == 0) {
+#pragma unroll
+                    for (int r = 0; r < 4; ++r) { sdst_mm[(j * 16 + r) * 2] = cmn[r]; sdst_mm[(j * 16 + r) * 2 + 1] = cmx[r]; }
                 }
             }
             if (do_stats) {
@@ -814,13 +862,21 @@
                 float* dst = a.stats + (size_t)tile_m * 2 * a.N_store;
                 dst[n] = sm;
                 dst[a.N_store + n] = sq;
+                if constexpr (MM) {
+                    float mn = INFINITY, mx = -INFINITY;
+#pragma unroll
+                    for (int wm = 0; wm < BM / WM; ++wm) { mn = fminf(mn, sred_mm[(wm * BN + tid) * 2]); mx = fmaxf(mx, sred_mm[(wm * BN + tid) * 2 + 1]); }
+                    float* dmm = a.stats_mm + (size_t)tile_m * 2 * a.N_store;
+                    dmm[n] = mn;
+                    dmm[a.N_store + n] = mx;
+                }
             }
         }
     }
     return tail_stores;
 }
 
-template <int NTERMS, int BM, bool STAMPS = false, bool BNB = false, bool NARROW = false, bool EP = false>
+template <int NTERMS, int BM, bool STAMPS = false, bool BNB = false, bool NARROW = false, bool EP = false, bool MM = false>
 __global__ __launch_bounds__(BM * 2, 2) void gg_pl_kernel(const GatherGemmArgs a) {
     constexpr int BN = PL_BN, AM = NARROW ? 2 : 4, WM = 16 * AM, WN = 64, AT = 4, ROW = pl_row_bytes<NTERMS>();
     constexpr int KS = ROW / 2;
@@ -1085,7 +1141,7 @@
     PL_STAMP();
     __syncthreads();
 
-    pl_epilogue<NTERMS, BM, BNB, AM, EP>(a, acc, acc_lo, rowoff, reinterpret_cast<float*>(smem), tile / a.tiles_n, n0, wave_m, wave_n, lane, tid, m0 + BM <= a.M);
+    pl_epilogue<NTERMS, BM, BNB, AM, EP, true, MM>(a, acc, acc_lo, rowoff, reinterpret_cast<float*>(smem), tile / a.tiles_n, n0, wave_m, wave_n, lane, tid, m0 + BM <= a.M);
     if constexpr (STAMPS) {
         __builtin_amdgcn_sched_barrier(0);
         PL_STAMP();
@@ -1175,7 +1231,7 @@
     }
 }
 
-template <typename Between, typename Stamp>
+template <bool MM, typename Between, typename Stamp>
 __device__ __forceinline__ void plp_epilogue_stats(const GatherGemmArgs& a, f32x4v (&acc)[4][4], const int* rowoff, float* sred, int tile_m, int n0,
                                                    int wave_m, int wave_n, int lane, int tid, float c, Between&& between, Stamp&& stamp) {
     constexpr int AM = 4, AT = 4, WM = 64, WN = 64, BN = PL_BN, BM = 128;
@@ -1198,11 +1254,16 @@
 #pragma unroll
     for (int j = 0; j < AT; ++j) {
         f32x4v cs = {0.f, 0.f, 0.f, 0.f}, css = cs;
+        [[maybe_unused]] f32x4v cmn = cs, cmx = cs;
 #pragma unroll
         for (int i = 0; i < AM; ++i) {
             const f32x4v t = acc[i][j];
             cs = i == 0 ? t : epi_add(cs, t);
             css = i == 0 ? epi_sq(t) : epi_add(css, epi_sq(t));
+            if constexpr (MM) {
+                cmn = i == 0 ? t : epi_min(cmn, t);
+                cmx = i == 0 ? t : epi_max(cmx, t);
+            }
             const f32x4v v = epi_mul(t, c);
             if ((j & 1) == 0) {
                 hold[i] = v;
@@ -1229,6 +1290,18 @@
                 const float s0 = cs[r] * c, s1 = css[r] * c * c;
                 asm volatile("ds_write_b32 %0, %1" :: "v"(sdst_at + (unsigned)((j * 16 + r) * 8)), "v"(s0) : "memory");
                 asm volatile("ds_write_b32 %0, %1" :: "v"(sdst_at + (unsigned)((j * 16 + r) * 8 + 4)), "v"(s1) : "memory");
+            }
+        }
+        if constexpr (MM) {
+#pragma unroll
+            for (int r = 0; r < 4; ++r) { cmn[r] = row_minmax16<false>(cmn[r]); cmx[r] = row_minmax16<true>(cmx[r]); }
+            if ((lane & 15) == 0) {
+#pragma unroll
+                for (int r = 0; r < 4; ++r) {
+                    const float m0 = cmn[r] * c, m1 = cmx[r] * c;
+                    asm volatile("ds_write_b32 %0, %1" :: "v"(sdst_at + (unsigned)(2 * BN * 8 + (j * 16 + r) * 8)), "v"(m0) : "memory");
+                    asm volatile("ds_write_b32 %0, %1" :: "v"(sdst_at + (unsigned)(2 * BN * 8 + (j * 16 + r) * 8 + 4)), "v"(m1) : "memory");
+                }
             }
         }
     }
@@ -1249,6 +1322,18 @@
             float* dst = a.stats + (size_t)tile_m * 2 * a.N_store;
             dst[n] = sm;
             dst[a.N_store + n] = sq;
+            if constexpr (MM) {
+                float q00, q01, q10, q11;
+                asm volatile("ds_read_b32 %0, %1" : "=v"(q00) : "v"(comb_at + (unsigned)(2 * BN * 8)) : "memory");
+                asm volatile("ds_read_b32 %0, %1" : "=v"(q01) : "v"(comb_at + (unsigned)(2 * BN * 8 + 4)) : "memory");
+                asm volatile("ds_read_b32 %0, %1" : "=v"(q10) : "v"(comb_at + (unsigned)(3 * BN * 8)) : "memory");
+                asm volatile("ds_read_b32 %0, %1" : "=v"(q11) : "v"(comb_at + (unsigned)(3 * BN * 8 + 4)) : "memory");
+                asm volatile("s_waitcnt lgkmcnt(0)" ::: "memory");
+                asm volatile("" : "+v"(q00), "+v"(q01), "+v"(q10), "+v"(q11));
+                float* dmm = a.stats_mm + (size_t)tile_m * 2 * a.N_store;
+                dmm[n] = fminf(q00, q10);
+                dmm[a.N_store + n] = fmaxf(q01, q11);
+            }
         }
     }
     static_assert(BM / WM == 2, "two row halves per statistics column");
@@ -1256,6 +1341,8 @@
 
 template <int NTERMS>
 constexpr int plp_lds_bytes() { return 2 * pl_stage_bytes<NTERMS, 128>() + 4 * 128 * 4 + 2 * PL_BN * 2 * 4 + 64; }
+template <int NTERMS>
+constexpr int plp_mm_lds_bytes() { return plp_lds_bytes<NTERMS>() + 2 * PL_BN * 2 * 4; }
 
 #define PLP_VMCNT(n) __builtin_amdgcn_s_waitcnt(((n) & 15) | (((n) >> 4) << 14) | (7 << 4) | (15 << 8))
 __device__ __forceinline__ void plp_wait_vm(int n) {
@@ -1450,8 +1537,8 @@
                     for (int j = 0; j < AT; ++j) acc[i][j] = epi_fma(acc_lo[i][j], 1.f / 2048.f, acc[i][j]);
             }
             auto between = [&]() { pre2 = issue(g & 1); };
-            if constexpr (EPK == 1)
-                plp_epilogue_stats(a, acc, rowoff4 + (k & 3) * BM, sred, tile / a.tiles_n, n0, wave_m, wave_n, lane, tid, c_unscale, between, stamp);
+            if constexpr (EPK == 1 || EPK == 4)
+                plp_epilogue_stats<EPK == 4>(a, acc, rowoff4 + (k & 3) * BM, sred, tile / a.tiles_n, n0, wave_m, wave_n, lane, tid, c_unscale, between, stamp);
             else
                 plp_epilogue_lean<EPK >= 2 ? EPK - 1 : 0>(a, acc, rowoff4 + (k & 3) * BM, n0, wave_m, wave_n, lane, c_unscale, a.add_src != nullptr ? a.add_src : a.y,
                                                           a.add_mask, between, stamp);
@@ -1483,6 +1570,7 @@
 template __global__ void gg_plp_kernel<3, 1>(const GatherGemmArgs);
 template __global__ void gg_plp_kernel<3, 2>(const GatherGemmArgs);
 template __global__ void gg_plp_kernel<3, 3>(const GatherGemmArgs);
+template __global__ void gg_plp_kernel<3, 4>(const GatherGemmArgs);
 template __global__ void gg_plp_kernel<1, 0>(const GatherGemmArgs);
 template __global__ void gg_plp_kernel<1, 1>(const GatherGemmArgs);
 template __global__ void gg_plp_kernel<1, 2>(const GatherGemmArgs);
@@ -1661,6 +1749,8 @@
 template __global__ void gg_pl_kernel<3, 256>(const GatherGemmArgs);
 template __global__ void gg_pl_kernel<1, 128>(const GatherGemmArgs);
 template __global__ void gg_pl_kernel<1, 256>(const GatherGemmArgs);
+template __global__ void gg_pl_kernel<3, 128, false, false, false, false, true>(const GatherGemmArgs);
+template __global__ void gg_pl_kernel<3, 256, false, false, false, false, true>(const GatherGemmArgs);
 template __global__ void gg_pl_kernel<3, 128, true>(const GatherGemmArgs);
 template __global__ void gg_pl_kernel<3, 256, true>(const GatherGemmArgs);
 #ifdef PYLC_EXPERIMENTAL
@@ -1881,9 +1971,22 @@
            a.w_plane_stride * 4 < (1ll << 31);
 }
 
+static bool mm_launch(const GatherGemmArgs& a) {
+    const bool ep = a.ep_scale != nullptr || a.ep_amax != nullptr || a.out_planes2 || a.ep_res != nullptr;
+    return a.stats_mm != nullptr && a.stats != nullptr && a.nterms == 3 && !ep && a.bn_y == nullptr && !a.out_half && !a.accumulate && a.add_src == nullptr &&
+           a.N_store > 64 && a.dbg == nullptr && !(a.dbg_flags & (8 | 64 | 128));
+}
+
 template <int NTERMS, int BM>
-static void launch_pl(const GatherGemmArgs& a, unsigned grid, hipStream_t st) {
+static void launch_pl(GatherGemmArgs& a, unsigned grid, hipStream_t st) {
     constexpr int lds_bytes = pl_lds_bytes<NTERMS, BM>();
+    if constexpr (NTERMS == 3) {
+        if (mm_launch(a)) {
+            a.mm_done = 1;
+            hipLaunchKernelGGL((gg_pl_kernel<3, BM, false, false, false, false, true>), dim3(grid), dim3(BM * 2), lds_bytes, st, a);
+            return;
+        }
+    }
     if (NTERMS == 3 && (a.dbg != nullptr || (a.dbg_flags & (64 | 128)))) {
         hipLaunchKernelGGL((gg_pl_kernel<3, BM, true>), dim3(grid), dim3(BM * 2), lds_bytes + 4096, st, a);
         return;
@@ -1990,6 +2093,12 @@
         (long long)a.M * a.y_pitch < (1ll << 31) && (a.add_mask == nullptr || (a.y_pitch == a.N_store && (reinterpret_cast<uintptr_t>(a.add_mask) & 7) == 0))) {
         const unsigned grid = (g_pp_flags & 1048576) ? (unsigned)n_tiles : ((g_pp_flags & 4194304) ? 3 * kNumCU : 2 * kNumCU);
         const int epk = extra_src != nullptr ? (a.add_mask != nullptr ? 3 : 2) : (a.stats != nullptr ? 1 : 0);
+        if (epk == 1 && mm_launch(a)) {
+            a.mm_done = 1;
+            hipLaunchKernelGGL((gg_plp_kernel<3, 4>), dim3(grid), dim3(256), plp_mm_lds_bytes<3>(), st, a);
+            PYLC_LAUNCH_CHECK();
+            return PYLC_OK;
+        }
 #define PYLC_PLP(NT, E) hipLaunchKernelGGL((gg_plp_kernel<NT, E>), dim3(grid), dim3(256), plp_lds_bytes<NT>(), st, a)
         if (a.dbg != nullptr && epk <= 1) {
             if (epk == 0) hipLaunchKernelGGL((gg_plp_kernel<3, 0, true>), dim3(grid), dim3(256), plp_lds_bytes<3>() + 4096, st, a);
@@ -2034,6 +2143,7 @@
     PYLC_HIP(opt_in((gg_plp_kernel<3, 1>), plp_lds_bytes<3>()));
     PYLC_HIP(opt_in((gg_plp_kernel<3, 2>), plp_lds_bytes<3>()));
     PYLC_HIP(opt_in((gg_plp_kernel<3, 3>), plp_lds_bytes<3>()));
+    PYLC_HIP(opt_in((gg_plp_kernel<3, 4>), plp_mm_lds_bytes<3>()));
     PYLC_HIP(opt_in((gg_plp_kernel<1, 0>), plp_lds_bytes<1>()));
     PYLC_HIP(opt_in((gg_plp_kernel<1, 1>), plp_lds_bytes<1>()));
     PYLC_HIP(opt_in((gg_plp_kernel<1, 2>), plp_lds_bytes<1>()));
@@ -2062,6 +2172,8 @@
     PYLC_HIP(opt_in((gg_pl_kernel<1, 256, false, false, true, true>), pl_lds_bytes<1, 256>()));
     PYLC_HIP(opt_in((gg_plh_kernel<3, false, true>), plh_lds_bytes<3>()));
     PYLC_HIP(opt_in((gg_plh_kernel<1, false, true>), plh_lds_bytes<1>()));
+    PYLC_HIP(opt_in((gg_pl_kernel<3, 128, false, false, false, false, true>), pl_lds_bytes<3, 128>()));
+    PYLC_HIP(opt_in((gg_pl_kernel<3, 256, false, false, false, false, true>), pl_lds_bytes<3, 256>()));
     PYLC_HIP(opt_in(gg_pl_kernel<3, 128, true>, pl_lds_bytes<3, 128>() + 4096));
     PYLC_HIP(opt_in(gg_pl_kernel<3, 256, true>, pl_lds_bytes<3, 256>() + 4096));
 
diff --git a/pylc_amd/layers.py b/pylc_amd/layers.py
--- a/pylc_amd/layers.py
+++ b/pylc_amd/layers.py
@@ -29,8 +29,9 @@
         else:
             self.register_parameter('bias', None)
 
-    def forward(self, x, res_link=None, out=None):
-        return ops.conv2d(x, self.weight, self.bias, self.stride, self.padding, self.dilation, self.feeds_bn and self.training and not self.bn_frozen, res_link, out)
+    def forward(self, x, res_link=None, out=None, want_minmax=False):
+        return ops.conv2d(x, self.weight, self.bias, self.stride, self.padding, self.dilation, self.feeds_bn and self.training and not self.bn_frozen, res_link, out,
+                          want_minmax)
 
     def takes_planes(self):
         return self.cout % 4 == 0 and self.cin % 8 == 0
diff --git a/pylc_amd/lib.py b/pylc_amd/lib.py
--- a/pylc_amd/lib.py
+++ b/pylc_amd/lib.py
@@ -109,6 +109,7 @@
     'pylc_conv2d_fwd_bnact_ex': (_I, [C.POINTER(ConvDesc), _P, _P, _P, C.POINTER(FwdEp), _P, _P]),
     'pylc_conv2d_fwd_stats_floats': (_SZ, [C.POINTER(ConvDesc)]),
     'pylc_conv2d_fwd_stats': (_I, [C.POINTER(ConvDesc), _P, _P, _P, _P, _P, C.POINTER(_I), _P]),
+    'pylc_conv2d_fwd_stats_mm': (_I, [C.POINTER(ConvDesc), _P, _P, _P, _P, _P, C.POINTER(_I), _P, C.POINTER(_I), _P]),
     'pylc_conv2d_dgrad': (_I, [C.POINTER(ConvDesc), _P, _P, _P, _I, _P]),
     'pylc_conv2d_dgrad_add': (_I, [C.POINTER(ConvDesc), _P, _P, _P, _I, _P, _P, _P]),
     'pylc_relu_bwd_bits': (_I, [_P, _P, _P, _LL, _I, _P]),
@@ -149,6 +150,7 @@
     'pylc_bn_local_moments': (_I, [_P, _D, _I, _P, _I, _LL, _P, _P, _P]),
     'pylc_bn_finalize_moments': (_I, [_P, _D, _I, _P, _P, _F, _F, _I, _P, _P, _P, _P, _P, _P, _P, _F, _P, _P, _P]),
     'pylc_bn_finalize_from_partial_ex': (_I, [_P, _I, _D, _I, _P, _P, _F, _F, _I, _P, _P, _P, _P, _P, _P, _P, _F, _P, _P, _I, _LL, _P, _P]),
+    'pylc_bn_finalize_from_partial_mm': (_I, [_P, _P, _I, _D, _I, _P, _P, _F, _F, _P, _P, _P, _P, _P, _P, _P, _P, _I, _LL, _P, _P]),
     'pylc_bn_apply_ex': (_I, [_P, _I, _P, _P, _P, _I, _P, _I, _LL, _I, _I, _P, C.POINTER(BnExtra), _P]),
     'pylc_bn_bwd_reduce_ex': (_I, [_P, _I, _P, _I, _P, _I, _P, _P, _LL, _I, _I, _P, _P, _P, _P, _P, _D, C.POINTER(BnExtra), _P, _P]),
     'pylc_bn_bwd_bound': (_I, [_P, _P, _P, _D, _I, _P, _P, _P]),
diff --git a/pylc_amd/nets/encoder_resnet.py b/pylc_amd/nets/encoder_resnet.py
--- a/pylc_amd/nets/encoder_resnet.py
+++ b/pylc_amd/nets/encoder_resnet.py
@@ -41,7 +41,7 @@
 
     def _tail_pair(self, out, x, link):
         dconv, dbn, bn3 = self.downsample.child(0), self.downsample.child(1), self.bn3
-        y_ds = dconv(x, res_link=link)
+        y_ds = dconv(x, res_link=link, want_minmax=bool(self.out_planes and runtime.proj_range_from_conv))
         y3 = self.conv3(out)
         bn3._nbt_pending += 1
         dbn._nbt_pending += 1
diff --git a/pylc_amd/ops/bn.py b/pylc_amd/ops/bn.py
--- a/pylc_amd/ops/bn.py
+++ b/pylc_amd/ops/bn.py
@@ -409,12 +409,22 @@
                 and relu_bits and needs_grad)
 
 
-def _pair_finalize(y, yp, pre_sums, gamma, beta, running_mean, running_var, eps, momentum, coef, res_amax, bound, m, c, st):
+def pair_minmax_ok(knob, out_planes, pre_sums2, minmax2, channels):
+    return bool(knob and out_planes and pre_sums2 is not None and minmax2 is not None and pre_sums2.dim() == 2 and
+                pre_sums2.shape[1] == 2 * channels and tuple(minmax2.shape) == tuple(pre_sums2.shape))
+
+
+def _pair_finalize(y, yp, pre_sums, gamma, beta, running_mean, running_var, eps, momentum, coef, res_amax, bound, m, c, st, minmax=None,
+                   affine_amax=None):
     mean, invstd, scale, shift = coef[:c], coef[c:2 * c], coef[2 * c:3 * c], coef[3 * c:]
     refine_y = y if _runtime.bn_refine else None
     partial = pre_sums if (pre_sums is not None and pre_sums.dim() == 2 and pre_sums.shape[1] == 2 * c) else None
     kshift = getattr(partial, '_pylc_shift', None) if partial is not None else None
-    if partial is not None:
+    if minmax is not None:
+        check(lib.pylc_bn_finalize_from_partial_mm(ptr(partial), ptr(minmax), partial.shape[0], float(m), c, ptr(gamma), ptr(beta), eps, momentum,
+                                                   ptr(running_mean), ptr(running_var), ptr(mean), ptr(invstd), ptr(scale), ptr(shift),
+                                                   ptr(affine_amax), ptr(refine_y), yp, m, ptr(kshift), st))
+    elif partial is not None:
         check(lib.pylc_bn_finalize_from_partial_ex(ptr(partial), partial.shape[0], float(m), c, ptr(gamma), ptr(beta), eps, momentum, 0,
                                                    ptr(running_mean), ptr(running_var), ptr(mean), ptr(invstd), ptr(scale), ptr(shift),
                                                    ptr(res_amax), 1.0, ptr(bound), ptr(refine_y), yp, m, ptr(kshift), st))
@@ -452,7 +462,7 @@
 
     @staticmethod
     def forward(ctx, y, y2, gamma, beta, running_mean, running_var, gamma2, beta2, running_mean2, running_var2, eps, momentum, eps2, momentum2,
-                pre_sums, pre_sums2, want_amax, out_planes, dy_planes, dy_planes2):
+                pre_sums, pre_sums2, want_amax, out_planes, dy_planes, dy_planes2, minmax2=None):
         L.init()
         ctx.set_materialize_grads(False)
         y, y2 = as_nhwc(y), as_nhwc(y2)
@@ -468,9 +478,13 @@
         out_planes = bool(out_planes and planes_ok(c, m) and m >= _core.PLANES_MIN_PIXELS)
         coef, coef2 = torch.empty(4 * c, device=dev), torch.empty(4 * c, device=dev)
         bound = amax_slot(dev) if out_planes else None
-        _pair_finalize(y2, yp2, pre_sums2, gamma2, beta2, running_mean2, running_var2, eps2, momentum2, coef2, None, None, m, c, st)
         res_amax = None
-        if out_planes:
+        from_conv = pair_minmax_ok(_runtime.proj_range_from_conv, out_planes, pre_sums2, minmax2, c)
+        if from_conv:
+            res_amax = amax_slot(dev)
+        _pair_finalize(y2, yp2, pre_sums2, gamma2, beta2, running_mean2, running_var2, eps2, momentum2, coef2, None, None, m, c, st,
+                       minmax2 if from_conv else None, res_amax)
+        if out_planes and not from_conv:
             res_amax = amax_slot(dev)
             tm = _bn_time('apply_range+proj', m, c, m * c * 4)
             tm.__enter__()
@@ -507,7 +521,7 @@
     @staticmethod
     def backward(ctx, dout, *_unused):
         if dout is None:
-            return (None,) * 20
+            return (None,) * 21
         y, y2, coef, coef2, mask = ctx.saved_tensors
         gamma, beta, gamma2, beta2 = ctx.params
         dout = as_nhwc(dout)
@@ -563,7 +577,7 @@
             t._pylc_zero_colsum = True
         dgamma, dbeta = _pair_param_grads(ctx, 2, 3, gamma, beta, tg, tb, direct, sums, c)
         dgamma2, dbeta2 = _pair_param_grads(ctx, 6, 7, gamma2, beta2, tg2, tb2, direct2, sums2, c)
-        return (dy, dy2, dgamma, dbeta, None, None, dgamma2, dbeta2) + (None,) * 12
+        return (dy, dy2, dgamma, dbeta, None, None, dgamma2, dbeta2) + (None,) * 13
 
 
 def bn_act_pair(y, gamma, beta, running_mean, running_var, eps, momentum, y2, gamma2, beta2, running_mean2, running_var2, eps2, momentum2,
@@ -576,7 +590,7 @@
     args = (y, y2, gamma, beta, running_mean, running_var, gamma2, beta2, running_mean2, running_var2, eps, momentum, eps2, momentum2, pre, pre2)
     if not ranged:
         return BnPairFn.apply(*args, False, False, False, False)
-    out, tagv = BnPairFn.apply(*args, True, out_planes, dy_pl, dy_pl2)
+    out, tagv = BnPairFn.apply(*args, True, out_planes, dy_pl, dy_pl2, getattr(pre2, '_pylc_minmax', None))
     if is_planes_candidate(out_planes, True, y):
         mark_planes(out, tagv)
     else:
diff --git a/pylc_amd/ops/conv.py b/pylc_amd/ops/conv.py
--- a/pylc_amd/ops/conv.py
+++ b/pylc_amd/ops/conv.py
@@ -32,7 +32,7 @@
 
 
 def conv2d_forward(needs, x, w, bias, stride, pad, dil, want_stats=False, x_amax=None, w_amax=None, res_link=None, out=None, convert=False,
-                   bn_src=None):
+                   bn_src=None, want_minmax=False):
     L.init()
     res_link = res_link.arm() if (res_link is not None and needs[0]) else None
     bn_src = bn_src if needs[0] else None
@@ -91,13 +91,20 @@
         ev = _core._timer.bracket(2.0 * b * oh * ow * cout * r * s * cin, 1, 'fwd%dx%d' % (r, s),
                             4.0 * (b * h * wd * cin + cout * r * s * cin + b * oh * ow * cout))
         ev[0].record()
-    sums = None
+    sums = minmax = None
     if want_stats:
         if cout % 4:
             raise L.PylcError('fused BatchNorm statistics need Cout % 4 == 0')
         part = torch.empty(lib.pylc_conv2d_fwd_stats_floats(C.byref(d)), device=x.device)
         rows = C.c_int(0)
-        check(lib.pylc_conv2d_fwd_stats(C.byref(d), ptr(x), ptr(w_k), ptr(bias), ptr(y), ptr(part), C.byref(rows), stream()))
+        if want_minmax and x_pl and y_bound is None and out is None and yp == cout:
+            part_mm, done = torch.empty_like(part), C.c_int(0)
+            check(lib.pylc_conv2d_fwd_stats_mm(C.byref(d), ptr(x), ptr(w_k), ptr(bias), ptr(y), ptr(part), C.byref(rows), ptr(part_mm), C.byref(done),
+                                               stream()))
+            if done.value:
+                minmax = part_mm[:rows.value * 2 * cout].view(rows.value, 2 * cout)
+        else:
+            check(lib.pylc_conv2d_fwd_stats(C.byref(d), ptr(x), ptr(w_k), ptr(bias), ptr(y), ptr(part), C.byref(rows), stream()))
         sums = part[:rows.value * 2 * cout].view(rows.value, 2 * cout)
     else:
         check(lib.pylc_conv2d_fwd(C.byref(d), ptr(x), ptr(w_k), ptr(bias), ptr(y), stream()))
@@ -105,7 +112,7 @@
         ev[1].record()
     st = ConvState((stride, pad, dil, cin_w, bias is not None), w, bias, (x_amax, w_amax), x_pl,
                    x_pl and cout % 8 == 0 and ow >= 16 and planes_ok(cout, b * oh * ow) and yp == cout, res_link, bn_src)
-    aux = tuple(t for t in (sums, y_bound) if t is not None)
+    aux = tuple(t for t in (sums, y_bound, minmax) if t is not None)
     return ((y,) + aux if aux else y), (x, w_k), st, aux
 
 
@@ -286,16 +293,18 @@
         return _adapt_back(ctx, conv2d_backward, dy)
 
 
-def conv2d(x, w, bias=None, stride=1, pad=0, dil=1, want_stats=False, res_link=None, out=None):
+def conv2d(x, w, bias=None, stride=1, pad=0, dil=1, want_stats=False, res_link=None, out=None, want_minmax=False):
     xa = wa = None
     if ranges_needed():
         L.init()
         xa, wa = amax_of(x), weight_amax(w)
     bn_src = bn_node_of(x)
     if want_stats:
-        res = Conv2dFn.apply(x, w, bias, stride, pad, dil, True, xa, wa, res_link, out, torch.is_grad_enabled(), bn_src)
+        res = Conv2dFn.apply(x, w, bias, stride, pad, dil, True, xa, wa, res_link, out, torch.is_grad_enabled(), bn_src, bool(want_minmax))
         y, sums = res[0], res[1]
-        if len(res) == 3:
+        if len(res) == 3 and res[2].dim() == 2:
+            sums._pylc_minmax = res[2]
+        elif len(res) == 3:
             mark_planes(y, res[2])
         y._pylc_sums = sums
         if bias is not None:
diff --git a/pylc_amd/runtime.py b/pylc_amd/runtime.py
--- a/pylc_amd/runtime.py
+++ b/pylc_amd/runtime.py
@@ -23,6 +23,7 @@
         self.no_relu_bits = False
         self.fuse_res_grad = True
         self.fuse_proj_bn = True
+        self.proj_range_from_conv = True
         self.skip_zero_bias_grad = True
         self.defer_bn_apply = True
         self.upcat_planes = True
```

Result: no change. 446.1 tiles/s (median of 4 runs) (+0.2%).
